# Shimmen/ArkoseRenderer

Hardware: AMD Instinct MI355X
Metric: Mrays/s + probes-updated/s, DDGI 32^3 grid x 256 rays, at 1/2/4/8 MI355X (higher is better)
Workload: dtype f32; 1 GPU; C4: synthetic 10M-triangle strip soup, 32x32x32 probes x 256 rays, whole grid updated per step; triangles=10000000, grid=32, rays_per_probe=256, parallelism=zslab1, bvh_nodes=1132708, bvh_max_depth=11

## Files before the change

arkoserenderer_amd/abi.py:

```python
from __future__ import annotations

import ctypes as C
import os

_HERE = os.path.dirname(os.path.abspath(__file__))
LIB_PATH = os.environ.get("ARK_DDGI_LIB") or os.path.join(_HERE, "lib", "libark_ddgi.so")

ARK_DDGI_IRRADIANCE_RES = 8
ARK_DDGI_VISIBILITY_RES = 16
ARK_DDGI_ATLAS_PADDING = 1
ARK_DDGI_MAX_RAYS_PER_PROBE = 512
ARK_DDGI_REFERENCE_MAX_PROBE_UPDATES = 4096

ARK_RT_HIT_MASK_OPAQUE = 0x01
ARK_RT_HIT_MASK_MASKED = 0x02
ARK_RT_HIT_MASK_BLEND = 0x04

ARK_BLEND_MODE_OPAQUE = 1
ARK_BLEND_MODE_MASKED = 2
ARK_BLEND_MODE_TRANSLUCENT = 3

ARK_DDGI_OK = 0
ERRORS = {
    -1: "ARK_DDGI_E_INVALID_ARGUMENT",
    -2: "ARK_DDGI_E_NO_PROBE_GRID",
    -3: "ARK_DDGI_E_NO_SCENE",
    -4: "ARK_DDGI_E_OUT_OF_MEMORY",
    -5: "ARK_DDGI_E_DEVICE",
    -6: "ARK_DDGI_E_UNSUPPORTED",
    -7: "ARK_DDGI_E_SIZE_MISMATCH",
}

ARK_DDGI_ATLAS_IRRADIANCE = 0
ARK_DDGI_ATLAS_VISIBILITY = 1
ARK_DDGI_SURFELS = 2
ARK_DDGI_PROBE_OFFSETS = 3
ARK_DDGI_DEBUG_HITS = 100
ARK_DDGI_DEBUG_RAY_STEPS = 101

ARK_DDGI_CLEAR_OVERFLOW_INF = 0
ARK_DDGI_CLEAR_OVERFLOW_MAX_FINITE = 1
ARK_DDGI_SUN_BVH_AUTO = 0
ARK_DDGI_SUN_BVH_WORLD = 1
ARK_DDGI_SUN_BVH_LIGHT_SPACE = 2
ARK_DDGI_FLAG_SERIAL_FRAMES = 0x1
ARK_DDGI_FLAG_NO_BACKGROUND_REBUILD = 0x2
ARK_DDGI_FLAG_GPU_REBUILD = 0x4
ARK_DDGI_FLAG_GPU_REBUILD_SUN = 0x8
ARK_DDGI_FLAG_GPU_REBUILD_SAH = 0x10
ARK_DDGI_FLAG_GPU_REBUILD_PLAN = 0x80
ARK_DDGI_FLAG_NO_SUN_COVER_MAP = 0x20
ARK_DDGI_FLAG_NO_FUSED_SUN_SHADE = 0x40

ARK_TEX_RGBA8_UNORM = 0
ARK_TEX_RGBA8_SRGB = 1
ARK_TEX_R32F = 2
ARK_TEX_RGBA32F = 3
ARK_BRDF_DEFAULT = 0
ARK_BRDF_SKIN = 1
ARK_WRAP_REPEAT = 0
ARK_WRAP_CLAMP_TO_EDGE = 1
ARK_WRAP_MIRRORED_REPEAT = 2
ARK_WRAP_PER_AXIS = 0x100


def ark_wrap_axes(s: int, t: int) -> int:
    return ARK_WRAP_PER_AXIS | (s & 0xF) | ((t & 0xF) << 4)


class ArkDdgiDesc(C.Structure):
    _fields_ = [
        ("struct_size", C.c_uint32),
        ("grid_dims", C.c_int32 * 3),
        ("probe_spacing", C.c_float * 3),
        ("offset_to_first", C.c_float * 3),
        ("z_far", C.c_float),
        ("max_rays_per_probe", C.c_int32),
        ("max_probe_updates", C.c_int32),
        ("device", C.c_int32),
        ("clear_overflow_mode", C.c_int32),
        ("shard_rank", C.c_int32),
        ("shard_count", C.c_int32),
        ("sun_bvh", C.c_int32),
        ("flags", C.c_uint32),
        ("build_threads", C.c_int32),
        ("reserved", C.c_int32 * 1),
    ]


class ArkRTVertex(C.Structure):
    _fields_ = [("tex_coord", C.c_float * 2), ("normal", C.c_float * 3), ("tangent", C.c_float * 4)]


class ArkRTTriangleMesh(C.Structure):
    _fields_ = [("first_vertex", C.c_int32), ("first_index", C.c_int32), ("material_index", C.c_int32)]


class ArkShaderMaterial(C.Structure):
    _fields_ = [
        ("base_color", C.c_int32),
        ("normal_map", C.c_int32),
        ("metallic_roughness", C.c_int32),
        ("emissive", C.c_int32),
        ("occlusion", C.c_int32),
        ("bent_normal_map", C.c_int32),
# ... 365 lines not shown
    "ark_ddgi_write": (C.c_int, [C.c_void_p, C.c_int, C.c_void_p, C.c_uint64]),
    "ark_ddgi_state_size": (C.c_int, [C.c_void_p, C.POINTER(C.c_uint64)]),
    "ark_ddgi_save_state": (C.c_int, [C.c_void_p, C.c_void_p, C.c_uint64]),
    "ark_ddgi_load_state": (C.c_int, [C.c_void_p, C.c_void_p, C.c_uint64]),
    "ark_ddgi_get_device_views": (C.c_int, [C.c_void_p, C.POINTER(ArkDdgiDeviceViews)]),
    "ark_ddgi_reset_history": (C.c_int, [C.c_void_p]),
    "ark_ddgi_set_counting": (C.c_int, [C.c_void_p, C.c_int]),
    "ark_ddgi_get_counters": (C.c_int, [C.c_void_p, C.POINTER(ArkDdgiCounters)]),
    "ark_ddgi_get_last_timings": (C.c_int, [C.c_void_p, C.POINTER(C.c_float), C.c_int]),
    "ark_ddgi_set_timing": (C.c_int, [C.c_void_p, C.c_int]),
    "ark_ddgi_get_bvh_stats": (C.c_int, [C.c_void_p, C.POINTER(ArkDdgiBvhStats)]),
    "ark_ddgi_bake_ao": (C.c_int, [C.c_void_p, C.POINTER(ArkBakeAoDesc), C.c_void_p]),
    "ark_ddgi_bake_read": (C.c_int, [C.c_void_p, C.c_int, C.c_void_p, C.c_uint64]),
    "ark_ddgi_lighting_compose": (C.c_int, [C.c_void_p, C.POINTER(ArkComposeDesc), C.c_void_p]),
    "ark_ddgi_probe_debug": (C.c_int, [C.c_void_p, C.POINTER(ArkProbeDebugDesc), C.c_void_p]),
    "ark_ddgi_rt_reflections": (C.c_int, [C.c_void_p, C.POINTER(ArkReflectionsDesc), C.c_void_p]),
    "ark_ies_lut_from_memory": (C.c_int, [C.c_char_p, C.c_uint64, C.c_uint32, C.c_void_p, C.POINTER(ArkIesInfo)]),
    "ark_ies_lut_from_file": (C.c_int, [C.c_char_p, C.c_uint32, C.c_void_p, C.POINTER(ArkIesInfo)]),
    "ark_ies_lookup": (C.c_int, [C.c_char_p, C.c_uint64, C.c_float, C.c_float, C.POINTER(C.c_float)]),
    "ark_ies_last_error": (C.c_char_p, []),
    "ark_soup_default_params": (None, [C.POINTER(ArkSoupParams)]),
    "ark_soup_generate": (C.c_int, [C.POINTER(ArkSoupParams), C.POINTER(C.c_void_p)]),
    "ark_soup_scene_view": (C.POINTER(ArkDdgiScene), [C.c_void_p]),
    "ark_soup_free": (None, [C.c_void_p]),
    "ark_ddgi_debug_fmath": (C.c_int, [C.c_int, C.c_int, C.c_void_p, C.c_void_p, C.c_void_p, C.c_uint64]),
    "ark_ddgi_debug_fmath_host": (C.c_int, [C.c_int, C.c_void_p, C.c_void_p, C.c_void_p, C.c_uint64]),
    "ark_ddgi_debug_struct_sizes": (C.c_int, [C.POINTER(C.c_uint32), C.c_int]),
    "ark_ddgi_debug_bvh8_check": (C.c_int, [C.c_void_p, C.c_uint64, C.POINTER(C.c_uint64)]),
    "ark_ddgi_debug_bvh8_check_opts": (C.c_int, [C.c_void_p, C.c_uint64, C.c_int, C.c_float, C.POINTER(C.c_uint64)]),
    "ark_ddgi_debug_sun_bvh_check": (C.c_int, [C.c_void_p, C.c_uint64, C.c_void_p, C.c_void_p, C.c_uint64, C.c_float, C.POINTER(C.c_uint64)]),
    "ark_ddgi_debug_sun_choice": (C.c_int, [C.c_void_p, C.c_uint64, C.c_void_p, C.c_uint32, C.POINTER(C.c_double)]),
    "ark_ddgi_debug_scene_digest": (C.c_int, [C.c_void_p, C.POINTER(C.c_uint64)]),
    "ark_ddgi_debug_lbvh_check": (C.c_int, [C.c_void_p, C.c_uint64, C.POINTER(C.c_uint64)]),
    "ark_ddgi_debug_lbvh_check_opts": (C.c_int, [C.c_void_p, C.c_uint64, C.c_int, C.POINTER(C.c_uint64)]),
    "ark_ddgi_debug_lbvh_device_parity_sah": (C.c_int, [C.c_int, C.c_void_p, C.c_uint64, C.c_void_p, C.c_uint32, C.c_void_p, C.c_int, C.c_int, C.POINTER(C.c_uint64)]),
    "ark_ddgi_debug_lbvh_device_parity": (C.c_int, [C.c_int, C.c_void_p, C.c_uint64, C.c_void_p, C.c_uint32, C.c_void_p, C.c_int, C.POINTER(C.c_uint64)]),
    "ark_ddgi_debug_bvh8_compare_selftest": (C.c_int, [C.c_void_p, C.c_uint64, C.c_void_p, C.c_uint64, C.POINTER(C.c_uint64)]),
    "ark_ddgi_debug_world_bvh_check": (C.c_int, [C.c_void_p, C.POINTER(C.c_uint64)]),
    "ark_ddgi_debug_lbvh_check_sah": (C.c_int, [C.c_void_p, C.c_uint64, C.c_int, C.c_int, C.POINTER(C.c_uint64)]),
    "ark_ddgi_debug_lbvh_check_plan": (C.c_int, [C.c_void_p, C.c_uint64, C.c_int, C.c_int, C.c_int, C.POINTER(C.c_uint64)]),
    "ark_ddgi_debug_sun_lbvh_check_plan": (C.c_int, [C.c_void_p, C.c_uint64, C.c_void_p, C.c_void_p, C.c_uint64, C.c_float, C.c_int, C.c_int, C.c_int, C.POINTER(C.c_uint64)]),
    "ark_ddgi_debug_lbvh_device_parity_plan": (C.c_int, [C.c_int, C.c_void_p, C.c_uint64, C.c_void_p, C.c_uint32, C.c_void_p, C.c_int, C.c_int, C.c_int, C.POINTER(C.c_uint64)]),
    "ark_ddgi_debug_sun_lbvh_check_sah": (C.c_int, [C.c_void_p, C.c_uint64, C.c_void_p, C.c_void_p, C.c_uint64, C.c_float, C.c_int, C.c_int, C.POINTER(C.c_uint64)]),
    "ark_ddgi_debug_sun_lbvh_check": (C.c_int, [C.c_void_p, C.c_uint64, C.c_void_p, C.c_void_p, C.c_uint64, C.c_float, C.POINTER(C.c_uint64)]),
    "ark_ddgi_debug_sun_lbvh_check_opts": (C.c_int, [C.c_void_p, C.c_uint64, C.c_void_p, C.c_void_p, C.c_uint64, C.c_float, C.c_int, C.POINTER(C.c_uint64)]),
    "ark_ddgi_debug_sun_bvh_installed_check": (C.c_int, [C.c_void_p, C.POINTER(C.c_uint64)]),
    "ark_ddgi_debug_refit_reach": (C.c_int, [C.c_void_p, C.POINTER(C.c_uint64)]),
    "ark_ddgi_debug_cover_map_check": (C.c_int, [C.c_void_p, C.c_uint64, C.c_void_p, C.c_void_p, C.c_uint64, C.c_float, C.c_uint64, C.POINTER(C.c_uint64)]),
    "ark_ddgi_debug_cover_map_device": (C.c_int, [C.c_int, C.c_void_p, C.c_uint64, C.c_void_p, C.c_uint64, C.POINTER(C.c_uint64)]),
    "ark_ddgi_debug_sun_cover_counts": (C.c_int, [C.c_void_p, C.POINTER(C.c_uint64)]),
    "ark_ddgi_debug_sun_cover_counts_device": (C.c_int, [C.c_void_p, C.POINTER(C.c_uint64)]),
    "ark_ddgi_debug_shade_schedule": (C.c_int, [C.c_void_p, C.POINTER(C.c_uint64)]),
    "ark_ddgi_debug_set_sun_only_small_windows": (C.c_int, [C.c_void_p, C.c_int]),
}

_lib = None


def library_path() -> str:
    return LIB_PATH


def load_library(path: str | None = None) -> C.CDLL:
    global _lib
    if _lib is not None and path is None:
        return _lib
    p = path or LIB_PATH
    if not os.path.exists(p):
        raise RuntimeError(f"libark_ddgi.so not found at {p}: run __graft_entry__.build() (no CPU fallback exists)")
    try:
        import torch
    except ImportError:
        pass
    lib = C.CDLL(p)
    for name, (res, args) in EXPORTS.items():
        fn = getattr(lib, name)
        fn.restype = res
        fn.argtypes = args
    if path is None:
        _lib = lib
    return lib


class ArkDdgiError(RuntimeError):
    def __init__(self, status: int, message: str):
        super().__init__(f"{ERRORS.get(status, status)}: {message}")
        self.status = status
```

arkoserenderer_amd/csrc/ark_ddgi.cpp:

```cpp
#include <hip/hip_runtime.h>
#include <rocprofiler-sdk-roctx/roctx.h>

#include <algorithm>
#include <chrono>
#include <cmath>
#include <cstdio>
#include <cstdlib>
#include <cstring>
#include <memory>
#include <string>
#include <vector>

#include "../../include/ark_ddgi.h"
#include "../../include/ark_ddgi_debug.h"
#include "ark_fmath.h"
#include "ddgi_kernels.h"
#include "scene_store.h"
#include "shade_schedule.h"
#include "sun_bvh.h"
#include "sun_cover_build.h"

using namespace ark;

namespace {
// ... 27 lines not shown
    return u;
}

void sampleTraversalOrder(uint32_t R, std::vector<uint32_t>& order)
{
    order.resize(R);
    for (uint32_t i = 0; i < R; ++i) order[i] = i;
    const uint32_t G = (R + 63) / 64;
    if (G <= 1) return;
    auto fib = [](uint32_t i, uint32_t n, double* d) {
        const double phi = 2.0 * M_PI * std::fmod(i * 0.6180339887498949, 1.0);
        const double z = 1.0 - (2.0 * i + 1.0) / n, r = std::sqrt(std::max(0.0, 1.0 - z * z));
        d[0] = std::cos(phi) * r; d[1] = std::sin(phi) * r; d[2] = z;
    };
    std::vector<double> pts(3 * R), ctr(3 * G);
    for (uint32_t i = 0; i < R; ++i) fib(i, R, &pts[3 * i]);
    for (uint32_t g = 0; g < G; ++g) fib(g, G, &ctr[3 * g]);
    struct Pair { double d; uint32_t i, g; };
    std::vector<Pair> pairs;
    pairs.reserve(static_cast<size_t>(R) * G);
    for (uint32_t i = 0; i < R; ++i)
        for (uint32_t g = 0; g < G; ++g)
            pairs.push_back({ pts[3 * i] * ctr[3 * g] + pts[3 * i + 1] * ctr[3 * g + 1] + pts[3 * i + 2] * ctr[3 * g + 2], i, g });
    std::stable_sort(pairs.begin(), pairs.end(), [](const Pair& a, const Pair& b) { return a.d > b.d; });
    std::vector<int> groupOf(R, -1);
    std::vector<uint32_t> room(G, 64u);
    room[G - 1] = R - 64u * (G - 1);
    for (const Pair& q : pairs)
        if (groupOf[q.i] < 0 && room[q.g] > 0) { groupOf[q.i] = static_cast<int>(q.g); room[q.g]--; }
    uint32_t k = 0;
    for (uint32_t g = 0; g < G; ++g)
        for (uint32_t i = 0; i < R; ++i)
            if (groupOf[i] == static_cast<int>(g)) order[k++] = i;
}

}

struct ArkDdgiCtx : ErrorSink {
    ArkDdgiDesc desc {};
    hipStream_t stream = nullptr;
    hipEvent_t evOrder = nullptr;
    hipStream_t orderStream = nullptr;
    bool orderValid = false;
    uint32_t refillMin = kRefillMin, sunRefillMin = kSunRefillMin, grabChunk = kGrabChunk;
    int device = 0;
    int cuCount = 0;
    int X = 0, Y = 0, Z = 0, N = 0;
    int Wi = 0, Hi = 0, Wv = 0, Hv = 0;
    int Kmax = 0, Rmax = 0;
    int slabZ0 = 0, slabZ1 = 0;
    DeviceBuffer irr, vis, offsets;
    DeviceBuffer slots, slotOrder, fib, fibOrder, order, hits, surfels, spill, rayCounter, counters, shadeWork, reflWork;
    DeviceBuffer raySteps;
    std::vector<uint32_t> orderHost;
    uint32_t orderR = 0;
    uint32_t lightCount = 0;
    uint32_t spillEntries = 0;
    uint32_t traceBlocks = 0, shadeBlocks = 0, shadowBlocks = 0, shadowBlocksPerCu = 1;
    bool pipelining = true;
    int sunBvh = -1;
    uint32_t pipeTraceBlocks = 0;
    bool pipeReady = false;
    uint32_t parity = 0;
    uint32_t prevR = 0;
    bool prevPipelined = false;
    hipStream_t traceStream = nullptr;
    hipEvent_t evTraced = nullptr, evFrameDone[2] = {};
    bool frameDoneValid[2] = { false, false };
    bool seqSync = true;
    DeviceBuffer seqWords;
    uint32_t frameSeq = 0;
    uint32_t setSeq[2] = { 0, 0 };
    bool setSeqValid[2] = { false, false };
    uint64_t seqTimeoutTicks = 0;
    uint32_t seqTimeoutMs = 10000;
    uint64_t wallClockKhz = 100000;
    uint32_t* hostAbort = nullptr;
    uint32_t* hostAbortDev = nullptr;
    uint32_t seqTimeouts = 0;
    uint32_t lastMainSeq = 0;
    hipStream_t lastStream = nullptr;
    hipEvent_t evExchangeSrc = nullptr;
    hipEvent_t evExchangeDone = nullptr;
    uint32_t exchSeq = 0;
    uint32_t pendingExchange = 0;
    uint32_t lastParity = 0;
    uint32_t fibR[2] = { 0, 0 };
    uint64_t spillRegionWords = 0;
    bool hasScene = false;
    std::shared_ptr<SceneStore> sceneStore;
    uint32_t sceneVersion = 0;
    DeviceBuffer lights;
    std::vector<GpuSpotLight> spotHost;
    int32_t hasSun = 0;
    float sunColor[3] { 0, 0, 0 }, sunDir[3] { 0, 0, 0 };
    bool lightsDirty = false;
    DeviceBuffer bakeTri, bakeBary, bakeOut, bakePixels, bakeCounters;
    uint32_t bakeW = 0, bakeH = 0;
    int bakeBent = 0;
    SceneArgs scene {};
    ArkDdgiBvhStats bvhStats {};
    uint32_t bvhMaxDepth = 0;
    bool counting = false;
    bool lastSunOnly = false;
    const uint32_t* lastDeferredCount = nullptr;
    bool sunOnlySmallWindows = false;
// ... 133 lines not shown
                       std::memcmp(ctx->sunDir, cm.dir, sizeof(ctx->sunDir)) == 0 && 2.0f * ctx->desc.z_far >= cm.grid.wExtent;
    sc.sun_map = mapOk ? cm.buf.as<float2>() : nullptr;
    if (mapOk) {
        sc.sun_grid = cm.grid;
        sc.map_lift = cover::kTmin + cm.grid.margin;
        sc.map_reach = cover::kTmin - cm.grid.margin;
        std::memcpy(sc.sun_frame, cm.frame, sizeof(sc.sun_frame));
    }
    ctx->scene = sc;
    ctx->lightCount = (ctx->hasSun ? 1u : 0u) + static_cast<uint32_t>(ctx->spotHost.size());
    ctx->bvhStats = st.bvhStats;
    ctx->bvhMaxDepth = st.bvhMaxDepth;
    ctx->sceneVersion = st.version;
}

int refreshScene(ArkDdgiCtx* ctx)
{
    deriveSceneArgs(ctx);
    return ensureSpill(ctx);
}

hipError_t flushLights(ArkDdgiCtx* ctx, hipStream_t s)
{
    if (!ctx->lightsDirty) return hipSuccess;
    LightBlock b {};
    b.count = static_cast<uint32_t>(ctx->spotHost.size());
    std::copy(ctx->spotHost.begin(), ctx->spotHost.end(), b.spots);
    const hipError_t e = launch_store_lights(b, ctx->lights.as<GpuSpotLight>(), s);
    if (e == hipSuccess) ctx->lightsDirty = false;
    return e;
}

hipError_t drainContext(ArkDdgiCtx* ctx)
{
    hipError_t e = hipStreamSynchronize(ctx->traceStream);
    if (e == hipSuccess && ctx->orderValid) e = hipEventSynchronize(ctx->evOrder);
    return e;
}

SceneCall sceneCall(ArkDdgiCtx* ctx)
{
    SceneCall c {};
    c.err = ctx;
    c.flags = ctx->desc.flags;
    c.hasSun = ctx->hasSun != 0;
    std::copy(ctx->sunDir, ctx->sunDir + 3, c.sunDir);
    c.shared = ctx->sceneStore.use_count() > 1;
    return c;
}

int adoptScene(ArkDdgiCtx* ctx, std::shared_ptr<SceneStore> st)
{
    ctx->geometrySeen = st->geometrySeq;
    ctx->hasSun = st->hasSunScene;
    for (int k = 0; k < 3; ++k) {
        ctx->sunColor[k] = st->sunScene.color[k];
        ctx->sunDir[k] = st->sunScene.world_space_direction[k];
    }
    ctx->spotHost = st->spotsScene;
    ctx->sceneStore = std::move(st);
    if (!ctx->lights.ptr) ARK_HIP(ctx->lights.alloc((kMaxLights - 1) * sizeof(GpuSpotLight)));
    if (!ctx->spotHost.empty()) ARK_HIP(hipMemcpy(ctx->lights.ptr, ctx->spotHost.data(), ctx->spotHost.size() * sizeof(GpuSpotLight), hipMemcpyHostToDevice));
    ctx->lightsDirty = false;
    deriveSceneArgs(ctx);
    int rc;
    if ((rc = ensureShadeWork(ctx)) != 0) return rc;
    if ((rc = ensureSpill(ctx)) != 0) return rc;
    ctx->hasScene = true;
    return ARK_DDGI_OK;
}

}

extern "C" {

int32_t ark_ddgi_abi_version(void) { return ARK_DDGI_ABI_VERSION; }

int ark_ddgi_create(const ArkDdgiDesc* desc, ArkDdgiCtx** outCtx)
{
    if (!desc || !outCtx || desc->struct_size != sizeof(ArkDdgiDesc)) return ARK_DDGI_E_INVALID_ARGUMENT;
    *outCtx = nullptr;
    if (desc->grid_dims[0] <= 0 || desc->grid_dims[1] <= 0 || desc->grid_dims[2] <= 0) return ARK_DDGI_E_NO_PROBE_GRID;
    auto* ctx = new ArkDdgiCtx();
    ctx->desc = *desc;
    ctx->X = desc->grid_dims[0];
    ctx->Y = desc->grid_dims[1];
    ctx->Z = desc->grid_dims[2];
    ctx->N = ctx->X * ctx->Y * ctx->Z;
    ctx->Rmax = desc->max_rays_per_probe > 0 ? desc->max_rays_per_probe : ARK_DDGI_MAX_RAYS_PER_PROBE;
    ctx->Kmax = desc->max_probe_updates > 0 ? desc->max_probe_updates : ARK_DDGI_REFERENCE_MAX_PROBE_UPDATES;
    const int shards = desc->shard_count > 0 ? desc->shard_count : 1;
    if (ctx->Rmax > ARK_DDGI_MAX_RAYS_PER_PROBE || ctx->Z % shards != 0 || desc->shard_rank < 0 || desc->shard_rank >= shards ||
        desc->sun_bvh < ARK_DDGI_SUN_BVH_AUTO || desc->sun_bvh > ARK_DDGI_SUN_BVH_LIGHT_SPACE || (desc->flags & ~(ARK_DDGI_FLAG_SERIAL_FRAMES | ARK_DDGI_FLAG_NO_BACKGROUND_REBUILD | ARK_DDGI_FLAG_GPU_REBUILD | ARK_DDGI_FLAG_GPU_REBUILD_SUN | ARK_DDGI_FLAG_GPU_REBUILD_SAH | ARK_DDGI_FLAG_GPU_REBUILD_PLAN | ARK_DDGI_FLAG_NO_SUN_COVER_MAP | ARK_DDGI_FLAG_NO_FUSED_SUN_SHADE)) ||
        desc->build_threads < 0) {
        delete ctx;
        return ARK_DDGI_E_INVALID_ARGUMENT;
    }
    ctx->desc.shard_count = shards;
    ctx->slabZ0 = desc->shard_rank * (ctx->Z / shards);
    ctx->slabZ1 = ctx->slabZ0 + ctx->Z / shards;
    const int si = ARK_DDGI_IRRADIANCE_RES + 2 * ARK_DDGI_ATLAS_PADDING;
    const int sv = ARK_DDGI_VISIBILITY_RES + 2 * ARK_DDGI_ATLAS_PADDING;
    ctx->Wi = ctx->X * si * ctx->Y;
    ctx->Hi = ctx->Z * si;
    ctx->Wv = ctx->X * sv * ctx->Y;
    ctx->Hv = ctx->Z * sv;
    auto bad = [&](hipError_t e, const char* what) {
        std::fprintf(stderr, "ark_ddgi_create: %s: %s\n", what, hipGetErrorString(e));
        delete ctx;
        return ARK_DDGI_E_DEVICE;
    };
    hipError_t e = hipSetDevice(desc->device);
    if (e != hipSuccess) return bad(e, "hipSetDevice");
    ctx->device = desc->device;
    hipDeviceProp_t prop;
    e = hipGetDeviceProperties(&prop, desc->device);
    if (e != hipSuccess) return bad(e, "hipGetDeviceProperties");
    ctx->cuCount = prop.multiProcessorCount;
    if ((e = hipStreamCreateWithFlags(&ctx->stream, hipStreamNonBlocking)) != hipSuccess) return bad(e, "hipStreamCreate");
    if ((e = hipEventCreateWithFlags(&ctx->evOrder, hipEventDisableTiming)) != hipSuccess) return bad(e, "hipEventCreate");
    ctx->pipelining = (desc->flags & ARK_DDGI_FLAG_SERIAL_FRAMES) == 0;
    ctx->sunBvh = desc->sun_bvh == ARK_DDGI_SUN_BVH_WORLD ? 0 : desc->sun_bvh == ARK_DDGI_SUN_BVH_LIGHT_SPACE ? 1 : -1;
    if (const char* pc = std::getenv("ROCPROF_COUNTER_COLLECTION"))
        if (*pc && std::strcmp(pc, "0") != 0 && std::strcmp(pc, "false") != 0) ctx->seqSync = false;
    if ((e = hipStreamCreateWithFlags(&ctx->traceStream, hipStreamNonBlocking)) != hipSuccess) return bad(e, "hipStreamCreate");
    const unsigned syncFlags = hipEventDisableTiming;
    if ((e = hipEventCreateWithFlags(&ctx->evTraced, syncFlags)) != hipSuccess) return bad(e, "hipEventCreate");
    if ((e = hipEventCreateWithFlags(&ctx->evExchangeSrc, hipEventDisableTiming)) != hipSuccess) return bad(e, "hipEventCreate");
    if ((e = hipEventCreateWithFlags(&ctx->evExchangeDone, hipEventDisableTiming)) != hipSuccess) return bad(e, "hipEventCreate");
    for (auto& ev : ctx->evFrameDone)
        if ((e = hipEventCreateWithFlags(&ev, syncFlags)) != hipSuccess) return bad(e, "hipEventCreate");
    for (auto& ev : ctx->ev)
        if ((e = hipEventCreate(&ev)) != hipSuccess) return bad(e, "hipEventCreate");
    const size_t K = static_cast<size_t>(ctx->Kmax), R = static_cast<size_t>(ctx->Rmax);
    if ((e = ctx->irr.alloc(static_cast<size_t>(ctx->Wi) * ctx->Hi * 8)) != hipSuccess) return bad(e, "alloc irradiance");
    if ((e = ctx->vis.alloc(static_cast<size_t>(ctx->Wv) * ctx->Hv * 4)) != hipSuccess) return bad(e, "alloc visibility");
    if ((e = ctx->offsets.alloc(static_cast<size_t>(ctx->N) * 16)) != hipSuccess) return bad(e, "alloc offsets");
    if ((e = ctx->slots.alloc(2 * K * sizeof(GpuProbeSlot))) != hipSuccess) return bad(e, "alloc slots");
    if ((e = ctx->slotOrder.alloc(2 * K * 4)) != hipSuccess) return bad(e, "alloc slot order");
    if ((e = ctx->fib.alloc(2 * R * 16)) != hipSuccess) return bad(e, "alloc fib");
    if ((e = ctx->order.alloc(R * 4)) != hipSuccess) return bad(e, "alloc order");
    if ((e = ctx->fibOrder.alloc(2 * R * 16)) != hipSuccess) return bad(e, "alloc fib order");
    if ((e = ctx->hits.alloc(2 * K * R * sizeof(GpuHit))) != hipSuccess) return bad(e, "alloc hits");
    if ((e = ctx->surfels.alloc(K * R * 8)) != hipSuccess) return bad(e, "alloc surfels");
    if ((e = ctx->rayCounter.alloc(2 * kRayCounterWords * 4)) != hipSuccess) return bad(e, "alloc counter");
    if ((e = ctx->counters.alloc(10 * sizeof(unsigned long long))) != hipSuccess) return bad(e, "alloc counters");
    if ((e = ctx->seqWords.alloc(128 * 4)) != hipSuccess) return bad(e, "alloc sequence words");
    if ((e = hipMemset(ctx->seqWords.ptr, 0, ctx->seqWords.bytes)) != hipSuccess) return bad(e, "clear sequence words");
    {
        int rateKhz = 0;
        if (hipDeviceGetAttribute(&rateKhz, hipDeviceAttributeWallClockRate, ctx->device) != hipSuccess || rateKhz <= 0) rateKhz = 100000;
        ctx->wallClockKhz = static_cast<uint64_t>(rateKhz);
        ctx->seqTimeoutTicks = ctx->wallClockKhz * ctx->seqTimeoutMs;
    }
    if ((e = hipHostMalloc(reinterpret_cast<void**>(&ctx->hostAbort), 64, hipHostMallocCoherent | hipHostMallocMapped)) != hipSuccess)
        return bad(e, "hipHostMalloc sequencing flag");
    *reinterpret_cast<volatile uint32_t*>(ctx->hostAbort) = 0u;
    if ((e = hipHostGetDevicePointer(reinterpret_cast<void**>(&ctx->hostAbortDev), ctx->hostAbort, 0)) != hipSuccess)
        return bad(e, "hipHostGetDevicePointer sequencing flag");
    int occT = 0, occS = 0, occW = 0;
    if ((e = hipOccupancyMaxActiveBlocksPerMultiprocessor(&occT, kernel_trace_ptr(false), kTraceBlock, 0)) != hipSuccess) return bad(e, "occupancy trace");
    if ((e = hipOccupancyMaxActiveBlocksPerMultiprocessor(&occS, kernel_shade_ptr(false), kShadeBlock, 0)) != hipSuccess) return bad(e, "occupancy shade");
    if ((e = hipOccupancyMaxActiveBlocksPerMultiprocessor(&occW, kernel_trace_shadow_ptr(false), kTraceBlock, 0)) != hipSuccess) return bad(e, "occupancy shadow");
    ctx->traceBlocks = static_cast<uint32_t>(std::max(1, occT) * ctx->cuCount);
    ctx->pipeTraceBlocks = static_cast<uint32_t>(std::min(kPipeTracePerCu, std::max(1, occT)) * ctx->cuCount);
    ctx->shadeBlocks = static_cast<uint32_t>(std::max(1, occS) * ctx->cuCount);
    ctx->shadowBlocks = static_cast<uint32_t>(std::max(1, occW) * ctx->cuCount);
    ctx->shadowBlocksPerCu = static_cast<uint32_t>(std::max(1, occW));
    if (clearHistory(ctx) != ARK_DDGI_OK) {
        std::fprintf(stderr, "ark_ddgi_create: %s\n", ctx->lastError.c_str());
        delete ctx;
        return ARK_DDGI_E_DEVICE;
    }
    *outCtx = ctx;
    return ARK_DDGI_OK;
}

void ark_ddgi_destroy(ArkDdgiCtx* ctx)
{
    if (!ctx) return;
    (void)hipSetDevice(ctx->device);
    (void)hipDeviceSynchronize();
    for (DeviceBuffer* b : { &ctx->irr, &ctx->vis, &ctx->offsets, &ctx->slots, &ctx->slotOrder, &ctx->fib, &ctx->fibOrder, &ctx->order, &ctx->hits, &ctx->surfels, &ctx->spill, &ctx->rayCounter, &ctx->seqWords, &ctx->shadeWork, &ctx->reflWork,
                             &ctx->raySteps, &ctx->counters, &ctx->lights, &ctx->bakeTri, &ctx->bakeBary, &ctx->bakeOut, &ctx->bakePixels, &ctx->bakeCounters })
        b->release();
    ctx->sceneStore.reset();
    for (auto& ev : ctx->ev)
        if (ev) (void)hipEventDestroy(ev);
    if (ctx->evOrder) (void)hipEventDestroy(ctx->evOrder);
    if (ctx->evTraced) (void)hipEventDestroy(ctx->evTraced);
    if (ctx->evExchangeSrc) (void)hipEventDestroy(ctx->evExchangeSrc);
    if (ctx->evExchangeDone) (void)hipEventDestroy(ctx->evExchangeDone);
    for (auto& ev : ctx->evFrameDone)
        if (ev) (void)hipEventDestroy(ev);
    if (ctx->traceStream) (void)hipStreamDestroy(ctx->traceStream);
    if (ctx->stream) (void)hipStreamDestroy(ctx->stream);
    if (ctx->hostAbort) (void)hipHostFree(ctx->hostAbort);
    delete ctx;
}

const char* ark_ddgi_last_error(const ArkDdgiCtx* ctx) { return ctx ? ctx->lastError.c_str() : "null context"; }

int ark_ddgi_set_scene(ArkDdgiCtx* ctx, const ArkDdgiScene* s)
{
    if (!ctx) return ARK_DDGI_E_INVALID_ARGUMENT;
    ctx->pipeReady = false;
    if (!s || s->struct_size != sizeof(ArkDdgiScene)) return ctx->fail(ARK_DDGI_E_INVALID_ARGUMENT, "bad ArkDdgiScene");
    ARK_HIP(hipSetDevice(ctx->device));
    ARK_HIP(hipDeviceSynchronize());
    ctx->hasScene = false;
    ctx->sceneStore.reset();
    std::shared_ptr<SceneStore> st;
    if (const int rc = buildScene(ctx, s, ctx->device, ctx->desc.build_threads, ctx->sunBvh, (ctx->desc.flags & ARK_DDGI_FLAG_NO_SUN_COVER_MAP) == 0, st)) return rc;
    return adoptScene(ctx, std::move(st));
}

int ark_ddgi_share_scene(ArkDdgiCtx* ctx, const ArkDdgiCtx* src)
{
    if (!ctx) return ARK_DDGI_E_INVALID_ARGUMENT;
    ctx->pipeReady = false;
    if (!src || src == ctx || !src->hasScene || !src->sceneStore) return ctx->fail(ARK_DDGI_E_INVALID_ARGUMENT, "share_scene: the source context has no scene");
    if (src->device != ctx->device) return ctx->fail(ARK_DDGI_E_INVALID_ARGUMENT, "share_scene: contexts on devices %d and %d", src->device, ctx->device);
    ARK_HIP(hipSetDevice(ctx->device));
    ARK_HIP(hipDeviceSynchronize());
    std::shared_ptr<SceneStore> st = src->sceneStore;
    ctx->hasScene = false;
    ctx->sceneStore.reset();
    return adoptScene(ctx, std::move(st));
}

int ark_ddgi_set_lights(ArkDdgiCtx* ctx, const ArkDdgiLights* L)
{
    if (!ctx) return ARK_DDGI_E_INVALID_ARGUMENT;
    if (!L || L->struct_size != sizeof(ArkDdgiLights)) return ctx->fail(ARK_DDGI_E_INVALID_ARGUMENT, "bad ArkDdgiLights");
    if (!ctx->hasScene) return ctx->fail(ARK_DDGI_E_NO_SCENE, "ark_ddgi_set_lights before ark_ddgi_set_scene");
    if (L->spot_light_count > ARK_DDGI_MAX_SPOT_LIGHTS) return ctx->fail(ARK_DDGI_E_UNSUPPORTED, "at most %d spot lights (GpuScene.cpp:430)", ARK_DDGI_MAX_SPOT_LIGHTS);
    if (L->spot_light_count && !L->spot_lights) return ctx->fail(ARK_DDGI_E_INVALID_ARGUMENT, "set_lights: null spot_lights");
// ... 136 lines not shown
    if (inUse) {
        std::vector<GpuTriangle> rec(st.world.records);
        ARK_HIP(hipMemcpy(rec.data(), st.world.tris(st.world.buf), rec.size() * sizeof(GpuTriangle), hipMemcpyDeviceToHost));
        double frame[3][3];
        sun_frame(ctx->sunDir, frame);
        float L[3];
        sunRayDirection(ctx->sunDir, L);
        ok = hostBuildCoverMap(rec.data(), rec.size(), &frame[0][0], L, cover::kDefaultBudget, grid, map) && 2.0f * ctx->desc.z_far >= grid.wExtent;
        for (int k = 0; k < 9; ++k) F[k] = static_cast<float>((&frame[0][0])[k]);
        if (ok) {
            if (std::memcmp(&grid, &st.coverMap.grid, sizeof(grid)) != 0) {
                out[11] = ~0ull;
            } else {
                std::vector<float> dmap(map.size());
                ARK_HIP(hipMemcpy(dmap.data(), st.coverMap.buf.ptr, dmap.size() * 4u, hipMemcpyDeviceToHost));
                for (size_t i = 0; i < map.size(); ++i) out[11] += cover::floatBits(map[i]) != cover::floatBits(dmap[i]);
            }
        }
    }
    const float lift = cover::kTmin + grid.margin, reach = cover::kTmin - grid.margin;
    for (uint32_t i = 0; i < f.window_rays; ++i) {
        const float* o = &P[4u * i];
        if (o[3] == 0.0f) continue;
        int vd = cover::kUndecided;
        if (ok) {
            const float pl[3] = { std::fma(o[0], F[0], std::fma(o[1], F[1], o[2] * F[2])), std::fma(o[0], F[3], std::fma(o[1], F[4], o[2] * F[5])),
                                  std::fma(o[0], F[6], std::fma(o[1], F[7], o[2] * F[8])) };
            const int64_t c = cover::cellIndex(grid, pl[0], pl[1]);
            if (c >= 0) vd = cover::verdict(pl[2], lift, reach, map[2 * c], map[2 * c + 1]);
        }
        out[vd == cover::kOccluded ? 8 : vd == cover::kLit ? 9 : 10]++;
    }
    return ARK_DDGI_OK;
}

int ark_ddgi_debug_set_sun_only_small_windows(ArkDdgiCtx* ctx, int enabled)
{
    if (!ctx) return ARK_DDGI_E_INVALID_ARGUMENT;
    ctx->sunOnlySmallWindows = enabled != 0;
    return ARK_DDGI_OK;
}

int ark_ddgi_debug_shade_schedule(ArkDdgiCtx* ctx, uint64_t* out)
{
    if (!ctx || !out) return ARK_DDGI_E_INVALID_ARGUMENT;
    out[0] = out[1] = 0;
    if (!ctx->lastSunOnly) return ARK_DDGI_OK;
    ARK_HIP(hipSetDevice(ctx->device));
    ARK_HIP(hipDeviceSynchronize());
    uint32_t n = 0;
    ARK_HIP(hipMemcpy(&n, ctx->lastDeferredCount, sizeof(n), hipMemcpyDeviceToHost));
    out[0] = 1;
    out[1] = n;
    return ARK_DDGI_OK;
}

int ark_ddgi_set_instances(ArkDdgiCtx* ctx, const ArkRTInstance* instances, uint32_t count)
{
    if (!ctx) return ARK_DDGI_E_INVALID_ARGUMENT;
    const auto t0 = std::chrono::steady_clock::now();
    if (const int rc = ark_ddgi_set_instances_async(ctx, instances, count, ctx->stream)) return rc;
    ARK_HIP(hipStreamSynchronize(ctx->stream));
    ctx->sceneStore->bvhStats.refit_ms = std::chrono::duration<float, std::milli>(std::chrono::steady_clock::now() - t0).count();
    ctx->bvhStats = ctx->sceneStore->bvhStats;
    return ARK_DDGI_OK;
}

static uint32_t countSlabProbes(const ArkDdgiCtx* ctx, uint32_t first, uint32_t K)
{
    if (ctx->desc.shard_count <= 1) return K;
    return slabRankOf(static_cast<uint32_t>(ctx->X), static_cast<uint32_t>(ctx->Y), static_cast<uint32_t>(ctx->Z), static_cast<uint32_t>(ctx->slabZ0),
                      static_cast<uint32_t>(ctx->slabZ1), first, K);
}

static int updateImpl(ArkDdgiCtx* ctx, const ArkDdgiFrameParams* p, void* hipStream, void* shadeWaitEvent, void* doneEvent, uint32_t shadeWaitSeq = 0);

static int checkSequencing(ArkDdgiCtx* ctx)
{
    if (!ctx->hostAbort || __atomic_load_n(ctx->hostAbort, __ATOMIC_ACQUIRE) == 0u) return ARK_DDGI_OK;
    ARK_HIP(hipSetDevice(ctx->device));
    ARK_HIP(hipDeviceSynchronize());
    ARK_HIP(hipMemset(ctx->seqWords.as<uint32_t>() + 64, 0, 4));
    __atomic_store_n(ctx->hostAbort, 0u, __ATOMIC_RELEASE);
    ctx->seqSync = false;
    ctx->pipeReady = false;
    ++ctx->seqTimeouts;
    return ctx->fail(ARK_DDGI_E_DEVICE,
                     "a frame-sequencing wait between the context's streams gave up after %u ms: every update kernel that started after it skipped "
                     "(its atlases, surfels and offsets left as they were); the context now orders its streams with events",
                     ctx->seqTimeoutMs);
}

int ark_ddgi_set_sequencing(ArkDdgiCtx* ctx, int device_sequence_words, uint32_t timeout_ms)
{
    if (!ctx) return ARK_DDGI_E_INVALID_ARGUMENT;
    if (timeout_ms > 3600u * 1000u) return ctx->fail(ARK_DDGI_E_INVALID_ARGUMENT, "sequencing timeout %u ms above one hour", timeout_ms);
    ctx->seqSync = device_sequence_words != 0;
    if (timeout_ms) {
        ctx->seqTimeoutMs = timeout_ms;
        ctx->seqTimeoutTicks = ctx->wallClockKhz * timeout_ms;
    }
    return ARK_DDGI_OK;
}

int ark_ddgi_get_sequencing(const ArkDdgiCtx* ctx, int* out_device_sequence_words, uint32_t* out_timeout_ms, uint32_t* out_timeouts)
{
// ... 142 lines not shown
        f.origin[k] = ctx->desc.offset_to_first[k];
    }
    f.z_far = ctx->desc.z_far;
    f.frame = p->frame_index;
    f.first = p->first_probe_index % N;
    f.window = K;
    f.sharded = ctx->desc.shard_count > 1 ? 1 : 0;
    f.slab_z0 = ctx->slabZ0;
    f.slab_z1 = ctx->slabZ1;
    f.window_probes = countSlabProbes(ctx, f.first, K);
    f.R = R;
    f.Rmax = static_cast<uint32_t>(ctx->Rmax);
    f.window_rays = f.window_probes * R;
    f.hysteresis_irradiance = p->hysteresis_irradiance;
    f.hysteresis_visibility = p->hysteresis_visibility;
    f.visibility_sharpness = p->visibility_sharpness;
    f.ambient_amount = p->ambient_amount;
    f.environment_multiplier = p->environment_multiplier;
    f.delta_time = p->delta_time;
    f.update_offsets = p->update_offsets;
    f.irr = ctx->irr.as<uint16_t>();
    f.vis = ctx->vis.as<uint16_t>();
    f.offsets = ctx->offsets.as<float4>();
    const bool timing = ctx->timing;
    const bool count = ctx->counting;
    const bool pipe = ctx->pipelining && ctx->pipeReady && !timing && !count && R == ctx->prevR;
    const uint32_t b = ctx->parity;
    const uint64_t Kmax = static_cast<uint64_t>(ctx->Kmax), Rmax = static_cast<uint64_t>(ctx->Rmax);
    f.slots = ctx->slots.as<GpuProbeSlot>() + b * Kmax;
    f.fib = ctx->fib.as<float4>() + b * Rmax;
    RoctxRange ddgiZone("DDGI");
    ARK_HIP(orderBegin(ctx, s));
    if (const int rc = sceneMaintenance(*ctx->sceneStore, sceneCall(ctx), s)) return rc;
    if (ctx->sceneVersion != ctx->sceneStore->version)
        if (const int rc = refreshScene(ctx)) return rc;
    ARK_HIP(flushLights(ctx, s));
    if (ctx->orderR != R) {
        sampleTraversalOrder(R, ctx->orderHost);
        ARK_HIP(hipMemcpyAsync(ctx->order.ptr, ctx->orderHost.data(), R * 4, hipMemcpyHostToDevice, s));
        ctx->orderR = R;
    }
    f.order = ctx->order.as<uint32_t>();
    f.fib_order = ctx->fibOrder.as<float4>() + b * Rmax;
    f.hits = ctx->hits.as<GpuHit>() + b * Kmax * Rmax;
    f.surfels = ctx->surfels.as<uint16_t>();
    f.spill = ctx->spill.as<uint32_t>() + ctx->spillRegionWords;
    f.light_count = ctx->lightCount;
    f.refill_min = ctx->refillMin;
    f.sun_refill_min = ctx->sunRefillMin;
    f.grab_chunk = (pipe && f.window_rays < kPipeHalfRays) ? std::min<uint32_t>(ctx->grabChunk, 32u) : ctx->grabChunk;
    f.ray_counter = ctx->rayCounter.as<uint32_t>() + b * kRayCounterWords;
    f.counters = ctx->counters.as<unsigned long long>();
    f.ray_steps = count ? ctx->raySteps.as<uint16_t>() : nullptr;
    f.cover_counts = count ? ctx->counters.as<uint32_t>() + ctx->counters.bytes / 4u - 3u : nullptr;
    ctx->coverCountsValid = count;
    {
        const ShadeWorkLayout l = shadeWorkLayout(ctx);
        char* w = static_cast<char*>(ctx->shadeWork.ptr);
        f.shadow_bits = reinterpret_cast<uint32_t*>(w + l.bits);
        f.shadow_rays = reinterpret_cast<ShadowRay*>(w + l.list);
    }
    f.shadow_count = f.ray_counter + kShadowCountWord;
    f.shadow_heads = f.ray_counter + kShadowHeadWord;
    if (ctx->scene.sun_root >= 0) {
        f.sun_rays = f.shadow_rays;
        f.shadow_rays += Kmax * Rmax;
        f.sun_count = f.ray_counter + kSunCountWord;
        f.sun_heads = f.ray_counter + kSunHeadWord;
    }
    const hipStream_t ts = pipe ? ctx->traceStream : s;
    uint32_t* seqTrace = ctx->seqWords.as<uint32_t>();
    uint32_t* seqMain = seqTrace + 32;
    uint32_t* seqTimedOut = seqTrace + 64;
    const bool seq = pipe && ctx->seqSync;
    const uint32_t seqN = seq ? ++ctx->frameSeq : 0u;
    if (pipe && ctx->setSeqValid[b]) ARK_HIP(launch_seq_wait(seqMain, ctx->setSeq[b], seqTimedOut, ctx->hostAbortDev, ctx->seqTimeoutTicks, ts));
    else if (pipe && ctx->frameDoneValid[b]) ARK_HIP(hipStreamWaitEvent(ts, ctx->evFrameDone[b], 0));
    if (pipe && !ctx->prevPipelined && ctx->frameDoneValid[b ^ 1u]) ARK_HIP(hipStreamWaitEvent(ts, ctx->evFrameDone[b ^ 1u], 0));
    if (ctx->geometrySeen != ctx->sceneStore->geometrySeq) {
        ARK_HIP(hipStreamWaitEvent(ts, ctx->sceneStore->evGeometry, 0));
        ctx->geometrySeen = ctx->sceneStore->geometrySeq;
    }
    if (count) ARK_HIP(hipMemsetAsync(ctx->counters.ptr, 0, ctx->counters.bytes, s));
    if (timing) ARK_HIP(hipEventRecord(ctx->ev[0], s));
    f.slot_order = ctx->slotOrder.as<uint32_t>() + b * Kmax;
    ARK_HIP(launch_probe_slots(f, ts));
    if (f.window_probes > 0) {
        RoctxRange traceZone("Trace rays");
        const bool half = pipe && f.window_rays < kPipeHalfRays;
        ARK_HIP(launch_trace(ctx->scene, f, half ? ctx->pipeTraceBlocks : ctx->traceBlocks, count, ts));
        if (pipe) {
            ARK_HIP(launch_probe_offsets(f, ts));
            ARK_HIP(tracedSync(ctx, seq, seqN, ts, s));
        }
        if (timing) ARK_HIP(hipEventRecord(ctx->ev[1], s));
        FrameArgs fs = f;
        fs.spill = ctx->spill.as<uint32_t>();
        if (count) ctx->coverFrame = fs;
        const bool sunOnly = shadeScheduleOf({ f.light_count, ctx->scene.has_sun != 0, ctx->scene.sun_map != nullptr, ctx->desc.flags, half,
                                               ctx->sunOnlySmallWindows }) == ShadeSchedule::SunOnly;
        ctx->lastSunOnly = sunOnly;
        ctx->lastDeferredCount = fs.sun_rays ? fs.sun_count : fs.shadow_count;
        if (f.light_count > 0 && !sunOnly) {
            ARK_HIP(launch_shadow_gen(ctx->scene, fs, s));
            ARK_HIP(launch_trace_shadow(ctx->scene, fs, count ? ctx->shadowBlocks : shadowBlocksFor(ctx, f.window_rays), count, s));
        }
        if (timing) ARK_HIP(hipEventRecord(ctx->ev[5], s));
        if (shadeWaitEvent) ARK_HIP(hipStreamWaitEvent(s, static_cast<hipEvent_t>(shadeWaitEvent), 0));
        if (shadeWaitSeq) ARK_HIP(launch_seq_wait(seqTrace + 96, shadeWaitSeq, seqTimedOut, ctx->hostAbortDev, ctx->seqTimeoutTicks, s));
        ARK_HIP(launch_shade(ctx->scene, fs, ctx->shadeBlocks, count, s, sunOnly));
        if (timing) ARK_HIP(hipEventRecord(ctx->ev[2], s));
        if (sunOnly) {
            ARK_HIP(launch_trace_shadow(ctx->scene, fs, count ? ctx->shadowBlocks : shadowBlocksFor(ctx, f.window_rays), count, s));
            ARK_HIP(launch_shade_deferred(ctx->scene, fs, s));
        }
        if (timing) ARK_HIP(hipEventRecord(ctx->ev[4], s));
        traceZone.end();
        RoctxRange updateZone("Update probes");
        if (!pipe) ARK_HIP(launch_probe_offsets(fs, s));
        ARK_HIP(launch_probe_update(fs, s));
    } else {
        ctx->lastSunOnly = false;
        if (pipe) ARK_HIP(tracedSync(ctx, seq, seqN, ts, s));
        if (shadeWaitEvent) ARK_HIP(hipStreamWaitEvent(s, static_cast<hipEvent_t>(shadeWaitEvent), 0));
        if (shadeWaitSeq) ARK_HIP(launch_seq_wait(seqTrace + 96, shadeWaitSeq, seqTimedOut, ctx->hostAbortDev, ctx->seqTimeoutTicks, s));
        if (timing) {
            ARK_HIP(hipEventRecord(ctx->ev[1], s));
            ARK_HIP(hipEventRecord(ctx->ev[5], s));
            ARK_HIP(hipEventRecord(ctx->ev[2], s));
            ARK_HIP(hipEventRecord(ctx->ev[4], s));
        }
    }
    if (timing) ARK_HIP(hipEventRecord(ctx->ev[3], s));
    if (seq) {
// ... 463 lines not shown
```

arkoserenderer_amd/csrc/bvh_builder.cpp:

```cpp
#include "bvh_builder.h"

#include "../../include/ark_ddgi.h"
#include "bvh_internal.h"

#include <algorithm>
#include <array>
#include <atomic>
#include <cmath>
#include <cstdint>
#include <cstdlib>
#include <cstdio>
#include <cstring>
#include <memory>
#include <thread>
#include <utility>

namespace ark {
namespace {

struct Ref {
    Aabb box;
    float c[3];
    uint32_t tri;
};
// ... 1119 lines not shown

bool bvhLevelOrder(const GpuBvh8Node* h, uint64_t n, const int32_t* roots, int nRoots, std::vector<uint32_t>& order, std::vector<uint32_t>& offsets)
{
    std::vector<std::vector<uint32_t>> byDepth;
    std::vector<std::pair<uint32_t, uint32_t>> work;
    for (int r = 0; r < nRoots; ++r)
        if (roots[r] >= 0) work.push_back({ static_cast<uint32_t>(roots[r]), 0u });
    while (!work.empty()) {
        const auto [node, d] = work.back();
        work.pop_back();
        if (node >= n) return false;
        if (byDepth.size() <= d) byDepth.resize(d + 1);
        byDepth[d].push_back(node);
        const uint32_t internal = static_cast<uint32_t>(__builtin_popcount(h[node].imask));
        for (uint32_t k = 0; k < internal; ++k) work.push_back({ h[node].child_base + k, d + 1 });
    }
    order.clear();
    order.reserve(n);
    offsets.assign(1, 0u);
    for (size_t d = byDepth.size(); d-- > 0;) {
        std::sort(byDepth[d].begin(), byDepth[d].end());
        order.insert(order.end(), byDepth[d].begin(), byDepth[d].end());
        offsets.push_back(static_cast<uint32_t>(order.size()));
    }
    return true;
}

bool build_world_bvh8(std::vector<BuildTriangle> cls[3], BvhBuildOptions opt, const Bvh8CollapseOptions& copt, WorldBvh8& out, std::string& why)
{
    out = WorldBvh8 {};
    opt.max_leaf_size = kBvh8MaxLeafSize;
    float lo[3] = { INFINITY, INFINITY, INFINITY }, hi[3] = { -INFINITY, -INFINITY, -INFINITY };
    for (int c = 0; c < 3; ++c)
        for (const BuildTriangle& t : cls[c])
            for (const float* v : { t.v0, t.v1, t.v2 })
                for (int a = 0; a < 3; ++a) {
                    lo[a] = std::min(lo[a], v[a]);
                    hi[a] = std::max(hi[a], v[a]);
                }
    out.inflateAbs = opt.inflate_abs = bvh8_inflation_box(lo, hi);
    for (int c = 0; c < 3; ++c) {
        if (cls[c].empty()) continue;
        BvhBuildResult r2 = build_bvh(cls[c], opt, 0u, 0u);
        std::vector<BuildTriangle>().swap(cls[c]);
        out.maxLeaf = std::max(out.maxLeaf, r2.max_leaf);
        if (r2.max_leaf > static_cast<uint32_t>(kBvh8MaxLeafSize)) {
            why = "BVH2 leaf of " + std::to_string(r2.max_leaf) + " triangles";
            return false;
        }
        if (c == 0) out.sah = r2.sah_cost;
        Bvh8BuildResult r = collapse_bvh8(r2, static_cast<uint32_t>(out.nodes.size()), static_cast<uint32_t>(out.tris.size()), copt);
        out.roots[c] = static_cast<int32_t>(out.nodes.size());
        if (c == 0) out.opaqueNodes = static_cast<uint32_t>(r.nodes.size());
        out.depth = std::max(out.depth, r.max_depth);
        out.triangles += r.triangles;
        out.nodes.insert(out.nodes.end(), r.nodes.begin(), r.nodes.end());
        out.tris.insert(out.tris.end(), r.tris.begin(), r.tris.end());
    }
    if (out.nodes.size() >= (1ull << 31) || out.tris.size() >= (1ull << 31)) {
        out.tooLarge = true;
        why = "scene too large for 31-bit BVH indices";
        return false;
    }
    return checkBvh8Structure(out.nodes, out.tris, out.roots, 3, why);
}

}
```

arkoserenderer_amd/csrc/bvh_builder.h:

```cpp
#pragma once

#include <stdint.h>
#include <string>
#include <vector>

#include "ddgi_types.h"

namespace ark {

struct BuildTriangle {
    float v0[3], v1[3], v2[3];
    uint32_t instance;
    uint32_t primitive;
    uint32_t flip_facing;
};

struct BvhBuildOptions {
    int max_leaf_size = 4;
    int bins = 32;
    int max_depth = 60;
    int threads = 0;
    float inflate_abs = 0.0f;
    float traversal_cost = 1.0f;
    float intersection_cost = 1.0f;
    float area_w[3] = { 1.0f, 1.0f, 1.0f };
    int presplit_levels = 0;
    float presplit_ratio = 8.0f;
};

struct BvhBuildResult {
    std::vector<GpuBvhNode> nodes;
    std::vector<GpuTriangle> tris;
    uint32_t max_depth = 0;
    uint32_t max_leaf = 0;
    float sah_cost = 0.0f;
};

BvhBuildResult build_bvh(const std::vector<BuildTriangle>& tris, const BvhBuildOptions& opt, uint32_t node_base, uint32_t tri_base);

struct Bvh8BuildResult {
    std::vector<GpuBvh8Node> nodes;
    std::vector<GpuTriangle> tris;
    uint32_t max_depth = 0;
    uint32_t leaf_children = 0;
    uint64_t triangles = 0;
    float sah_cost = 0.0f;
};

struct Bvh8CollapseOptions {
    bool sah_optimal = true;
    float node_cost = 1.0f;
    float tri_cost = 1.0f;
    float area_w[3] = { 1.0f, 1.0f, 1.0f };
    int slot_sort_axis = -1;
    int threads = 0;
};
Bvh8BuildResult collapse_bvh8(const BvhBuildResult& bvh2, uint32_t node_base, uint32_t tri_base, const Bvh8CollapseOptions& opt);

int hit_mask_class(uint32_t hit_mask);

struct WorldBvh8 {
    std::vector<GpuBvh8Node> nodes;
    std::vector<GpuTriangle> tris;
    int32_t roots[3] = { -1, -1, -1 };
    uint32_t opaqueNodes = 0, depth = 0, maxLeaf = 0;
    uint64_t triangles = 0;
    float sah = 0.0f;
    float inflateAbs = 0.0f;
    bool tooLarge = false;
};
bool build_world_bvh8(std::vector<BuildTriangle> cls[3], BvhBuildOptions opt, const Bvh8CollapseOptions& copt, WorldBvh8& out, std::string& why);

bool checkBvh8Structure(const std::vector<GpuBvh8Node>& allNodes, const std::vector<GpuTriangle>& allTris, const int32_t* roots, int nRoots, std::string& why);
bool bvhLevelOrder(const GpuBvh8Node* h, uint64_t n, const int32_t* roots, int nRoots, std::vector<uint32_t>& order, std::vector<uint32_t>& offsets);

GpuTriangle make_gpu_triangle(const BuildTriangle& t);

GpuTriangle holeTriangle();
bool isHoleTriangle(const GpuTriangle& t);
int bvh8SlotTriangles(const GpuBvh8Node& nd, int s, uint32_t out[kBvh8MaxLeafSize]);
bool decodeSlotBox(const GpuBvh8Node& nd, int slot, float lo[3], float hi[3]);

std::vector<BuildTriangle> soupTriangles(const float* triangles, uint64_t n);

float bvh8_inflation(const float* xyz, uint64_t nTriangles);
float bvh8_inflation_box(const float lo[3], const float hi[3]);

}
```

arkoserenderer_amd/csrc/ddgi_kernels.h:

```cpp
#pragma once

#include <hip/hip_runtime.h>
#include <stdint.h>

#include "../../include/ark_ddgi.h"
#include "ddgi_types.h"
#include "lbvh_build.h"
#include "sun_cover_map.h"

namespace ark {

#ifndef ARK_STACK_LDS
#define ARK_STACK_LDS 8
#endif
#ifndef ARK_LDS_NODES
#define ARK_LDS_NODES 48
#endif
constexpr int kStackLds = ARK_STACK_LDS;
constexpr int kTraceBlock = 256;
constexpr int kLdsNodes = ARK_LDS_NODES;
constexpr int kShadeBlock = 256;
constexpr int kUpdateProbes = 4;
constexpr int kUpdateBlock = 320;
constexpr int kRayParts = 8;
constexpr int kRayCounterStride = 32;
constexpr int kShadeChunk = 1024;
constexpr int kMaxLights = 11;
constexpr uint32_t kNoHit = 0xffffffffu;

struct ProbeXZY {
    uint32_t y, z, x;
};

__host__ __device__ inline ProbeXZY probeXZY(uint32_t X, uint32_t Z, uint32_t p)
{
    const uint32_t XZ = X * Z, y = p / XZ, r = p - y * XZ, z = r / X;
    return { y, z, r - z * X };
}

__host__ __device__ inline uint32_t boxProbesBelow(ProbeXZY q, uint32_t xa, uint32_t xb, uint32_t za, uint32_t zb)
{
    const uint32_t zc = q.z < za ? za : (q.z > zb ? zb : q.z);
    const uint32_t xc = q.x < xa ? xa : (q.x > xb ? xb : q.x);
    return q.y * (xb - xa) * (zb - za) + (xb - xa) * (zc - za) + ((q.z >= za && q.z < zb) ? xc - xa : 0u);
}

__host__ __device__ inline uint32_t windowBoxCount(uint32_t X, uint32_t Y, uint32_t Z, uint32_t first, uint32_t s, uint32_t xa, uint32_t xb, uint32_t za,
                                                   uint32_t zb)
{
    const uint32_t N = X * Y * Z;
    const uint64_t end = static_cast<uint64_t>(first) + s;
    const uint32_t below = boxProbesBelow(probeXZY(X, Z, first), xa, xb, za, zb);
    if (end <= N) return boxProbesBelow(probeXZY(X, Z, static_cast<uint32_t>(end)), xa, xb, za, zb) - below;
    return Y * (xb - xa) * (zb - za) - below + boxProbesBelow(probeXZY(X, Z, static_cast<uint32_t>(end - N)), xa, xb, za, zb);
}

__host__ __device__ inline uint32_t slabRankOf(uint32_t X, uint32_t Y, uint32_t Z, uint32_t z0, uint32_t z1, uint32_t first, uint32_t s)
{
    return windowBoxCount(X, Y, Z, first, s, 0u, X, z0, z1);
}
// ... 4 lines not shown
    return x * 8u / X;
}

__host__ __device__ inline void slotBucketBox(uint32_t X, uint32_t zlo, uint32_t zext, uint32_t b, uint32_t& xa, uint32_t& xb, uint32_t& za, uint32_t& zb)
{
    if (zext >= 2) {
        const uint32_t bx = b & 3u, zm = (zext + 1u) / 2u;
        xa = (bx * X + 3u) / 4u;
        xb = ((bx + 1u) * X + 3u) / 4u;
        za = zlo + ((b >> 2) ? zm : 0u);
        zb = zlo + ((b >> 2) ? zext : zm);
    } else {
        xa = (b * X + 7u) / 8u;
        xb = ((b + 1u) * X + 7u) / 8u;
        za = zlo;
        zb = zlo + zext;
    }
}

__host__ __device__ inline uint32_t slotQueuePos(uint32_t X, uint32_t Y, uint32_t Z, uint32_t zlo, uint32_t zext, uint32_t first, uint32_t K, uint32_t s,
                                                 uint32_t p)
{
    const ProbeXZY q = probeXZY(X, Z, p);
    const uint32_t b = slotBucketOf(X, zlo, zext, q.x, q.z);
    uint32_t xa, xb, za, zb, pos = 0;
    for (uint32_t k = 0; k < b; ++k) {
        slotBucketBox(X, zlo, zext, k, xa, xb, za, zb);
        pos += windowBoxCount(X, Y, Z, first, K, xa, xb, za, zb);
    }
    slotBucketBox(X, zlo, zext, b, xa, xb, za, zb);
    return pos + windowBoxCount(X, Y, Z, first, s, xa, xb, za, zb);
}

struct alignas(16) ShadowRay {
    float4 origin_tmax;
    float4 dir_owner;
};

constexpr int kShadeHeadWord = kRayParts * kRayCounterStride;
constexpr int kShadowCountWord = 2 * kRayParts * kRayCounterStride;
constexpr int kShadowHeadWord = kShadowCountWord + kRayCounterStride;
constexpr int kSunCountWord = kShadowHeadWord + kRayParts * kRayCounterStride;
constexpr int kSunHeadWord = kSunCountWord + kRayCounterStride;
constexpr int kRayCounterWords = kSunHeadWord + kRayParts * kRayCounterStride;

struct SceneArgs {
    const GpuBvh8Node* nodes;
    const GpuTriangle* tris;
    uint32_t tri_byte_offset;
    int32_t root_opaque;
    int32_t root_masked;
    int32_t root_blend;
    uint32_t opaque_nodes;
    int32_t texture_count;
    const uint32_t* indices;
    const float* vertices;
    const ArkRTTriangleMesh* meshes;
    const ArkShaderMaterial* materials;
    const GpuInstance* instances;
    const GpuTextureInfo* tex_infos;
    const float4* texels;
    int32_t white_texture;
    int32_t env_texture;
    int32_t has_sun;
    int32_t spot_count;
    float sun_color[3];
    float sun_dir[3];
    const GpuSpotLight* spots;
    const float4* tri_normals;
    const GpuBvh8Node* sun_nodes;
    const GpuTriangle* sun_tris;
    int32_t sun_root = -1;
    float sun_frame[9];
    const float2* sun_map;
    cover::Grid sun_grid;
    float map_lift, map_reach;

    __device__ __forceinline__ int resolveTexture(int idx) const
    {
        return (idx >= 0 && idx < texture_count) ? idx : white_texture;
    }
    __device__ __forceinline__ float4 sample(int idx, float u, float v) const;
};

struct FrameArgs {
    int32_t X, Y, Z;
    int32_t Wi, Hi, Wv, Hv;
    float spacing[3];
    float origin[3];
    float z_far;
    uint32_t frame;
    uint32_t first;
    uint32_t window;
    uint32_t window_probes;
    uint32_t window_rays;
    uint32_t R;
    uint32_t Rmax;
    int32_t sharded;
    int32_t slab_z0, slab_z1;
    float hysteresis_irradiance;
    float hysteresis_visibility;
    float visibility_sharpness;
    float ambient_amount;
    float environment_multiplier;
    float delta_time;
    int32_t update_offsets;
    uint16_t* irr;
    uint16_t* vis;
    float4* offsets;
    GpuProbeSlot* slots;
    float4* fib;
    const uint32_t* order;
    const uint32_t* slot_order;
    float4* fib_order;
    GpuHit* hits;
    uint16_t* surfels;
    uint32_t* spill;
    uint32_t light_count;
    uint32_t refill_min;
    uint32_t sun_refill_min;
    uint32_t grab_chunk;
    uint32_t* shadow_bits;
    ShadowRay* shadow_rays;
    uint32_t* shadow_count;
    uint32_t* shadow_heads;
    ShadowRay* sun_rays;
    uint32_t* sun_count;
    uint32_t* sun_heads;
    uint32_t* ray_counter;
    unsigned long long* counters;
    uint32_t* cover_counts;
    uint16_t* ray_steps;
    const float4* ray_list;
    const uint32_t* list_count;
    const uint32_t* abort_word;
};

__device__ __forceinline__ bool frameAborted(const uint32_t* abortWord)
{
    if (!abortWord) return false;
    __shared__ uint32_t sAbort;
    if (threadIdx.x == 0) sAbort = __hip_atomic_load(abortWord, __ATOMIC_RELAXED, __HIP_MEMORY_SCOPE_AGENT);
    __syncthreads();
    return sAbort != 0u;
}

struct BakeArgs {
    uint32_t W, H, samples, tri_count;
    int32_t bent;
    uint32_t first_index, first_vertex;
    const uint32_t* indices;
    const float* positions;
    const float* vertices;
    uint32_t* tri_idx;
    uint16_t* bary;
    uint8_t* out;
    uint32_t* pixels;
    uint32_t* counters;
    uint32_t* spill;
};

struct LightBlock {
    GpuSpotLight spots[kMaxLights - 1];
    uint32_t count;
};
struct alignas(16) RefitInstance {
    float m[12];
    int32_t first_vertex;
    uint32_t first_index;
    uint32_t flip;
    uint32_t dirty;
};
struct RefitBoxArgs {
    double frame[9];
    float inflate;
    uint32_t light;
    uint64_t dirty;
};
hipError_t launch_store_lights(const LightBlock& b, GpuSpotLight* dst, hipStream_t s);
hipError_t launch_node_masks(const GpuBvh8Node* nodes, const GpuTriangle* tris, uint64_t* masks, const uint32_t* order, uint32_t count, hipStream_t s);
hipError_t launch_refit_nodes(GpuBvh8Node* nodes, GpuTriangle* tris, float* boxes, const uint32_t* order, uint32_t count, const RefitBoxArgs& a,
                              const uint64_t* masks, const RefitInstance* inst, const uint32_t* indices, const float* positions, hipStream_t s);
hipError_t launch_gather_records(float4* dst, const float4* src, const uint32_t* perm, uint64_t count, hipStream_t s);

struct LbvhHeader {
// ... 119 lines not shown
```

arkoserenderer_amd/csrc/ddgi_kernels.hip:

```cpp

#include <hip/hip_runtime.h>

#include <algorithm>
#include <cstdlib>
#include <type_traits>
#include <utility>
#include <vector>

#include "../../include/ark_ddgi.h"
#include "ddgi_device.h"
#include "ddgi_kernels.h"

namespace ark {

__device__ __forceinline__ float4 SceneArgs::sample(int idx, float u, float v) const
{
    const int r = resolveTexture(idx);
    if (r == white_texture && fabsf(u) < INFINITY && fabsf(v) < INFINITY) return make_float4(1.0f, 1.0f, 1.0f, 1.0f);
    return dev::sampleTexture(tex_infos, texels, r, u, v);
}

namespace dev {

__device__ V3 sphericalFibonacciSample(uint32_t i, uint32_t n)
// ... 649 lines not shown
        const uint32_t off = atomicAdd(heads + p * kRayCounterStride, CHUNK);
        if (off < pe - pb) {
            b = pb + off;
            e = min(b + CHUNK, pe);
            return;
        }
    }
}

__device__ __forceinline__ uint32_t waveAtomicAdd(uint32_t* p, uint32_t v, uint32_t lane)
{
    uint32_t off = 0;
    if (lane == 0) off = atomicAdd(p, v);
    return __builtin_amdgcn_readfirstlane(off);
}

__device__ __forceinline__ void grabItemsWave(uint32_t* heads, uint32_t total, uint32_t home, uint32_t lane, uint32_t& tried, uint32_t& b, uint32_t& e, uint32_t CHUNK)
{
    b = e = 0;
    for (; tried < kRayParts; ++tried) {
        const uint32_t p = (home + tried) & (kRayParts - 1);
        const uint32_t pb = static_cast<uint32_t>(static_cast<uint64_t>(total) * p / kRayParts);
        const uint32_t pe = static_cast<uint32_t>(static_cast<uint64_t>(total) * (p + 1) / kRayParts);
        if (pb >= pe) continue;
        const uint32_t off = waveAtomicAdd(heads + p * kRayCounterStride, CHUNK, lane);
        if (off < pe - pb) {
            b = pb + off;
            e = min(b + CHUNK, pe);
            return;
        }
    }
}

__device__ __forceinline__ void grabRaysWave(const FrameArgs& f, uint32_t* heads, uint32_t home, uint32_t lane, uint32_t& tried, uint32_t& b, uint32_t& e, uint32_t CHUNK)
{
    b = e = 0;
    for (; tried < kRayParts; ++tried) {
        const uint32_t p = (home + tried) & (kRayParts - 1);
        const uint32_t pb = partRayBegin(f, p), pe = partRayBegin(f, p + 1);
        if (pb >= pe) continue;
        const uint32_t off = waveAtomicAdd(heads + p * kRayCounterStride, CHUNK, lane);
        if (off < pe - pb) {
            b = pb + off;
            e = min(b + CHUNK, pe);
            return;
        }
    }
}


struct PoolRec {
    V3 o, d;
    uint32_t a;
};

struct ProbeRays {
    static constexpr bool kMaskedPass = true;
    static constexpr float kTmin = 0.0001f;
    __device__ static void grab(const FrameArgs& f, uint32_t home, uint32_t lane, uint32_t& tried, uint32_t& b, uint32_t& e, uint32_t chunk)
    {
        grabRaysWave(f, f.ray_counter, home, lane, tried, b, e, chunk);
    }
    __device__ static PoolRec stage(const FrameArgs& f, uint32_t r)
    {
        const uint32_t qp = r / f.R;
        const uint32_t slot = slotAt(f, qp);
        const float4 fv = f.fib_order[r - qp * f.R];
        const GpuProbeSlot ps = f.slots[slot];
        PoolRec rec;
        rec.o = { ps.pos[0], ps.pos[1], ps.pos[2] };
        rec.d = rotate(v3(fv.x, fv.y, fv.z), v3(ps.axis[0], ps.axis[1], ps.axis[2]), ps.angle_sin, ps.angle_cos);
        rec.a = slot * f.R + __float_as_uint(fv.w);
        return rec;
    }
    __device__ static void take(const FrameArgs& f, uint32_t r, uint32_t recA, uint32_t& ray, float& tmax)
    {
        ray = recA;
        tmax = f.z_far;
    }
};

struct ListRays {
    static constexpr bool kMaskedPass = false;
    static constexpr float kTmin = 0.01f;
    __device__ static void grab(const FrameArgs& f, uint32_t home, uint32_t lane, uint32_t& tried, uint32_t& b, uint32_t& e, uint32_t chunk)
    {
        grabItemsWave(f.ray_counter, *f.list_count, home, lane, tried, b, e, chunk);
    }
    __device__ static PoolRec stage(const FrameArgs& f, uint32_t r)
    {
        const float4 a = f.ray_list[2u * r], b = f.ray_list[2u * r + 1u];
        PoolRec rec;
        rec.o = { a.x, a.y, a.z };
        rec.d = { b.x, b.y, b.z };
        rec.a = __float_as_uint(a.w);
        return rec;
    }
    __device__ static void take(const FrameArgs& f, uint32_t r, uint32_t recA, uint32_t& ray, float& tmax)
    {
        ray = r;
        tmax = __uint_as_float(recA);
    }
};

template<bool COUNT, int WPE, class Src = ProbeRays, int SLOTS = 64>
__global__ void __launch_bounds__(kTraceBlock) __attribute__((amdgpu_waves_per_eu(WPE))) k_trace(SceneArgs sc, FrameArgs f)
{
    if (frameAborted(f.abort_word)) return;
    __shared__ uint32_t ldsStack[kStackLds * 2 * kTraceBlock];
    __shared__ uint4 ldsNodes[5];
    static_assert(SLOTS == 32 || SLOTS == 64, "a wave stages at most one record per lane");
    __shared__ uint4 ldsPool[2 * SLOTS * (kTraceBlock / 64)];
    const NodeCache nc = loadNodeCache<kTraceBlock, 0>(sc, ldsNodes);
    const uint32_t gtid = blockIdx.x * kTraceBlock + threadIdx.x;
    const uint32_t nthreads = gridDim.x * kTraceBlock;
    Stack<kTraceBlock> st { ldsStack + threadIdx.x, f.spill + gtid, nthreads, 0 };
    const uint32_t lane = threadIdx.x & 63u;
    uint4* const pool = ldsPool + 2u * SLOTS * (threadIdx.x >> 6);
    const uint32_t chunk = min(f.grab_chunk, static_cast<uint32_t>(SLOTS));
    const float tmin = Src::kTmin;
    uint32_t cNodes = 0, cTris = 0, cHits = 0, cIter = 0, rSteps = 0;

    uint32_t poolNext = 0, poolEnd = 0;
    uint32_t poolBase = 0;
    const uint32_t home = xccId();
    uint32_t tried = 0;
    bool exhausted = false;
    bool active = false;
    uint32_t ray = 0;
    int pass = 0;
    TravState ts { 0u, 0u, 0u, 0u };
    uint32_t nBase = 0, nBits = 0;
    uint32_t oct = 0;
    V3 o = { 0, 0, 0 }, d = { 0, 0, 1 }, idir = { 0, 0, 1 };
    RayHit h { 0.0f, 0.0f, 0.0f, kNoHit, 0u, 0u, false };
    float opaqueT = 0.0f;
    auto done = [&]() { return travDoneDual(ts, nBits, st); };
    bool pending = false;
    auto storeHit = [&]() {
        GpuHit out;
        if (h.tri == kNoHit) {
            out.t = __builtin_bit_cast(float, 0x7f800000u);
            out.u = out.v = 0.0f;
            out.tri = kNoHit;
        } else {
            out.t = h.backface ? -h.t : h.t;
            out.u = h.u;
            out.v = h.v;
            out.tri = h.tri;
            if (COUNT) cHits++;
        }
        f.hits[ray] = out;
        if (COUNT && f.ray_steps) f.ray_steps[ray] = static_cast<uint16_t>(min(rSteps, 65535u));
        if (COUNT) rSteps = 0;
    };

    for (;;) {
        const uint64_t need = __ballot(!active);
        if (need != 0 && !exhausted && (static_cast<uint32_t>(__popcll(need)) >= f.refill_min || need == ~0ull)) {
            if (pending) {
                storeHit();
                pending = false;
            }
            const uint32_t n = static_cast<uint32_t>(__popcll(need));
            const uint32_t rank = __builtin_amdgcn_mbcnt_hi(static_cast<uint32_t>(need >> 32), __builtin_amdgcn_mbcnt_lo(static_cast<uint32_t>(need), 0u));
            const uint32_t avail = poolEnd - poolNext;
            uint32_t fb = 0, fe = 0;
            if (avail < n) Src::grab(f, home, lane, tried, fb, fe, chunk);
            uint32_t r = kNoHit, recA = 0;
            auto readRec = [&](uint32_t slot) {
                const uint4 lo = pool[slot], hi = pool[SLOTS + slot];
                o = { __uint_as_float(lo.x), __uint_as_float(lo.y), __uint_as_float(lo.z) };
                d = { __uint_as_float(lo.w), __uint_as_float(hi.x), __uint_as_float(hi.y) };
                recA = hi.z;
            };
            if (!active && rank < avail) {
                r = poolNext + rank;
                readRec(r - poolBase);
            }
            if (fb < fe) {
                __builtin_amdgcn_fence(__ATOMIC_SEQ_CST, "wavefront");
                if (lane < fe - fb) {
                    const PoolRec s = Src::stage(f, fb + lane);
                    pool[lane] = make_uint4(__float_as_uint(s.o.x), __float_as_uint(s.o.y), __float_as_uint(s.o.z), __float_as_uint(s.d.x));
                    pool[SLOTS + lane] = make_uint4(__float_as_uint(s.d.y), __float_as_uint(s.d.z), s.a, 0u);
                }
                __builtin_amdgcn_fence(__ATOMIC_SEQ_CST, "wavefront");
                poolBase = __builtin_amdgcn_readfirstlane(fb);
                if (!active && rank >= avail && rank - avail < fe - fb) {
                    r = fb + (rank - avail);
                    readRec(rank - avail);
                }
            }
            if (r != kNoHit) {
                float tmax;
                Src::take(f, r, recA, ray, tmax);
                idir = safeInv(d);
                oct = rayOctant(idir);
                active = true;
                h = RayHit { tmax, 0.0f, 0.0f, kNoHit, 0u, 0u, false };
                pass = 0;
                st.depth = 0;
                nBits = 0;
                ts = TravState { static_cast<uint32_t>(sc.root_opaque), sc.root_opaque >= 0 ? rootGroupBits() : 0u, 0u, 0u };
            }
            if (avail < n) {
                if (fb >= fe) {
                    exhausted = true;
                    poolNext = poolEnd = 0;
                } else {
                    poolNext = min(fb + (n - avail), fe);
                    poolEnd = fe;
                }
            } else {
                poolNext += n;
            }
        }
        if (__ballot(active) == 0) break;
        if (COUNT) {
            cIter++;
            rSteps += active ? 1u : 0u;
        }
        if (active) travStepDual<kTraceBlock, false, true>(sc, nc, ts, nBase, nBits, st, o, d, idir, oct, tmin, h, pass, cNodes, cTris);
        if (active && done() && (!Src::kMaskedPass || sc.root_masked < 0) && !exhausted) {
            active = false;
            pending = true;
        } else if (active && done()) {
            bool finished = true;
            if (Src::kMaskedPass && pass == 0) {
                opaqueT = (h.tri != kNoHit) ? (h.backface ? -h.t : h.t) : f.z_far;
                if (sc.root_masked >= 0 && opaqueT >= tmin) {
                    pass = 1;
                    finished = false;
                    ts = TravState { static_cast<uint32_t>(sc.root_masked), rootGroupBits(), 0u, 0u };
                    st.depth = 0;
                    f.hits[ray] = GpuHit { h.tri == kNoHit ? __builtin_bit_cast(float, 0x7f800000u) : opaqueT, h.u, h.v, h.tri };
                    h = RayHit { opaqueT, 0.0f, 0.0f, kNoHit, 0u, 0u, false };
                }
            }
            if (finished) {
                GpuHit out;
                if (pass == 1 && h.tri == kNoHit) {
                    out = f.hits[ray];
                    if (COUNT && out.tri != kNoHit) cHits++;
                    if (COUNT && f.ray_steps) f.ray_steps[ray] = static_cast<uint16_t>(min(rSteps, 65535u));
                    if (COUNT) rSteps = 0;
                } else {
                    storeHit();
                }
                active = false;
            }
        }
    }
    if (COUNT) {
        atomicAdd(&f.counters[0], static_cast<unsigned long long>(cNodes));
        atomicAdd(&f.counters[1], static_cast<unsigned long long>(cTris));
        atomicAdd(&f.counters[2], static_cast<unsigned long long>(cHits));
        if (lane == 0) atomicAdd(&f.counters[7], static_cast<unsigned long long>(cIter));
    }
}

__device__ __forceinline__ void atlasSampleUV(const FrameArgs& f, int px, int py, int pz, V3 dir, int res, float invW, float invH, float* u, float* v)
{
    const int pad = ARK_DDGI_ATLAS_PADDING;
    int tileX = px + py * f.X, tileY = pz;
    int firstX = pad + tileX * (res + 2 * pad), firstY = pad + tileY * (res + 2 * pad);
    float ex, ey;
    octahedralEncode(dir, &ex, &ey);
    float tx = (ex * 0.5f + 0.5f) * static_cast<float>(res);
    float ty = (ey * 0.5f + 0.5f) * static_cast<float>(res);
    float ax = static_cast<float>(firstX) + tx, ay = static_cast<float>(firstY) + ty;
    *u = ax * invW;
    *v = ay * invH;
}

template<int CH, int NOUT>
__device__ __forceinline__ void sampleAtlas(const uint16_t* __restrict__ atlas, int W, int H, float u, float v, float* out)
{
    float x = u * static_cast<float>(W) - 0.5f;
    float y = v * static_cast<float>(H) - 0.5f;
    float x0f = floorf_(x), y0f = floorf_(y);
    float fx = x - x0f, fy = y - y0f;
    int x0 = static_cast<int>(x0f), y0 = static_cast<int>(y0f);
    int xa = min(max(x0, 0), W - 1), xb = min(max(x0 + 1, 0), W - 1);
    int ya = min(max(y0, 0), H - 1), yb = min(max(y0 + 1, 0), H - 1);
    uint16_t q[4][CH];
    auto loadRow = [&](int k, int yy) {
        const uint16_t* pa = atlas + (static_cast<size_t>(yy) * W + xa) * CH;
        const uint16_t* pb = atlas + (static_cast<size_t>(yy) * W + xb) * CH;
        if (CH == 4) {
            uint2 wa, wb;
            if (xb == xa + 1) {
                const uint4 w = *reinterpret_cast<const uint4*>(pa);
                wa = make_uint2(w.x, w.y);
                wb = make_uint2(w.z, w.w);
            } else {
                wa = *reinterpret_cast<const uint2*>(pa);
                wb = *reinterpret_cast<const uint2*>(pb);
            }
            q[k][0] = static_cast<uint16_t>(wa.x & 0xffffu);
            q[k][1] = static_cast<uint16_t>(wa.x >> 16);
            q[k][2 % CH] = static_cast<uint16_t>(wa.y & 0xffffu);
            q[k][3 % CH] = static_cast<uint16_t>(wa.y >> 16);
            q[k + 1][0] = static_cast<uint16_t>(wb.x & 0xffffu);
            q[k + 1][1] = static_cast<uint16_t>(wb.x >> 16);
            q[k + 1][2 % CH] = static_cast<uint16_t>(wb.y & 0xffffu);
            q[k + 1][3 % CH] = static_cast<uint16_t>(wb.y >> 16);
        } else {
            uint32_t wa, wb;
            if (xb == xa + 1) {
                const uint2 w = *reinterpret_cast<const uint2*>(pa);
// ... 1060 lines not shown
                ++pass;
                while (pass < 3 && roots[pass] < 0) ++pass;
                if (pass < 3) {
                    st.depth = 0;
                    ts = TravState { static_cast<uint32_t>(roots[pass]), rootGroupBits(), 0u, 0u };
                } else {
                    rayDone = true;
                }
            }
            if (rayDone) {
                if (hit) aoAcc += 1.0f;
                else dirAcc = dirAcc + d;
                if (++sampleIdx < b.samples) {
                    startRay();
                } else {
                    if (b.bent) {
                        const V3 bent = dirAcc / static_cast<float>(b.samples);
                        const float cone = (kPi / 2.0f) / (kPi / 2.0f);
                        const V3 enc = bent * v3(0.5f, 0.5f, 0.5f) + v3(0.5f, 0.5f, 0.5f);
                        reinterpret_cast<uint32_t*>(b.out)[pixel] = static_cast<uint32_t>(unorm8(enc.x)) | (static_cast<uint32_t>(unorm8(enc.y)) << 8) |
                                                                    (static_cast<uint32_t>(unorm8(enc.z)) << 16) | (static_cast<uint32_t>(unorm8(cone)) << 24);
                    } else {
                        const float ao = aoAcc / static_cast<float>(b.samples);
                        b.out[pixel] = unorm8(1.0f - ao);
                    }
                    active = false;
                }
            }
        }
    }
}

#include "ddgi_compose.inc"
#include "ddgi_reflections.inc"

}

hipError_t launch_probe_slots(const FrameArgs& f, hipStream_t s)
{
    const uint32_t n = f.window > f.R ? f.window : f.R;
    hipLaunchKernelGGL(dev::k_probe_slots, dim3((n + 255u) / 256u), dim3(256), 0, s, f);
    return hipGetLastError();
}

constexpr int kTraceWpe = 6, kShadowWpe = 6;
const void* kernel_trace_ptr(bool count)
{
    return count ? reinterpret_cast<const void*>(&dev::k_trace<true, 1>) : reinterpret_cast<const void*>(&dev::k_trace<false, kTraceWpe>);
}

hipError_t launch_trace(const SceneArgs& sc, const FrameArgs& f, uint32_t blocks, bool count, hipStream_t s)
{
    void* args[] = { const_cast<SceneArgs*>(&sc), const_cast<FrameArgs*>(&f) };
    const void* fn = kernel_trace_ptr(count);
    if (!count && f.grab_chunk <= 32u) fn = reinterpret_cast<const void*>(&dev::k_trace<false, kTraceWpe, dev::ProbeRays, 32>);
    return hipLaunchKernel(fn, dim3(blocks), dim3(kTraceBlock), args, 0, s);
}

static uint32_t persistentBlocks(const void* fn, int block, uint32_t fallback)
{
    static thread_local std::vector<std::pair<const void*, uint32_t>> cache;
    for (const auto& c : cache)
        if (c.first == fn) return c.second;
    int dev = 0, cus = 0, occ = 0;
    if (hipGetDevice(&dev) != hipSuccess || hipDeviceGetAttribute(&cus, hipDeviceAttributeMultiprocessorCount, dev) != hipSuccess ||
        hipOccupancyMaxActiveBlocksPerMultiprocessor(&occ, fn, block, 0) != hipSuccess || occ <= 0 || cus <= 0)
        return fallback;
    cache.emplace_back(fn, static_cast<uint32_t>(occ * cus));
    return cache.back().second;
}

constexpr int kShadeWpe = 4;
hipError_t launch_shade(const SceneArgs& sc, const FrameArgs& f, uint32_t blocks, bool count, hipStream_t s, bool sunFused)
{
    if (sunFused && (f.light_count != 1u || !sc.has_sun || sc.sun_map == nullptr)) return hipErrorInvalidValue;
    void* args[] = { const_cast<SceneArgs*>(&sc), const_cast<FrameArgs*>(&f) };
    const void* fn;
    if (count) {
        fn = sunFused ? reinterpret_cast<const void*>(&dev::k_shade<true, 1, dev::kShadeSunFused>) : reinterpret_cast<const void*>(&dev::k_shade<true, 1>);
    } else {
        fn = sunFused ? reinterpret_cast<const void*>(&dev::k_shade<false, kShadeWpe, dev::kShadeSunFused>)
                      : reinterpret_cast<const void*>(&dev::k_shade<false, kShadeWpe>);
        blocks = persistentBlocks(fn, kShadeBlock, blocks);
    }
    return hipLaunchKernel(fn, dim3(blocks), dim3(kShadeBlock), args, 0, s);
}

constexpr uint32_t kDeferredBlocks = 512;
hipError_t launch_shade_deferred(const SceneArgs& sc, const FrameArgs& f, hipStream_t s)
{
    hipLaunchKernelGGL((dev::k_shade<false, kShadeWpe, dev::kShadeDeferred>), dim3(kDeferredBlocks), dim3(kShadeBlock), 0, s, sc, f);
    return hipGetLastError();
}

hipError_t launch_trace_shadow(const SceneArgs& sc, const FrameArgs& f, uint32_t blocks, bool count, hipStream_t s)
{
    void* args[] = { const_cast<SceneArgs*>(&sc), const_cast<FrameArgs*>(&f) };
    const void* fn = kernel_trace_shadow_ptr(count);
    if (f.sun_rays && f.light_count <= 1u)
        fn = count ? reinterpret_cast<const void*>(&dev::k_trace_shadow<true, 1, dev::kShadowSun>)
                   : reinterpret_cast<const void*>(&dev::k_trace_shadow<false, kShadowWpe, dev::kShadowSun>);
    else if (f.sun_rays)
        fn = count ? reinterpret_cast<const void*>(&dev::k_trace_shadow<true, 1, dev::kShadowSunWorld>)
                   : reinterpret_cast<const void*>(&dev::k_trace_shadow<false, kShadowWpe, dev::kShadowSunWorld>);
    return hipLaunchKernel(fn, dim3(blocks), dim3(kTraceBlock), args, 0, s);
}

hipError_t launch_shadow_gen(const SceneArgs& sc, const FrameArgs& f, hipStream_t s)
// ... 91 lines not shown
```

arkoserenderer_amd/csrc/ddgi_update.hip:

```cpp

#include <hip/hip_runtime.h>

#include <algorithm>

#include "../../include/ark_ddgi.h"
#include "ddgi_device.h"
#include "ddgi_kernels.h"

namespace ark {
namespace dev {


__device__ __forceinline__ void borderSource(int res, int b, int* dx, int* dy, int* sx, int* sy)
{
    const int side = res + 2;
    if (b < 4) {
        int cx = b & 1, cy = b >> 1;
        int scx = (cx + 1) % 2, scy = (cy + 1) % 2;
        *dx = cx * (side - 1);
        *dy = cy * (side - 1);
        *sx = scx * (side - 1) + (scx == 0 ? 1 : -1);
        *sy = scy * (side - 1) + (scy == 0 ? 1 : -1);
        return;
    }
// ... 282 lines not shown
__host__ __device__ __forceinline__ uint32_t offsetProbesPerBlock(uint32_t R)
{
    const uint32_t p = R ? 1024u / R : 1u;
    return p < 1u ? 1u : (p > 32u ? 32u : p);
}


__host__ __device__ __forceinline__ size_t offsetLdsBytes(uint32_t P, uint32_t R)
{
    return sizeof(float) * (static_cast<size_t>(P) * (6u * R + 8u) + 6u * P) + sizeof(uint32_t) * 2u * P;
}

__global__ void __launch_bounds__(kOffsetBlock) k_probe_offsets(FrameArgs f)
{
    if (frameAborted(f.abort_word)) return;
    extern __shared__ __attribute__((aligned(16))) unsigned char smem[];
    const uint32_t R = f.R;
    const uint32_t P = offsetProbesPerBlock(R);
    const uint32_t stride = 6u * R + 8u;
    float* valL = reinterpret_cast<float*>(smem);
    float* sumL = valL + P * stride;
    uint32_t* cntL = reinterpret_cast<uint32_t*>(sumL + 6u * P);
    const uint32_t tid = threadIdx.x;
    const uint32_t slot0 = blockIdx.x * P;
    const float minAxialSpacing = fminf_(f.spacing[0], fminf_(f.spacing[1], f.spacing[2]));
    const float maxOffset = minAxialSpacing / 2.0f;
    for (uint32_t i = tid; i < 2u * P; i += kOffsetBlock) cntL[i] = 0u;
    __syncthreads();
    constexpr uint32_t kBatch = 4;
    for (uint32_t i0 = 0; i0 < P * R; i0 += kBatch * kOffsetBlock) {
        GpuHit h[kBatch];
        float4 fb[kBatch];
        bool ok[kBatch];
#pragma unroll
        for (uint32_t k = 0; k < kBatch; ++k) {
            const uint32_t i = i0 + k * kOffsetBlock + tid;
            const uint32_t p = i / R, s = i - p * R;
            ok[k] = i < P * R && slot0 + p < f.window_probes;
            if (ok[k]) {
                h[k] = f.hits[static_cast<size_t>(slot0 + p) * R + s];
                fb[k] = f.fib[s];
            }
        }
#pragma unroll
        for (uint32_t k = 0; k < kBatch; ++k) {
            if (!ok[k]) continue;
            const uint32_t i = i0 + k * kOffsetBlock + tid;
            const uint32_t p = i / R, s = i - p * R;
            const float dist = h[k].tri == kNoHit ? f.z_far : (h[k].t < 0.0f ? h[k].t * 0.2f : h[k].t);
            const float a = f16_to_f32(f32_to_f16(dist));
            const uint32_t cls = (a > 0.0f && a < maxOffset) ? 1u : (a < 0.0f ? 2u : 0u);
            const GpuProbeSlot& ps = f.slots[slot0 + p];
            const V3 d = rotate(v3(fb[k].x, fb[k].y, fb[k].z), v3(ps.axis[0], ps.axis[1], ps.axis[2]), ps.angle_sin, ps.angle_cos);
            float* v = valL + p * stride + 6u * s;
            v[0] = cls == 1u ? d.x : 0.0f;
            v[1] = cls == 1u ? d.y : 0.0f;
            v[2] = cls == 1u ? d.z : 0.0f;
            v[3] = cls == 2u ? d.x : 0.0f;
            v[4] = cls == 2u ? d.y : 0.0f;
            v[5] = cls == 2u ? d.z : 0.0f;
            if (cls) atomicAdd(cntL + 2u * p + (cls - 1u), 1u);
        }
    }
    __syncthreads();
    if (tid < 6u * P && slot0 + tid / 6u < f.window_probes) {
        const float* v = valL + (tid / 6u) * stride + tid % 6u;
        float acc = 0.0f;
#pragma unroll 8
        for (uint32_t s = 0; s < R; ++s) acc += v[6u * s];
        sumL[tid] = acc;
    }
    __syncthreads();
    const uint32_t slot = slot0 + tid;
    if (tid < P && slot < f.window_probes) {
        const float* sm = sumL + 6u * tid;
        const V3 accumNearFrontfaceDir = v3(sm[0], sm[1], sm[2]);
        const V3 accumBackfaceDir = v3(sm[3], sm[4], sm[5]);
        const uint32_t nc = cntL[2u * tid], bc = cntL[2u * tid + 1u];
        const uint32_t probeIdx = f.slots[slot].probe_index;
        float4 cur = f.offsets[probeIdx];
        V3 currentOffset = v3(cur.x, cur.y, cur.z);
        V3 offset = splat(0.0f);
        const float stepSize = 0.125f, lerpSpeed = 10.0f;
        if (static_cast<float>(bc) / static_cast<float>(R) >= 0.25f)
            offset = offset + normalize(accumBackfaceDir) * stepSize;
        else if (nc >= 1)
            offset = offset - normalize(accumNearFrontfaceDir) * stepSize;
        else
            offset = offset - currentOffset * stepSize;
        V3 newOffset = currentOffset + offset;
        if (length(newOffset) > maxOffset) newOffset = maxOffset * normalize(newOffset);
        newOffset = mix3(newOffset, currentOffset, exp2f_(-lerpSpeed * f.delta_time));
        f.offsets[probeIdx] = make_float4(newOffset.x, newOffset.y, newOffset.z, 0.0f);
    }
}

}

hipError_t launch_probe_offsets(const FrameArgs& f, hipStream_t s)
{
    if (f.window_probes == 0 || !f.update_offsets) return hipSuccess;
    const uint32_t P = dev::offsetProbesPerBlock(f.R);
    const uint32_t blocks = (f.window_probes + P - 1) / P;
    const size_t lds = dev::offsetLdsBytes(P, f.R);
    static size_t lds_set = 0;
    if (lds > 65536 && lds > lds_set) {
// ... 25 lines not shown
```

arkoserenderer_amd/csrc/lbvh_device_build.cpp:

```cpp
#include "lbvh_device_build.h"

#include <algorithm>
#include <array>
#include <cstring>

#include "../../include/ark_ddgi_debug.h"
#include "bvh8_check.h"
#include "bvh_builder.h"
#include "lbvh_host.h"
#include "sun_bvh.h"

namespace ark {

constexpr uint32_t kGpuBuildMaxDepth = 60;

bool isDeviceFault(hipError_t e)
{
    return e == hipErrorIllegalAddress || e == hipErrorLaunchFailure || e == hipErrorLaunchTimeOut || e == hipErrorECCNotCorrectable || e == hipErrorAssert ||
           e == hipErrorNoDevice || e == hipErrorInvalidDevice;
}

struct LbvhGpuTrace {
    LbvhHeader hdr {};
    std::vector<uint32_t> idx, idxSorted, split;
// ... 186 lines not shown
    a.position = w.position.as<uint32_t>();
    a.counters = w.counters.as<uint32_t>();
    a.criterion = g.sah ? lbvh::kOpenLargestBox : lbvh::kDefaultCriterion;
    a.slotRule = g.slotRule;
    a.wBits = g.wBits;
    a.useSah = g.sah ? 1 : 0;
    a.sah.nbox = w.nbox.as<float>();
    a.sah.pbox = w.pbox.as<float>();
    for (int k = 0; k < 3; ++k) {
        a.sah.lo[k] = lo[k];
        a.sah.hi[k] = hi[k];
    }
    std::vector<std::array<uint32_t, 3>> levels;
    uint32_t nodeTotal = 0, counters[kLbvhCounters] = {};
    for (int c = 0; c < 3; ++c) {
        if (!hdr.classCount[c]) continue;
        g.roots[c] = static_cast<int32_t>(nodeTotal);
        a.items = nullptr;
        a.root.r.first = classLo[c];
        a.root.r.last = classLo[c] + hdr.classCount[c] - 1u;
        a.root.node = classLo[c];
        a.count = 1;
        a.levelBase = nodeTotal;
        int pong = 0;
        for (uint32_t depth = 0; a.count; ++depth) {
            if (depth >= kGpuBuildMaxDepth || a.levelBase + a.count > nodeCap) {
                why = depth >= kGpuBuildMaxDepth ? "BVH8 deeper than the device build installs" : "more nodes than the device build's scratch";
                return hipSuccess;
            }
            a.nextBase = a.levelBase + a.count;
            a.nextCapacity = nodeCap - a.nextBase;
            a.next = w.items[pong].as<lbvh::Member>();
            ARK_GB(hipMemsetAsync(w.counters.as<uint32_t>() + kLbvhNextCount, 0, 4, s));
            ARK_GB(launch_lbvh_collapse(a, s, plan ? w.picks.as<uint32_t>() : nullptr));
            ARK_GB(hipMemcpyAsync(counters, w.counters.ptr, sizeof(counters), hipMemcpyDeviceToHost, s));
            ARK_GB(hipStreamSynchronize(s));
            if (counters[kLbvhOverflow]) {
                why = "more nodes than the device build's scratch";
                return hipSuccess;
            }
            if (counters[kLbvhPlanStalled]) {
                why = "the collapse plan did not finish";
                return hipSuccess;
            }
            if (levels.size() <= depth) levels.push_back({ 0u, 0u, 0u });
            levels[depth][c] = a.count;
            a.items = a.next;
            a.levelBase = a.nextBase;
            a.count = counters[kLbvhNextCount];
            pong ^= 1;
        }
        nodeTotal = a.levelBase;
        if (c == 0) g.opaqueNodes = nodeTotal;
    }
    const uint32_t outRecords = counters[kLbvhRecords];
    if (!(DeviceBvh::bytesFor(nodeTotal, outRecords) < (1ull << 32))) {
        why = "nodes and records of 4 GiB or more";
        return hipSuccess;
    }
    DeviceBvh& b = *g.bvh;
    b.triOffset = DeviceBvh::triOffsetFor(nodeTotal);
    ARK_GB(b.buf.alloc(DeviceBvh::bytesFor(nodeTotal, outRecords)));
    if (g.perm) ARK_GB(g.perm->alloc(std::max<size_t>(16, outRecords * 4ull)));
    GpuBvh8Node* nodes = b.nodes(b.buf);
    GpuTriangle* tris = b.tris(b.buf);
    ARK_GB(hipMemcpyAsync(nodes, w.nodes.ptr, nodeTotal * sizeof(GpuBvh8Node), hipMemcpyDeviceToDevice, s));
    ARK_GB(launch_lbvh_scatter(snap, w.idxSorted.as<uint32_t>(), w.position.as<uint32_t>(), tris, g.perm ? g.perm->as<uint32_t>() : nullptr, n, outRecords, s));
    std::vector<uint32_t>& order = g.order;
    order.clear();
    order.reserve(nodeTotal);
    b.levelOffsets.assign(1, 0u);
    {
        std::vector<std::array<uint32_t, 3>> base(levels.size());
        uint32_t at[3];
        for (int c = 0; c < 3; ++c) at[c] = g.roots[c] >= 0 ? static_cast<uint32_t>(g.roots[c]) : 0u;
        for (size_t d = 0; d < levels.size(); ++d)
            for (int c = 0; c < 3; ++c) {
                base[d][c] = at[c];
                at[c] += levels[d][c];
            }
        for (size_t d = levels.size(); d-- > 0;) {
            for (int c = 0; c < 3; ++c)
                for (uint32_t k = 0; k < levels[d][c]; ++k) order.push_back(base[d][c] + k);
            b.levelOffsets.push_back(static_cast<uint32_t>(order.size()));
        }
    }
    ARK_GB(b.order.alloc(std::max<size_t>(16, order.size() * 4)));
    ARK_GB(hipMemcpyAsync(b.order.ptr, order.data(), order.size() * 4, hipMemcpyHostToDevice, s));
    ARK_GB(hipMemsetAsync(w.masks.ptr, 0xff, nodeTotal * 8ull, s));
    ARK_GB(hipMemsetAsync(w.inst.ptr, 0, instances * sizeof(RefitInstance), s));
    RefitBoxArgs ra {};
    ra.inflate = bvh8_inflation_box(lo, hi);
    ra.light = 0;
    if (g.light) {
        float maxAbs;
        std::memcpy(&maxAbs, &hdr.maxAbs, 4);
        ra.inflate = 2.0f * bvh8_inflation_box(lo, hi) + 2e-6f * maxAbs;
        ra.light = 1;
        std::memcpy(ra.frame, g.frame, sizeof(ra.frame));
    }
    g.inflateAbs = ra.inflate;
    ra.dirty = ~0ull;
    for (size_t l = 0; l + 1 < b.levelOffsets.size(); ++l)
        ARK_GB(launch_refit_nodes(nodes, tris, w.boxes.as<float>(), b.order.as<uint32_t>() + b.levelOffsets[l], b.levelOffsets[l + 1] - b.levelOffsets[l], ra,
                                  w.masks.as<uint64_t>(), w.inst.as<RefitInstance>(), nullptr, nullptr, s));
    ARK_GB(hipStreamSynchronize(s));
// ... 283 lines not shown
```

arkoserenderer_amd/csrc/lbvh_device_build.h:

```cpp
#pragma once

#include <hip/hip_runtime.h>

#include <cstdint>
#include <string>
#include <vector>

#include "device_bvh.h"
#include "lbvh_build.h"

namespace ark {

struct LbvhGpuTrace;

struct LbvhGpuBuild {
    const GpuTriangle* snap = nullptr;
    hipEvent_t evSnap = nullptr;
    uint32_t records = 0;
    std::vector<uint32_t> classHost;
    bool light = false;
    double frame[9] {};
    int slotRule = lbvh::kSlotsOctant, wBits = lbvh::kMortonBits;
    bool sah = false;
    bool plan = false;
    DeviceBvh* bvh = nullptr;
    DeviceBuffer* perm = nullptr;
    LbvhGpuTrace* trace = nullptr;
    int32_t roots[3] { -1, -1, -1 };
    uint32_t opaqueNodes = 0, prims = 0;
    float inflateAbs = 0.0f;
    std::vector<uint32_t> order;
};

hipError_t buildLbvhGpu(LbvhGpuBuild& g, hipStream_t s, std::string& why);

bool isDeviceFault(hipError_t e);

}
```

arkoserenderer_amd/csrc/scene_store.cpp:

```cpp
#include "scene_store.h"

#include <algorithm>
#include <atomic>
#include <chrono>
#include <cmath>
#include <cstring>
#include <mutex>
#include <thread>

#include "../../include/ark_ddgi_debug.h"
#include "ark_fmath.h"
#include "bvh8_check.h"
#include "bvh_builder.h"
#include "lbvh_device_build.h"
#include "sun_bvh.h"
#include "sun_cover_build.h"

#define ARK_HIP(expr) ARK_HIP_TO(err, expr)

namespace ark {

struct RebuildJob {
    enum Kind { World, Sun } kind = World;
    std::thread t;
    std::atomic<bool> done { false };
    uint32_t version = 0;
    uint32_t refitsAt = 0;
    DeviceBuffer snap;
    hipEvent_t evSnap = nullptr;
    uint64_t snapRecords = 0;
    DeviceBvh bvh;
    float ms = 0.0f;
    bool ok = false;
    bool gpu = false, gpuFallback = false;
    std::vector<int> classOf;
    DeviceBuffer perm;
    int32_t roots[3] { -1, -1, -1 };
    uint32_t opaqueNodes = 0, maxLeaf = 0;
    float sah = 0.0f;
    std::string error;
    float dir[3] {};
    double frame[9] {};
    uint32_t instances = 0;
    bool sahPass = false;
    bool planPass = false;
    bool coverWanted = false, coverOk = false;
    float coverDir[3] {};
    double coverFrame[9] {};
    cover::Grid coverGrid {};
    DeviceBuffer coverBuf;
    float coverMs = 0.0f;
    ~RebuildJob()
    {
        if (t.joinable()) t.join();
        bvh.release();
        for (DeviceBuffer* b : { &perm, &snap, &coverBuf }) b->release();
        if (evSnap) (void)hipEventDestroy(evSnap);
    }
};

namespace {

template<typename T>
int upload(ErrorSink* err, DeviceBuffer& buf, const T* data, size_t count)
{
    size_t bytes = count * sizeof(T);
    ARK_HIP(buf.alloc(std::max<size_t>(bytes, 16)));
    if (bytes) ARK_HIP(hipMemcpy(buf.ptr, data, bytes, hipMemcpyHostToDevice));
    return ARK_DDGI_OK;
}

}

GpuSpotLight gpuSpotLight(const ArkSpotLight& sl)
{
    GpuSpotLight g;
    std::memset(&g, 0, sizeof(g));
    for (int k = 0; k < 3; ++k) {
        g.color[k] = sl.color[k];
        g.direction[k] = sl.world_space_direction[k];
        g.right[k] = sl.world_space_right[k];
        g.up[k] = sl.world_space_up[k];
        g.position[k] = sl.world_space_position[k];
    }
    g.position[3] = sl.outer_cone_half_angle;
    g.ies_texture = sl.ies_profile_index;
    return g;
}

namespace {

// ... 211 lines not shown
    return e;
}

struct HostBvh {
    std::vector<GpuBvh8Node> nodes;
    std::vector<GpuTriangle> tris;
    std::vector<uint32_t> perm, order;
};

bool hostBuildWorld(RebuildJob* job, const std::vector<GpuTriangle>& rec, int threads, HostBvh& out)
{
    std::vector<BuildTriangle> cls[3];
    for (size_t i = 0; i < rec.size(); ++i) {
        const GpuTriangle& g = rec[i];
        if (isHoleTriangle(g)) continue;
        uint32_t inst, flip;
        std::memcpy(&inst, &g.t2[1], 4);
        std::memcpy(&flip, &g.t2[3], 4);
        if (inst >= job->classOf.size()) {
            job->error = "record of an unknown instance";
            return false;
        }
        BuildTriangle t;
        const float e1[3] = { g.t0[3], g.t1[0], g.t1[1] }, e2[3] = { g.t1[2], g.t1[3], g.t2[0] };
        for (int a = 0; a < 3; ++a) {
            t.v0[a] = g.t0[a];
            t.v1[a] = g.t0[a] + e1[a];
            t.v2[a] = g.t0[a] + e2[a];
        }
        t.instance = inst;
        t.primitive = static_cast<uint32_t>(i);
        t.flip_facing = flip;
        cls[job->classOf[inst]].push_back(t);
    }
    WorldBvh8 w;
    BvhBuildOptions opt;
    opt.threads = threads;
    Bvh8CollapseOptions copt;
    copt.threads = threads;
    const bool ok = build_world_bvh8(cls, opt, copt, w, job->error);
    if (w.maxLeaf > static_cast<uint32_t>(kBvh8MaxLeafSize)) job->error = "BVH2 leaf over the leaf size";
    if (!ok) return false;
    out.perm.assign(w.tris.size(), 0xffffffffu);
    for (size_t i = 0; i < w.tris.size(); ++i) {
        GpuTriangle& g = w.tris[i];
        if (isHoleTriangle(g)) continue;
        uint32_t src;
        std::memcpy(&src, &g.t2[2], 4);
        out.perm[i] = src;
        g = rec[src];
    }
    std::copy(w.roots, w.roots + 3, job->roots);
    job->opaqueNodes = w.opaqueNodes;
    job->maxLeaf = w.maxLeaf;
    job->sah = w.sah;
    job->bvh.depth = w.depth;
    out.nodes.swap(w.nodes);
    out.tris.swap(w.tris);
    return bvhLevelOrder(out.nodes.data(), out.nodes.size(), job->roots, 3, out.order, job->bvh.levelOffsets);
}

bool hostBuildSun(RebuildJob* job, std::vector<GpuTriangle>& rec, int threads, HostBvh& out)
{
    SunBvhInput in;
    std::memcpy(in.frame, job->frame, sizeof(in.frame));
    sun_add_records(in, rec, threads);
    std::vector<GpuTriangle>().swap(rec);
    BvhBuildOptions opt;
    opt.threads = threads;
    Bvh8CollapseOptions copt;
    copt.threads = threads;
    Bvh8BuildResult r;
    const bool ok = build_sun_bvh(in, opt, copt, r) && !r.nodes.empty();
    job->bvh.inflateAbs = in.inflateAbs;
    job->bvh.depth = r.max_depth;
    out.nodes.swap(r.nodes);
    out.tris.swap(r.tris);
    const int32_t root = 0;
    return ok && bvhLevelOrder(out.nodes.data(), out.nodes.size(), &root, 1, out.order, job->bvh.levelOffsets);
}

bool hostBuild(RebuildJob* job, hipStream_t s, int threads)
{
    const bool world = job->kind == RebuildJob::World;
    bool ok = s && hipEventSynchronize(job->evSnap) == hipSuccess;
    std::vector<GpuTriangle> rec(ok ? job->snapRecords : 0);
    ok = ok && hipMemcpyAsync(rec.data(), job->snap.ptr, rec.size() * sizeof(GpuTriangle), hipMemcpyDeviceToHost, s) == hipSuccess && hipStreamSynchronize(s) == hipSuccess;
    if (!ok) job->error = "snapshot download failed";
    HostBvh h;
    ok = ok && (world ? hostBuildWorld(job, rec, threads, h) : hostBuildSun(job, rec, threads, h));
    if (ok) {
        ok = (!world || (DeviceBvh::bytesFor(h.nodes.size(), h.tris.size()) < (1ull << 32) && job->perm.alloc(std::max<size_t>(16, h.perm.size() * 4)) == hipSuccess)) &&
             job->bvh.order.alloc(std::max<size_t>(16, h.order.size() * 4)) == hipSuccess &&
             (!world || hipMemcpyAsync(job->perm.ptr, h.perm.data(), h.perm.size() * 4, hipMemcpyHostToDevice, s) == hipSuccess) &&
             hipMemcpyAsync(job->bvh.order.ptr, h.order.data(), h.order.size() * 4, hipMemcpyHostToDevice, s) == hipSuccess && uploadBvh(h.nodes, h.tris, s, job->bvh) == hipSuccess;
        if (!ok && job->error.empty()) job->error = "upload failed";
    }
    return ok;
}

void deviceBuildWorld(RebuildJob* job, LbvhGpuBuild& g)
{
    g.classHost.assign(job->classOf.begin(), job->classOf.end());
    g.perm = &job->perm;
    g.sah = job->sahPass;
    g.plan = job->planPass;
}

void deviceBuildSun(RebuildJob* job, LbvhGpuBuild& g)
{
    g.classHost.assign(job->instances, 0u);
    g.light = true;
    std::memcpy(g.frame, job->frame, sizeof(g.frame));
    g.slotRule = lbvh::kSlotsAscendingW;
    g.wBits = lbvh::kSunKeyBitsW;
    g.sah = job->sahPass;
    g.plan = job->planPass;
}

hipError_t deviceBuild(RebuildJob* job, hipStream_t s, std::string& why)
{
    if (job->snapRecords > 0x7fffffffull) {
        why = "no records";
        return hipSuccess;
    }
    const bool world = job->kind == RebuildJob::World;
    LbvhGpuBuild g;
    g.snap = job->snap.as<GpuTriangle>();
    g.evSnap = job->evSnap;
    g.records = static_cast<uint32_t>(job->snapRecords);
    g.bvh = &job->bvh;
    world ? deviceBuildWorld(job, g) : deviceBuildSun(job, g);
    const hipError_t e = buildLbvhGpu(g, s, why);
    if (world) {
        std::copy(g.roots, g.roots + 3, job->roots);
        job->opaqueNodes = g.opaqueNodes;
        job->maxLeaf = std::min<uint32_t>(g.prims, static_cast<uint32_t>(kBvh8MaxLeafSize));
        job->sah = 0.0f;
    } else {
        job->bvh.inflateAbs = g.inflateAbs;
    }
    return e;
}

void runRebuildJob(RebuildJob* job, int device, int threads, bool tryDevice)
{
    const auto t0 = std::chrono::steady_clock::now();
    hipStream_t s = nullptr;
    auto openStream = [&](bool lowest) {
        hipError_t e = hipSetDevice(device);
        int least = 0, greatest = 0;
        if (e == hipSuccess && lowest) e = hipDeviceGetStreamPriorityRange(&least, &greatest);
        if (e == hipSuccess) e = lowest ? hipStreamCreateWithPriority(&s, hipStreamNonBlocking, least) : hipStreamCreateWithFlags(&s, hipStreamNonBlocking);
        return e;
    };
    auto closeStream = [&] {
        if (s) (void)hipStreamDestroy(s);
        s = nullptr;
    };
    DeviceBuildOutcome outcome = DeviceBuildOutcome::HostBuild;
    if (tryDevice) {
        std::string why;
        hipError_t e = openStream(true);
        if (e == hipSuccess) e = deviceBuild(job, s, why);
        closeStream();
        outcome = deviceBuildOutcome(e == hipSuccess, isDeviceFault(e), !why.empty());
        if (outcome == DeviceBuildOutcome::Failed) job->error = std::string("device build: ") + hipGetErrorString(e);
        if (outcome == DeviceBuildOutcome::HostBuild) {
            job->bvh.release();
            job->bvh = DeviceBvh {};
            job->perm.release();
            job->roots[0] = job->roots[1] = job->roots[2] = -1;
            job->opaqueNodes = 0;
            job->gpuFallback = true;
        }
    }
    bool ok = outcome == DeviceBuildOutcome::Installed;
    job->gpu = ok;
    if (outcome == DeviceBuildOutcome::HostBuild) {
        (void)openStream(false);
        ok = hostBuild(job, s, threads);
        closeStream();
    }
    if (ok && job->coverWanted) {
        const auto tc = std::chrono::steady_clock::now();
        float L[3];
        sunRayDirection(job->coverDir, L);
        if (openStream(true) == hipSuccess && hipEventSynchronize(job->evSnap) == hipSuccess &&
            deviceBuildCoverMap(job->snap.as<GpuTriangle>(), job->snapRecords, job->coverFrame, L, cover::kDefaultBudget, s, job->coverGrid, job->coverBuf,
                                job->coverOk) != hipSuccess)
            job->coverOk = false;
        closeStream();
        job->coverMs = std::chrono::duration<float, std::milli>(std::chrono::steady_clock::now() - tc).count();
    }
    job->ms = std::chrono::duration<float, std::milli>(std::chrono::steady_clock::now() - t0).count();
    job->ok = ok;
    job->done.store(true, std::memory_order_release);
}

hipError_t sharedBegin(const SceneCall& c) { return c.shared ? hipDeviceSynchronize() : hipSuccess; }
hipError_t sharedEnd(const SceneCall& c, hipStream_t s) { return c.shared ? hipStreamSynchronize(s) : hipSuccess; }

hipError_t geometryChanged(SceneStore& st, hipStream_t s)
{
    ++st.geometrySeq;
    return hipEventRecord(st.evGeometry, s);
}

std::vector<int> instanceClasses(const SceneStore& st)
{
    std::vector<int> c(st.instHost.size());
    for (size_t i = 0; i < c.size(); ++i) c[i] = hit_mask_class(st.instHost[i].hit_mask);
    return c;
}

void setWorldArgs(SceneStore& st)
{
    st.args.nodes = st.world.nodes(st.world.buf);
    st.args.tris = st.world.tris(st.world.buf);
    st.args.tri_byte_offset = static_cast<uint32_t>(st.world.triOffset);
    st.args.instances = st.instances.as<GpuInstance>();
}

void setWorldRoots(SceneStore& st, const int32_t roots[3], uint32_t opaqueNodes)
{
    st.args.root_opaque = roots[0];
    st.args.root_masked = roots[1];
    st.args.root_blend = roots[2];
    st.args.opaque_nodes = opaqueNodes;
}

void setSunArgs(SceneStore& st)
{
    st.sunArgs.sun_nodes = st.sun.nodes(st.sun.buf);
    st.sunArgs.sun_tris = st.sun.tris(st.sun.buf);
    st.sunArgs.sun_root = 0;
}

hipError_t growBoxes(SceneStore& st, DeviceBvh& b, hipStream_t s)
{
    const size_t need = b.nodeCount * 6 * sizeof(float);
    if (b.boxes.bytes >= need) return hipSuccess;
    const hipError_t e = retireBuffer(st, b.boxes, s);
    return e == hipSuccess ? b.boxes.alloc(std::max<size_t>(16, need * 5 / 4)) : e;
}

hipError_t replaceBvh(SceneStore& st, DeviceBvh& cur, DeviceBvh& b, hipStream_t s)
{
    hipError_t e = retireBuffer(st, cur.buf, s);
    if (e == hipSuccess) e = retireBuffer(st, cur.order, s);
    if (e != hipSuccess) return e;
    b.boxes = cur.boxes;
    b.masks = cur.masks;
    b.masksValid = false;
    cur = std::move(b);
    b = DeviceBvh {};
    return hipSuccess;
}

int installSunBvh(ErrorSink* err, SceneStore& st, DeviceBvh& b, Bvh8BuildResult* host, const double* frame, const float* dir, hipStream_t s)
{
    ARK_HIP(replaceBvh(st, st.sun, b, s));
    ARK_HIP(growBoxes(st, st.sun, s));
    if (host) ARK_HIP(uploadBvh(host->nodes, host->tris, nullptr, st.sun));
    setSunArgs(st);
    for (int k = 0; k < 9; ++k) {
        st.sunArgs.sun_frame[k] = static_cast<float>(frame[k]);
        st.sunFrameD[k] = frame[k];
    }
    std::memcpy(st.sunDirBuilt, dir, sizeof(st.sunDirBuilt));
    return ARK_DDGI_OK;
}

hipError_t clearCoverMap(SceneStore& st, hipStream_t s)
{
    if (st.coverMap.buf.ptr) ++st.version;
    st.coverMap.valid = false;
    return retireBuffer(st, st.coverMap.buf, s);
}

void setCoverMap(SceneStore& st, DeviceBuffer& buf, const cover::Grid& grid, const float* dir, const double* frame, float ms)
{
// ... 97 lines not shown
    job.coverWanted = st.coverWanted && hasSun;
    if (job.coverWanted) {
        std::memcpy(job.coverDir, sunDir, sizeof(job.coverDir));
        double frame[3][3];
        sun_frame(sunDir, frame);
        std::memcpy(job.coverFrame, frame, sizeof(job.coverFrame));
    }
    job.t = std::thread(runRebuildJob, &job, st.device, std::max(1, st.buildThreads / 2), gpu);
    return ARK_DDGI_OK;
}

int sunStart(SceneStore& st, const SceneCall& c, hipStream_t s, bool gpu)
{
    auto job = std::make_unique<RebuildJob>();
    job->kind = RebuildJob::Sun;
    std::memcpy(job->dir, c.sunDir, sizeof(job->dir));
    double frame[3][3];
    sun_frame(job->dir, frame);
    std::memcpy(job->frame, frame, sizeof(job->frame));
    job->instances = static_cast<uint32_t>(st.instHost.size());
    job->sahPass = (c.flags & ARK_DDGI_FLAG_GPU_REBUILD_SAH) != 0;
    job->planPass = (c.flags & ARK_DDGI_FLAG_GPU_REBUILD_PLAN) != 0;
    if (const int rc = launchJob(st, c.err, *job, s, gpu, c.hasSun, c.sunDir)) return rc;
    st.sunJob = std::move(job);
    st.lastBackground = kBackgroundSun;
    return ARK_DDGI_OK;
}

int worldCollect(SceneStore& st, const SceneCall& c, hipStream_t s)
{
    ErrorSink* err = c.err;
    if (st.worldJob && st.worldJob->done.load(std::memory_order_acquire)) {
        std::unique_ptr<RebuildJob> job = std::move(st.worldJob);
        job->t.join();
        if (job->gpuFallback) st.bvhStats.bvh_gpu_fallbacks++;
        if (!job->ok) {
            st.worldRebuildFailed = true;
            st.bvhStats.bvh_rebuild_failures++;
            err->lastError = "background BVH rebuild failed: " + job->error;
            return ARK_DDGI_OK;
        }
        ARK_HIP(sharedBegin(c));
        DeviceBuffer tn;
        ARK_HIP(tn.alloc(std::max<size_t>(64, job->bvh.records * 64)));
        ARK_HIP(launch_gather_records(tn.as<float4>(), st.triNormals.as<float4>(), job->perm.as<uint32_t>(), job->bvh.records, s));
        ARK_HIP(retireBuffer(st, st.triNormals, s));
        st.triNormals = tn;
        job->bvh.inflateAbs = st.world.inflateAbs;
        ARK_HIP(replaceBvh(st, st.world, job->bvh, s));
        ARK_HIP(retireBuffer(st, job->perm, s));
        ARK_HIP(retireBuffer(st, job->snap, s));
        ARK_HIP(growBoxes(st, st.world, s));
        setWorldArgs(st);
        setWorldRoots(st, job->roots, job->opaqueNodes);
        st.args.tri_normals = st.triNormals.as<float4>();
        st.bvhMaxDepth = std::max(st.world.depth, st.sunArgs.sun_root >= 0 ? st.sun.depth : 0u);
        st.bvhStats.node_count = st.world.nodeCount;
        st.bvhStats.max_depth = st.bvhMaxDepth;
        st.bvhStats.max_leaf_size = job->maxLeaf;
        st.bvhStats.sah_cost = job->sah;
        st.bvhStats.node_bytes = st.world.nodeCount * sizeof(GpuBvh8Node);
        st.bvhStats.triangle_bytes = st.world.records * sizeof(GpuTriangle);
        st.bvhStats.bvh_rebuilds = ++st.worldRebuilds;
        ArkDdgiBvhStats& b = st.bvhStats;
        return finishInstall(st, c, *job, { st.worldGpuBuilt, st.refitsSinceBuild, b.bvh_installed_builder, b.bvh_gpu_rebuilds, b.bvh_built_refit_version, b.bvh_rebuild_ms }, s);
    }
    return ARK_DDGI_OK;
}

int worldStart(SceneStore& st, const SceneCall& c, hipStream_t s, bool gpu)
{
    auto job = std::make_unique<RebuildJob>();
    job->kind = RebuildJob::World;
    job->classOf = instanceClasses(st);
    job->sahPass = (c.flags & ARK_DDGI_FLAG_GPU_REBUILD_SAH) != 0;
    job->planPass = (c.flags & ARK_DDGI_FLAG_GPU_REBUILD_PLAN) != 0;
    if (const int rc = launchJob(st, c.err, *job, s, gpu, c.hasSun, c.sunDir)) return rc;
    st.worldJob = std::move(job);
    st.lastBackground = kBackgroundWorld;
    st.refitsSinceBuild = 0;
    return ARK_DDGI_OK;
}

int startRebuild(SceneStore& st, const SceneCall& c, hipStream_t s, bool sunOnly)
{
    RebuildState q;
    q.sunWanted = st.sunWanted;
    q.hasSun = c.hasSun;
    q.sunJobRunning = static_cast<bool>(st.sunJob);
    q.worldJobRunning = static_cast<bool>(st.worldJob);
    q.sunInstalled = st.sunArgs.sun_root >= 0 && sameDir(c.sunDir, st.sunDirBuilt);
    q.requestStable = st.sunReqStreak >= 2 && sameDir(st.sunReqDir, c.sunDir);
    q.sunFailedHere = st.sunFailed && st.sunFailedVersion == st.version && sameDir(st.sunFailedDir, c.sunDir);
    q.worldRebuildFailed = st.worldRebuildFailed;
    q.worldGpuBuilt = st.worldGpuBuilt;
    q.sunGpuBuilt = st.sunGpuBuilt && q.sunInstalled;
    q.refitsSinceBuild = st.refitsSinceBuild;
    q.sunRefitsSinceBuild = st.sunRefitsSinceBuild;
    q.flags = c.flags;
    q.lastBackground = st.lastBackground;
    q.sunOnly = sunOnly;
    switch (rebuildToStart(q)) {
    case RebuildStart::Sun: return sunStart(st, c, s, false);
    case RebuildStart::SunDevice: return sunStart(st, c, s, true);
    case RebuildStart::WorldHost: return worldStart(st, c, s, false);
    case RebuildStart::WorldDevice: return worldStart(st, c, s, true);
    case RebuildStart::None: break;
// ... 271 lines not shown
    if (sunThread.t.joinable()) sunThread.t.join();
    const auto ts0 = std::chrono::steady_clock::now();
    const int32_t sroot = 0;
    if (sunBuilt) {
        if (!sunOk) return err->fail(ARK_DDGI_E_DEVICE, "sun BVH2 leaf over %d triangles", kBvh8MaxLeafSize);
        if (!checkBvh8Structure(r.nodes, r.tris, &sroot, 1, why)) return err->fail(ARK_DDGI_E_DEVICE, "%s", why.c_str());
        const float* sd = s->directional_light.world_space_direction;
        const float dd = sd[0] * sd[0] + sd[1] * sd[1] + sd[2] * sd[2];
        const float isc = 1.0f / std::sqrt(dd);
        const float L[3] = { -(sd[0] * isc), -(sd[1] * isc), -(sd[2] * isc) };
        std::vector<float> origins;
        sun_sample_origins(w.tris, L, 4096u, origins);
        st->sunCostWorld = static_cast<float>(sun_shadow_cost(w.nodes, w.tris, w.roots, 3, nullptr, L, origins));
        st->sunCostLight = static_cast<float>(sun_shadow_cost(r.nodes, r.tris, &sroot, 1, sunIn.frame, L, origins));
    }
    st->sunArgs.sun_root = -1;
    if (sunBuilt && (sunBvh == 1 ||sun_bvh_pays(st->sunCostWorld, st->sunCostLight))) {
        DeviceBvh sb;
        std::vector<uint32_t> order;
        if (!bvhLevelOrder(r.nodes.data(), r.nodes.size(), &sroot, 1, order, sb.levelOffsets)) return err->fail(ARK_DDGI_E_DEVICE, "sun BVH: a node outside it");
        sb.depth = r.max_depth;
        sb.inflateAbs = sunIn.inflateAbs;
        sb.nodeCount = r.nodes.size();
        rc = upload(err, sb.order, order.data(), order.size());
        if (rc == 0) rc = installSunBvh(err, *st, sb, &r, &sunIn.frame[0][0], s->directional_light.world_space_direction, nullptr);
        sb.order.release();
        if (rc != 0) return rc;
    }
    sunBuildMs += std::chrono::duration<float, std::milli>(std::chrono::steady_clock::now() - ts0).count();
    std::vector<GpuTriangle>().swap(sunIn.world);
    if ((rc = upload(err, st->indices, s->indices, s->index_count)) != 0) return rc;
    if ((rc = upload(err, st->vertices, reinterpret_cast<const float*>(s->vertices), s->vertex_count * 9)) != 0) return rc;
    if ((rc = upload(err, st->positions, s->positions, s->vertex_count * 3)) != 0) return rc;
    st->instHost.assign(s->instances, s->instances + s->instance_count);
    st->xf[0].resize(s->instance_count);
    for (uint32_t ii = 0; ii < s->instance_count; ++ii) std::memcpy(st->xf[0][ii].data(), s->instances[ii].object_to_world, sizeof(float) * 12);
    st->xf[1] = st->xf[2] = st->xf[0];
    st->spare[0].slot = 1;
    st->spare[1].slot = 2;
    st->meshHost.assign(s->meshes, s->meshes + s->mesh_count);
    instanceObjectBoxes(s, opt.threads, st->instObjBox);
    if ((rc = upload(err, st->meshes, s->meshes, s->mesh_count)) != 0) return rc;
    if ((rc = upload(err, st->materials, s->materials, s->material_count)) != 0) return rc;
    if ((rc = upload(err, st->instances, ginst.data(), ginst.size())) != 0) return rc;
    if ((rc = upload(err, st->texInfos, infos.data(), infos.size())) != 0) return rc;
    if ((rc = upload(err, st->texels, texels.data(), texels.size())) != 0) return rc;
    {
        std::vector<float> tn;
        shadingRecords(s, w.tris, opt.threads, tn);
        if ((rc = upload(err, st->triNormals, tn.data(), tn.size())) != 0) return rc;
    }
    SceneArgs& sc = st->args;
    setWorldArgs(*st);
    setWorldRoots(*st, w.roots, w.opaqueNodes);
    sc.tri_normals = st->triNormals.as<float4>();
    sc.texture_count = static_cast<int32_t>(s->texture_count);
    sc.indices = st->indices.as<uint32_t>();
    sc.vertices = st->vertices.as<float>();
    sc.meshes = st->meshes.as<ArkRTTriangleMesh>();
    sc.materials = st->materials.as<ArkShaderMaterial>();
    sc.tex_infos = st->texInfos.as<GpuTextureInfo>();
    sc.texels = st->texels.as<float4>();
    sc.white_texture = static_cast<int32_t>(s->texture_count);
    sc.env_texture = (s->environment_texture >= 0 && static_cast<uint32_t>(s->environment_texture) < s->texture_count) ? s->environment_texture : sc.white_texture;
    sc.sun_root = -1;
    st->hasSunScene = s->has_directional_light ? 1 : 0;
    st->sunScene = s->directional_light;
    st->spotsScene = std::move(gspots);
    st->sunWanted = st->sun.nodeCount > 0;
    st->buildThreads = opt.threads;
    st->coverWanted = coverMap;
    if (coverMap && s->has_directional_light && st->world.records > 0) {
        const auto tc = std::chrono::steady_clock::now();
        double frame[3][3];
        sun_frame(s->directional_light.world_space_direction, frame);
        float L[3];
        sunRayDirection(s->directional_light.world_space_direction, L);
        cover::Grid grid {};
        DeviceBuffer buf;
        bool ok = false;
        ARK_HIP(deviceBuildCoverMap(st->world.tris(st->world.buf), st->world.records, &frame[0][0], L, cover::kDefaultBudget, nullptr, grid, buf, ok));
        if (ok) setCoverMap(*st, buf, grid, s->directional_light.world_space_direction, &frame[0][0], std::chrono::duration<float, std::milli>(std::chrono::steady_clock::now() - tc).count());
    }
    st->bvhMaxDepth = std::max(st->world.depth, st->sun.depth);
    const auto t1 = std::chrono::steady_clock::now();
    st->bvhStats.node_count = w.nodes.size();
    st->bvhStats.triangle_count = w.triangles;
    st->bvhStats.max_depth = st->bvhMaxDepth;
    st->bvhStats.max_leaf_size = w.maxLeaf;
    st->bvhStats.sah_cost = w.sah;
    st->bvhStats.build_ms = std::chrono::duration<float, std::milli>(t1 - t0).count();
    st->bvhStats.node_bytes = w.nodes.size() * sizeof(GpuBvh8Node);
    st->bvhStats.triangle_bytes = w.tris.size() * sizeof(GpuTriangle);
    st->bvhStats.sun_node_count = st->sun.nodeCount;
    st->bvhStats.sun_max_depth = st->sun.depth;
    st->bvhStats.sun_cost_world = st->sunCostWorld;
    st->bvhStats.sun_cost_light = st->sunCostLight;
    st->bvhStats.sun_build_ms = sunBuildMs;
    out = std::move(st);
    return ARK_DDGI_OK;
}

namespace {

int prepareRefit(ErrorSink* err, SceneStore& st)
{
    DeviceBvh& w = st.world;
// ... 226 lines not shown
```

arkoserenderer_amd/csrc/scene_store.h:

```cpp
#pragma once

#include <hip/hip_runtime.h>

#include <array>
#include <cstdarg>
#include <cstdint>
#include <cstdio>
#include <memory>
#include <string>
#include <vector>

#include "../../include/ark_ddgi.h"
#include "ddgi_kernels.h"
#include "device_bvh.h"
#include "scene_rebuild_policy.h"

namespace ark {

struct ErrorSink {
    std::string lastError;
    int fail(int code, const char* fmt, ...)
    {
        char buf[512];
        va_list ap;
// ... 41 lines not shown
        float buildMs = 0.0f;
    } coverMap;
    bool coverWanted = false;
    int32_t hasSunScene = 0;
    ArkDirectionalLight sunScene {};
    std::vector<GpuSpotLight> spotsScene;
    ArkDdgiBvhStats bvhStats {};
    uint32_t bvhMaxDepth = 0;
    uint32_t version = 0;
    DeviceBuffer refitInst;
    double sunFrameD[9] {};
    std::vector<RefitInstance> refitHost;
    static constexpr int kStageSlots = 8;
    void* stage[kStageSlots] {};
    size_t stageBytes[kStageSlots] {};
    hipEvent_t stageDone[kStageSlots] {};
    int stageNext = 0;
    std::vector<std::array<float, 6>> instObjBox;
    struct Spare {
        DeviceBuffer world, sun, instances;
        bool valid = false;
        int slot = 0;
    };
    Spare spare[2];
    bool refitFull = true;
    float inflCopy[3][2] {};
    int front = 0;
    std::vector<std::array<float, 12>> xf[3];
    bool sunWanted = false;
    int buildThreads = 16;
    std::unique_ptr<RebuildJob> sunJob;
    uint32_t sunRebuilds = 0;
    float sunReqDir[3] { 0, 0, 0 };
    uint32_t sunReqStreak = 0;
    bool sunFailed = false;
    float sunFailedDir[3] { 0, 0, 0 };
    uint32_t sunFailedVersion = 0;
    uint32_t sunFailures = 0;
    uint32_t refitsSinceBuild = 0, sunRefitsSinceBuild = 0;
    std::unique_ptr<RebuildJob> worldJob;
    uint32_t worldRebuilds = 0, refitCount = 0;
    bool worldRebuildFailed = false;
    bool worldGpuBuilt = false;
    bool sunGpuBuilt = false;
    uint8_t lastBackground = kBackgroundNone;
    std::vector<Retired> retired;
    hipStream_t refitStream = nullptr;
    hipEvent_t evFree[3] = {};
    bool freeValid[3] = { false, false, false };
    hipEvent_t evInstalled = nullptr;
    bool installValid = false;
    hipEvent_t evGeometry = nullptr;
    uint32_t geometrySeq = 0;
    SceneStore();
    SceneStore(const SceneStore&) = delete;
    SceneStore& operator=(const SceneStore&) = delete;
    ~SceneStore();
};

struct SceneCall {
    ErrorSink* err;
    uint32_t flags;
    bool hasSun;
    float sunDir[3];
    bool shared;
};

int buildScene(ErrorSink* err, const ArkDdgiScene* s, int device, int buildThreads, int sunBvh, bool coverMap, std::shared_ptr<SceneStore>& out);

int sceneMaintenance(SceneStore& st, const SceneCall& c, hipStream_t s);

int sceneSunStep(SceneStore& st, const SceneCall& c, hipStream_t s, bool mayEnqueue);
bool sunStepMayEnqueue(const SceneStore& st, const SceneCall& c);
bool sunJobPending(const SceneStore& st);

int sceneSetInstances(SceneStore& st, const SceneCall& c, const ArkRTInstance* instances, uint32_t count, hipStream_t s);

int sceneDigest(const SceneStore& st, ErrorSink* err, uint64_t* out);
int sceneWorldBvhCheck(const SceneStore& st, ErrorSink* err, uint64_t* out);
int sceneSunBvhCheck(const SceneStore& st, ErrorSink* err, uint64_t* out);
int sceneRefitReach(const SceneStore& st, ErrorSink* err, uint64_t* out);

GpuSpotLight gpuSpotLight(const ArkSpotLight& sl);

}
```

arkoserenderer_amd/ddgi.py:

```python
from __future__ import annotations

import ctypes as C
from dataclasses import dataclass

import numpy as np

from . import abi
from .scene import SceneData


@dataclass
class ProbeGrid:
    grid_dimensions: tuple
    probe_spacing: tuple
    offset_to_first: tuple

    def probe_count(self) -> int:
        x, y, z = self.grid_dimensions
        return int(x * y * z)

    @staticmethod
    def from_bounding_box(lo, hi):
        lo = np.asarray(lo, np.float32) - np.float32(1.0)
        hi = np.asarray(hi, np.float32) + np.float32(1.0)
        bounds = (hi - lo).astype(np.float32)
        largest = 0
        if bounds[1] > bounds[0] or bounds[2] > bounds[0]:
            largest = 1 if bounds[1] > bounds[2] else 2
        counts = np.array([16.0, 16.0, 16.0], np.float32)
        counts[largest] = 32.0
        spacing = (bounds / counts).astype(np.float32)
        return ProbeGrid(tuple(int(v) for v in counts), tuple(float(v) for v in spacing), tuple(float(v) for v in lo))


@dataclass
class DDGIConfig:
    rays_per_probe: int = 256
    hysteresis_irradiance: float = 0.93
    hysteresis_visibility: float = 0.93
    visibility_sharpness: float = 50.0
    probe_updates_per_frame: int = 2048
    compute_probe_offsets: bool = True
    apply_probe_offsets: bool = True
    use_scene_ambient: bool = True
    injected_ambient_lx: float = 100.0
    max_rays_per_probe: int = abi.ARK_DDGI_MAX_RAYS_PER_PROBE
    max_probe_updates: int = abi.ARK_DDGI_REFERENCE_MAX_PROBE_UPDATES
    clear_overflow_mode: int = abi.ARK_DDGI_CLEAR_OVERFLOW_INF
    sun_bvh: int = abi.ARK_DDGI_SUN_BVH_AUTO
    serial_frames: bool = False
    background_rebuild: bool = True
    gpu_rebuild: bool = False
    gpu_rebuild_sun: bool = False
    gpu_rebuild_sah: bool = False
    gpu_rebuild_plan: bool = False
    sun_cover_map: bool = True
    fused_sun_shade: bool = True
    build_threads: int = 0


@dataclass
class AppState:
    frame_index: int = 0
    delta_time: float = 1.0 / 60.0

    def is_first_frame(self) -> bool:
        return self.frame_index == 0


def _check(lib, ctx, rc, what):
    if rc != 0:
        msg = lib.ark_ddgi_last_error(ctx)
        raise abi.ArkDdgiError(rc, f"{what}: {msg.decode() if msg else ''}")


def desc_for(grid: ProbeGrid, z_far: float, config: DDGIConfig, device: int = 0, shard_rank: int = 0,
             shard_count: int = 1) -> abi.ArkDdgiDesc:
    d = abi.ArkDdgiDesc()
    d.struct_size = C.sizeof(abi.ArkDdgiDesc)
    for k in range(3):
        d.grid_dims[k] = int(grid.grid_dimensions[k])
        d.probe_spacing[k] = float(grid.probe_spacing[k])
        d.offset_to_first[k] = float(grid.offset_to_first[k])
    d.z_far = float(z_far)
    d.max_rays_per_probe = int(config.max_rays_per_probe)
    d.max_probe_updates = int(config.max_probe_updates)
    d.device = int(device)
    d.clear_overflow_mode = int(config.clear_overflow_mode)
    d.shard_rank = int(shard_rank)
    d.shard_count = int(shard_count)
    d.sun_bvh = int(config.sun_bvh)
    d.flags = (abi.ARK_DDGI_FLAG_SERIAL_FRAMES if config.serial_frames else 0) | (0 if config.background_rebuild else abi.ARK_DDGI_FLAG_NO_BACKGROUND_REBUILD)
    d.flags |= abi.ARK_DDGI_FLAG_GPU_REBUILD if config.gpu_rebuild else 0
    d.flags |= abi.ARK_DDGI_FLAG_GPU_REBUILD_SUN if config.gpu_rebuild_sun else 0
    d.flags |= abi.ARK_DDGI_FLAG_GPU_REBUILD_SAH if config.gpu_rebuild_sah else 0
    d.flags |= abi.ARK_DDGI_FLAG_GPU_REBUILD_PLAN if config.gpu_rebuild_plan else 0
    d.flags |= 0 if config.sun_cover_map else abi.ARK_DDGI_FLAG_NO_SUN_COVER_MAP
    d.flags |= 0 if config.fused_sun_shade else abi.ARK_DDGI_FLAG_NO_FUSED_SUN_SHADE
    d.build_threads = int(config.build_threads)
    return d


class DDGIContext:

    def __init__(self, grid: ProbeGrid, z_far: float, config: DDGIConfig | None = None, device: int = 0,
                 shard_rank: int = 0, shard_count: int = 1):
        self.lib = abi.load_library()
        self.grid = grid
        self.config = config or DDGIConfig()
        d = desc_for(grid, z_far, self.config, device, shard_rank, shard_count)
        self.desc = d
        h = C.c_void_p()
        rc = self.lib.ark_ddgi_create(C.byref(d), C.byref(h))
        if rc != 0:
            raise abi.ArkDdgiError(rc, "ark_ddgi_create")
        self.h = h
        self._scene = None

    def close(self):
        if getattr(self, "h", None):
            self.lib.ark_ddgi_destroy(self.h)
            self.h = None

    def __del__(self):
        self.close()

    def check(self, rc, what):
        _check(self.lib, self.h, rc, what)

    def last_error(self) -> str:
        m = self.lib.ark_ddgi_last_error(self.h)
        return m.decode() if m else ""

    def set_scene(self, scene: SceneData):
        s = scene.to_abi()
        self.check(self.lib.ark_ddgi_set_scene(self.h, C.byref(s)), "ark_ddgi_set_scene")
        self._scene = scene

    def set_lights(self, sun=None, spots=()):
        from .scene import lights_abi

        L, keep = lights_abi(sun, spots)
        self.check(self.lib.ark_ddgi_set_lights(self.h, C.byref(L)), "ark_ddgi_set_lights")
        del keep

    def set_instances(self, instances: np.ndarray):
        a = np.ascontiguousarray(instances)
        self.check(self.lib.ark_ddgi_set_instances(self.h, C.c_void_p(a.ctypes.data), int(a.size)), "ark_ddgi_set_instances")

    def set_instances_async(self, instances: np.ndarray, stream: int | None):
        a = np.ascontiguousarray(instances)
# ... 128 lines not shown
        d = abi.ArkComposeDesc()
        d.struct_size = C.sizeof(abi.ArkComposeDesc)
        d.width, d.height, d.flags = int(width), int(height), int(flags)
        for k in ("view_from_pixel", "view_from_world", "world_from_view"):
            m = np.ascontiguousarray(camera[k], np.float32).reshape(16)
            getattr(d, k)[:] = [float(v) for v in m]
        for name, _, _ in abi.COMPOSE_PLANES:
            ptr = planes.get(name)
            setattr(d, name, int(ptr) if ptr else None)
        d.out = int(out_ptr)
        self.check(self.lib.ark_ddgi_lighting_compose(self.h, C.byref(d), C.c_void_p(stream) if stream else None),
                   "ark_ddgi_lighting_compose")

    def rt_reflections(self, desc: abi.ArkReflectionsDesc, stream: int | None = None):
        desc.struct_size = C.sizeof(abi.ArkReflectionsDesc)
        self.check(self.lib.ark_ddgi_rt_reflections(self.h, C.byref(desc), C.c_void_p(stream) if stream else None), "ark_ddgi_rt_reflections")

    def probe_debug(self, visualisation: int, distance_scale: float, count: int, probes_ptr: int, dirs_ptr: int, out_ptr: int,
                    stream: int | None = None):
        d = abi.ArkProbeDebugDesc()
        d.struct_size = C.sizeof(abi.ArkProbeDebugDesc)
        d.visualisation, d.distance_scale, d.count = int(visualisation), float(distance_scale), int(count)
        d.probe_indices, d.directions, d.out = int(probes_ptr), int(dirs_ptr), int(out_ptr)
        self.check(self.lib.ark_ddgi_probe_debug(self.h, C.byref(d), C.c_void_p(stream) if stream else None), "ark_ddgi_probe_debug")

    def bvh_stats(self) -> abi.ArkDdgiBvhStats:
        s = abi.ArkDdgiBvhStats()
        self.check(self.lib.ark_ddgi_get_bvh_stats(self.h, C.byref(s)), "ark_ddgi_get_bvh_stats")
        return s

    def scene_digest(self) -> tuple:
        out = (C.c_uint64 * 4)()
        self.check(self.lib.ark_ddgi_debug_scene_digest(self.h, out), "ark_ddgi_debug_scene_digest")
        return tuple(int(v) for v in out)

    def world_bvh_check(self) -> dict:
        out = (C.c_uint64 * 8)()
        rc = self.lib.ark_ddgi_debug_world_bvh_check(self.h, out)
        if rc < 0:
            self.check(rc, "ark_ddgi_debug_world_bvh_check")
        return dict(zip(_BVH_CHECK_KEYS, (int(v) for v in out)))

    def sun_cover_counts(self, host_restatement: bool = True) -> dict:
        out = (C.c_uint64 * 12)()
        fn = self.lib.ark_ddgi_debug_sun_cover_counts if host_restatement else self.lib.ark_ddgi_debug_sun_cover_counts_device
        self.check(fn(self.h, out), "ark_ddgi_debug_sun_cover_counts")
        keys = ("occluded", "lit", "listed", "in_use", "nx", "ny", "bytes", "build_us", "host_occluded", "host_lit", "host_listed", "map_diff")
        return dict(zip(keys, (int(v) for v in out)))

    def shade_schedule(self) -> dict:
        out = (C.c_uint64 * 2)()
        self.check(self.lib.ark_ddgi_debug_shade_schedule(self.h, out), "ark_ddgi_debug_shade_schedule")
        return {"sun_only": bool(out[0]), "deferred": int(out[1])}

    def set_sun_only_small_windows(self, on: bool):
        self.check(self.lib.ark_ddgi_debug_set_sun_only_small_windows(self.h, int(on)), "ark_ddgi_debug_set_sun_only_small_windows")

    def sun_bvh_installed_check(self) -> dict:
        out = (C.c_uint64 * 8)()
        rc = self.lib.ark_ddgi_debug_sun_bvh_installed_check(self.h, out)
        if rc < 0:
            self.check(rc, "ark_ddgi_debug_sun_bvh_installed_check")
        r = dict(zip(_BVH_CHECK_KEYS, (int(v) for v in out)))
        r["installed"] = r["nodes"] > 0
        return r

    def refit_reach(self) -> dict:
        out = (C.c_uint64 * 4)()
        self.check(self.lib.ark_ddgi_debug_refit_reach(self.h, out), "ark_ddgi_debug_refit_reach")
        return dict(zip(("world_nodes", "world_reached", "sun_nodes", "sun_reached"), (int(v) for v in out)))


_BVH_CHECK_KEYS = ("nodes", "leaf_children", "max_depth", "violations", "records", "records_with_holes", "record_digest", "installed_builder")


def sun_lbvh_check(triangles, sun_dir, origins, tmax: float = 1e30, w_bits: int | None = None, sah: bool | None = None, plan: bool | None = None) -> tuple:
    lib = abi.load_library()
    tris = np.ascontiguousarray(triangles, dtype=np.float32).reshape(-1, 9)
    sd = np.ascontiguousarray(sun_dir, dtype=np.float32).reshape(3)
    org = np.ascontiguousarray(origins, dtype=np.float32).reshape(-1, 3)
    keys = ("rays", "occluded_brute", "occluded_bvh", "mismatches", "node_visits", "triangle_tests", "nodes", "max_stack_depth", "violations",
            "inflation_differs", "cost_lbvh", "cost_host", "leaf_children", "depth", "records_with_holes", "w_bits")
    if plan is not None:
        out = (C.c_uint64 * 19)()
        rc = lib.ark_ddgi_debug_sun_lbvh_check_plan(tris.ctypes.data, tris.shape[0], sd.ctypes.data, org.ctypes.data, org.shape[0], float(tmax),
                                                    -1 if w_bits is None else int(w_bits), 0 if sah is False else 1, 1 if plan else 0, out)
        keys = keys + ("treelets", "plan_root_cost", "small_internal")
    elif sah is None:
        out = (C.c_uint64 * 16)()
        rc = lib.ark_ddgi_debug_sun_lbvh_check_opts(tris.ctypes.data, tris.shape[0], sd.ctypes.data, org.ctypes.data, org.shape[0], float(tmax),
                                                    -1 if w_bits is None else int(w_bits), out)
    else:
        out = (C.c_uint64 * 17)()
        rc = lib.ark_ddgi_debug_sun_lbvh_check_sah(tris.ctypes.data, tris.shape[0], sd.ctypes.data, org.ctypes.data, org.shape[0], float(tmax),
                                                   -1 if w_bits is None else int(w_bits), 1 if sah else 0, out)
        keys = keys + ("treelets",)
    r = dict(zip(keys, (int(v) for v in out)))
    r["cost_lbvh"] /= 1e6
    r["cost_host"] /= 1e6
    return rc, r


def lbvh_check(triangles, criterion: int | None = None, sah: bool | None = None, plan: bool | None = None) -> tuple:
    lib = abi.load_library()
    tris = np.ascontiguousarray(triangles, dtype=np.float32).reshape(-1, 9)
    out = (C.c_uint64 * (11 if plan is not None else 8 if sah is None else 9))()
# ... 313 lines not shown
```

arkoserenderer_amd/host/apps/ddgi_headless.cpp:

```cpp
#include <sys/stat.h>

#include <algorithm>
#include <chrono>
#include <cstdio>
#include <cstdlib>
#include <cstring>
#include <ctime>
#include <memory>
#include <thread>
#include <string>
#include <vector>

#include "../../../include/ark_ddgi.h"
#include "../../../include/ark_scene.h"
#include "core/Logging.h"
#include "rendering/GpuScene.h"
#include "rendering/RenderPipeline.h"
#include "rendering/backend/hip/SlabExchange.h"
#include "rendering/nodes/DDGINode.h"

#include <hip/hip_runtime.h>

namespace {

// ... 204 lines not shown
            int32_t ies = -1;
            ok = rd(v, sizeof(v)) && rd(&ies, 4);
            ManagedSpotLight sl;
            for (int k = 0; k < 3; ++k) {
                sl.color[k] = v[k];
                sl.forward[k] = v[4 + k];
                sl.right[k] = v[7 + k];
                sl.up[k] = v[10 + k];
                sl.position[k] = v[13 + k];
            }
            sl.intensity = v[3];
            sl.outerConeAngle = v[16];
            sl.iesLut = ies;
            c.spots.push_back(sl);
        }
        uint32_t moved = 0;
        ok = ok && rd(&moved, 4);
        if (ok && moved) {
            c.transforms.resize(static_cast<size_t>(instances) * 12);
            ok = rd(c.transforms.data(), c.transforms.size() * 4);
        }
        out.push_back(std::move(c));
    }
    std::fclose(f);
    return ok;
}

bool dump(ArkDdgiCtx* ctx, int which, const std::string& path)
{
    uint64_t bytes = 0;
    if (ark_ddgi_resource_size(ctx, which, &bytes) != 0) return false;
    std::vector<uint8_t> buf(bytes);
    if (ark_ddgi_read(ctx, which, buf.data(), bytes) != 0) return false;
    FILE* f = std::fopen(path.c_str(), "wb");
    if (!f) return false;
    bool ok = std::fwrite(buf.data(), 1, bytes, f) == bytes;
    std::fclose(f);
    return ok;
}

}

int main(int argc, char** argv)
{
    std::string scenePath, out = "ddgi";
    uint64_t soupTris = 0;
    ProbeGrid grid;
    int rays = 64, updates = 512, frames = 4, device = 0, offsets = 1, rebuildAt = -1;
    int shards = 1, world = 1, rank = 0;
    std::string ncclIdPath, ncclNonce;
    double exchangeTimeout = 0.0;
    std::string saveStatePath, loadStatePath, frameScriptPath;
    int firstFrame = 0, gpuRebuild = 0;
    bool deadlineTest = false;
    const std::time_t startedAt = std::time(nullptr);
    float zFar = 10000.0f, exposure = 1.0f, env = 1.0f, ambient = 0.0f;
    for (int i = 1; i < argc; ++i) {
        std::string a = argv[i];
        auto next = [&]() -> const char* {
            if (i + 1 >= argc) ARKOSE_LOG(Fatal, "missing value for %s", a.c_str());
            return argv[++i];
        };
        if (a == "--scene") scenePath = next();
        else if (a == "--soup") soupTris = std::strtoull(next(), nullptr, 10);
        else if (a == "--grid") for (int k = 0; k < 3; ++k) grid.gridDimensions[k] = std::atoi(next());
        else if (a == "--spacing") for (int k = 0; k < 3; ++k) grid.probeSpacing[k] = std::strtof(next(), nullptr);
        else if (a == "--origin") for (int k = 0; k < 3; ++k) grid.offsetToFirst[k] = std::strtof(next(), nullptr);
        else if (a == "--rays") rays = std::atoi(next());
        else if (a == "--updates") updates = std::atoi(next());
        else if (a == "--frames") frames = std::atoi(next());
        else if (a == "--zfar") zFar = std::strtof(next(), nullptr);
        else if (a == "--exposure") exposure = std::strtof(next(), nullptr);
        else if (a == "--env") env = std::strtof(next(), nullptr);
        else if (a == "--ambient") ambient = std::strtof(next(), nullptr);
        else if (a == "--offsets") offsets = std::atoi(next());
        else if (a == "--rebuild-at") rebuildAt = std::atoi(next());
        else if (a == "--device") device = std::atoi(next());
        else if (a == "--out") out = next();
        else if (a == "--shards") shards = std::atoi(next());
        else if (a == "--world") world = std::atoi(next());
        else if (a == "--rank") rank = std::atoi(next());
        else if (a == "--nccl-id") ncclIdPath = next();
        else if (a == "--nccl-nonce") ncclNonce = next();
        else if (a == "--exchange-timeout") exchangeTimeout = std::strtod(next(), nullptr);
        else if (a == "--exchange-deadline-test") deadlineTest = true;
        else if (a == "--save-state") saveStatePath = next();
        else if (a == "--load-state") loadStatePath = next();
        else if (a == "--first-frame") firstFrame = std::atoi(next());
        else if (a == "--frame-script") frameScriptPath = next();
        else if (a == "--gpu-rebuild") gpuRebuild = std::atoi(next());
        else ARKOSE_LOG(Fatal, "unknown argument %s", a.c_str());
    }
    SceneFile file;
    ArkSoupScene* soup = nullptr;
    const ArkDdgiScene* rt = nullptr;
    if (!scenePath.empty()) {
        if (!loadScene(scenePath.c_str(), file)) ARKOSE_LOG(Fatal, "cannot read scene %s", scenePath.c_str());
        rt = &file.view;
    } else {
        ArkSoupParams sp;
        ark_soup_default_params(&sp);
        sp.triangle_count = soupTris ? soupTris : 1000000;
        if (ark_soup_generate(&sp, &soup) != 0) ARKOSE_LOG(Fatal, "soup generation failed");
        rt = ark_soup_scene_view(soup);
    }

    HipBackend backend(device);
    GpuScene scene(backend);
    populate(scene, *rt);
    if (scene.rtScene().instance_count != rt->instance_count) ARKOSE_LOG(Fatal, "GpuScene adapter dropped instances");
    scene.scene().setProbeGrid(grid);
    scene.scene().setAmbientIlluminance(ambient);
    scene.scene().setEnvironmentBrightness(env);
    scene.camera().setFarClipPlane(zFar);
    scene.camera().setExposure(exposure);

    if (world > 1 && ncclNonce.empty())
        ARKOSE_LOG(Fatal, "--world %d needs --nccl-nonce S (one value per launch, the same on every rank): a rendezvous file's age "
                          "cannot tell this launch's id from a stale one", world);
    if (shards < 1 || world < 1 || rank < 0 || rank >= world || (shards > 1 && world > 1) || (world > 1 && ncclIdPath.empty()))
        ARKOSE_LOG(Fatal, "bad sharding arguments (--shards %d, --world %d --rank %d)", shards, world, rank);
    const bool rccl = !ncclIdPath.empty();
    const int ranksHere = shards;
    const int slabCount = rccl ? world : shards;

    auto makePipeline = [&](int shardRank) {
        auto pipeline = std::make_unique<RenderPipeline>(&scene);
        DDGINode& node = pipeline->addNode<DDGINode>();
        node.setRaysPerProbe(rays);
        node.setProbeUpdatesPerFrame(updates);
        node.setComputeProbeOffsets(offsets != 0);
        node.setMaxProbeUpdates(updates);
        node.setGpuRebuild((gpuRebuild & 1) != 0);
        node.setGpuRebuildSun((gpuRebuild & 2) != 0);
        node.setGpuRebuildSah((gpuRebuild & 4) != 0);
        node.setGpuRebuildPlan((gpuRebuild & 8) != 0);
        if (slabCount > 1) node.setShard(shardRank, slabCount);
        return pipeline;
    };
    auto nodeOf = [](RenderPipeline& p) {
        RenderPipelineNode* n = nullptr;
        p.forEachNodeInResolvedOrder([&](RenderPipelineNode& node, const RenderPipelineNode::ExecuteCallback&) { n = &node; });
        return static_cast<DDGINode*>(n);
    };
    std::vector<std::unique_ptr<RenderPipeline>> pipelines;
    std::vector<std::unique_ptr<Registry>> registries;
    for (int r = 0; r < ranksHere; ++r) {
        pipelines.push_back(makePipeline(rccl ? rank : r));
        registries.push_back(std::make_unique<Registry>(backend, nullptr));
        pipelines.back()->constructAll(*registries.back());
    }
    std::unique_ptr<SlabExchange> exchange;
    if (slabCount > 1 || rccl) {
        std::string err;
        if (rccl) {
            SlabBands bands;
            if (!SlabBands::fromContext(nodeOf(*pipelines[0])->context(), rank, world, bands, err)) ARKOSE_LOG(Fatal, "%s", err.c_str());
            std::vector<uint8_t> id;
            if (!shareUniqueId(ncclIdPath, rank, ncclNonce, startedAt, id)) ARKOSE_LOG(Fatal, "cannot share the ncclUniqueId through %s", ncclIdPath.c_str());
            auto ex = std::make_unique<RcclSlabExchange>(device, rank, world, id.data(), bands, deadlineTest ? 0.2 : exchangeTimeout);
            if (!ex->ok()) ARKOSE_LOG(Fatal, "RCCL: %s", ex->error().c_str());
            if (deadlineTest) {
                if (world != 1) ARKOSE_LOG(Fatal, "--exchange-deadline-test runs with --world 1");
                RcclSlabExchange* rx = ex.get();
                rx->watchdog().setFailureHandler([rx](const std::string& why) {
                    std::printf("ddgi_headless: watchdog fired: %s\n", why.c_str());
                    (void)hipDeviceSynchronize();
                    ExchangeWatchdog::abortAndExit(rx->comm(), why);
                });
                int khz = 0;
                if (hipDeviceGetAttribute(&khz, hipDeviceAttributeWallClockRate, device) != hipSuccess || khz <= 0) khz = 100000;
                hipLaunchKernelGGL(k_stall, dim3(1), dim3(1), 0, static_cast<hipStream_t>(rx->stream()), static_cast<uint64_t>(khz) * 1500u);
                if (hipGetLastError() != hipSuccess) ARKOSE_LOG(Fatal, "stall kernel launch failed");
            }
            exchange = std::move(ex);
        } else {
            std::vector<SlabBands> all(ranksHere);
            for (int r = 0; r < ranksHere; ++r)
                if (!SlabBands::fromContext(nodeOf(*pipelines[r])->context(), r, ranksHere, all[r], err)) ARKOSE_LOG(Fatal, "%s", err.c_str());
            exchange = std::make_unique<DeviceCopySlabExchange>(std::move(all));
        }
        for (auto& p : pipelines) nodeOf(*p)->setSlabExchange(exchange.get());
    }
    if (!loadStatePath.empty()) {
        if (ranksHere != 1 || exchange) ARKOSE_LOG(Fatal, "--load-state is for unsharded runs");
        FILE* fh = std::fopen(loadStatePath.c_str(), "rb");
        if (!fh) ARKOSE_LOG(Fatal, "cannot read %s", loadStatePath.c_str());
        std::vector<uint8_t> blob;
        uint8_t buf[1 << 16];
// ... 83 lines not shown
```

arkoserenderer_amd/host/rendering/nodes/DDGINode.cpp:

```cpp
#include "DDGINode.h"

#include <hip/hip_runtime.h>

#include <algorithm>
#include <cstring>
#include <vector>

#include "core/Logging.h"

struct DDGIProbeGridData {
    int gridDimensions[4];
    float probeSpacing[4];
    float offsetToFirst[4];
};

DDGINode::~DDGINode()
{
    if (m_updateDone) (void)hipEventDestroy(static_cast<hipEvent_t>(m_updateDone));
}

bool DDGINode::saveState(std::vector<uint8_t>& out) const
{
    uint64_t bytes = 0;
    if (!m_ctx || ark_ddgi_state_size(m_ctx, &bytes) != ARK_DDGI_OK) return false;
    out.resize(bytes);
    if (int rc = ark_ddgi_save_state(m_ctx, out.data(), bytes); rc != ARK_DDGI_OK) {
        ARKOSE_LOG(Error, "DDGINode: ark_ddgi_save_state failed (%d): %s", rc, ark_ddgi_last_error(m_ctx));
        return false;
    }
    return true;
}

bool DDGINode::loadState(const std::vector<uint8_t>& blob)
{
    if (!m_ctx) return false;
    if (int rc = ark_ddgi_load_state(m_ctx, blob.data(), blob.size()); rc != ARK_DDGI_OK) {
        ARKOSE_LOG(Error, "DDGINode: ark_ddgi_load_state failed (%d): %s", rc, ark_ddgi_last_error(m_ctx));
        return false;
    }
    uint32_t next = 0;
    if (ark_ddgi_get_next_probe_index(m_ctx, &next) != ARK_DDGI_OK) return false;
    m_probeUpdateIdx = static_cast<int>(next);
    return true;
}

RenderPipelineNode::ExecuteCallback DDGINode::construct(GpuScene& scene, Registry& reg)
{
    if (!scene.scene().hasProbeGrid()) {
        ARKOSE_LOG(Error, "DDGINode is used but no probe grid is available, will no-op");
        return RenderPipelineNode::NullExecuteCallback;
    }

    const ProbeGrid& probeGrid = scene.scene().probeGrid();
    DDGIProbeGridData probeGridData {};
    for (int k = 0; k < 3; ++k) {
        probeGridData.gridDimensions[k] = probeGrid.gridDimensions[k];
        probeGridData.probeSpacing[k] = probeGrid.probeSpacing[k];
        probeGridData.offsetToFirst[k] = probeGrid.offsetToFirst[k];
    }
    Buffer& probeGridDataBuffer = reg.createBufferForData(probeGridData, Buffer::Usage::ConstantBuffer);

    ArkDdgiDesc desc {};
    desc.struct_size = sizeof(ArkDdgiDesc);
    for (int k = 0; k < 3; ++k) {
        desc.grid_dims[k] = probeGrid.gridDimensions[k];
        desc.probe_spacing[k] = probeGrid.probeSpacing[k];
        desc.offset_to_first[k] = probeGrid.offsetToFirst[k];
    }
    desc.z_far = scene.camera().farClipPlane();
    desc.max_rays_per_probe = MaxNumProbeSamples;
    desc.max_probe_updates = std::min(m_maxProbeUpdates, probeGrid.probeCount());
    desc.device = scene.backend().device();
    desc.clear_overflow_mode = ARK_DDGI_CLEAR_OVERFLOW_INF;
    desc.shard_rank = m_shardRank;
    desc.shard_count = m_shardCount;
    desc.flags = (m_gpuRebuild ? ARK_DDGI_FLAG_GPU_REBUILD : 0u) | (m_gpuRebuildSun ? ARK_DDGI_FLAG_GPU_REBUILD_SUN : 0u) |
                 (m_gpuRebuildSah ? ARK_DDGI_FLAG_GPU_REBUILD_SAH : 0u) | (m_gpuRebuildPlan ? ARK_DDGI_FLAG_GPU_REBUILD_PLAN : 0u);
    auto created = reg.createOrReuseDdgiContext("ddgi", desc);
    ArkDdgiCtx* ctx = created.first;
    if (!ctx) {
        ARKOSE_LOG(Error, "DDGINode: could not create the DDGI context, will no-op");
        return RenderPipelineNode::NullExecuteCallback;
    }
    m_ctx = ctx;
    if (created.second == Registry::ReuseMode::Reused) {
        uint64_t bytes = 0;
        ark_ddgi_resource_size(ctx, ARK_DDGI_PROBE_OFFSETS, &bytes);
        std::vector<uint8_t> zeros(bytes, 0);
        ark_ddgi_write(ctx, ARK_DDGI_PROBE_OFFSETS, zeros.data(), bytes);
    }
    if (int rc = ark_ddgi_set_scene(ctx, &scene.rtScene()); rc != ARK_DDGI_OK) {
        ARKOSE_LOG(Error, "DDGINode: ark_ddgi_set_scene failed (%d): %s", rc, ark_ddgi_last_error(ctx));
        return RenderPipelineNode::NullExecuteCallback;
    }
    m_instanceVersion = scene.instanceVersion();

    ArkDdgiDeviceViews views {};
    ark_ddgi_get_device_views(ctx, &views);
    Buffer& probeOffsetBuffer = reg.wrapBuffer(views.probe_offsets, views.probe_offsets_bytes, Buffer::Usage::StorageBuffer);
    probeOffsetBuffer.setName("DDGIProbeOffsetBuffer");
    probeOffsetBuffer.setStride(16);
    Texture& irradiance = reg.wrapTexture("ddgi-irradiance", views.irradiance_atlas, views.irradiance_width, views.irradiance_height, Texture::Format::RGBA16F);
    Texture& visibility = reg.wrapTexture("ddgi-visibility", views.visibility_atlas, views.visibility_width, views.visibility_height, Texture::Format::RG16F);
    BindingSet& ddgiSamplingBindingSet = reg.createBindingSet({ ShaderBinding::constantBuffer(probeGridDataBuffer),
                                                                ShaderBinding::storageBuffer(probeOffsetBuffer),
                                                                ShaderBinding::sampledTexture(irradiance),
                                                                ShaderBinding::sampledTexture(visibility) });
    reg.publish("DDGISamplingSet", ddgiSamplingBindingSet);

    return [&, ctx](const AppState& appState, CommandList& cmdList, UploadBuffer&) {
        const ProbeGrid& grid = scene.scene().probeGrid();
        const uint32_t frameIdx = appState.frameIndex();
        const uint32_t raysPerProbe = static_cast<uint32_t>(m_raysPerProbeInt);
        const float ambientLx = m_useSceneAmbient ? scene.scene().ambientIlluminance() : m_injectedAmbientLx;
        const uint32_t probeUpdatesThisFrame = static_cast<uint32_t>(std::min(m_probeUpdatesPerFrame, grid.probeCount()));
        const uint32_t firstProbeIdx = static_cast<uint32_t>(m_probeUpdateIdx);

        ArkDdgiFrameParams p {};
        p.struct_size = sizeof(ArkDdgiFrameParams);
        p.frame_index = frameIdx;
        p.first_probe_index = firstProbeIdx;
        p.probe_updates = probeUpdatesThisFrame;
        p.rays_per_probe = raysPerProbe;
        p.hysteresis_irradiance = appState.isFirstFrame() ? 0.0f : m_hysteresisIrradiance;
        p.hysteresis_visibility = appState.isFirstFrame() ? 0.0f : m_hysteresisVisibility;
        p.visibility_sharpness = m_visibilitySharpness;
        p.ambient_amount = ambientLx * scene.lightPreExposure();
        p.environment_multiplier = scene.preExposedEnvironmentBrightnessFactor();
        p.delta_time = appState.deltaTime();
        p.update_offsets = (m_computeProbeOffsets && m_applyProbeOffsets) ? 1 : 0;
// ... 32 lines not shown
```

arkoserenderer_amd/host/rendering/nodes/DDGINode.h:

```cpp
#pragma once

#include "../GpuScene.h"
#include "../RenderPipelineNode.h"
#include "../backend/hip/SlabExchange.h"

#include <cstdint>
#include <vector>

class DDGINode final : public RenderPipelineNode {
public:
    std::string name() const override { return "DDGI"; }
    void drawGui() override {}

    ExecuteCallback construct(GpuScene&, Registry&) override;

    void setRaysPerProbe(int r) { m_raysPerProbeInt = r; }
    void setProbeUpdatesPerFrame(int n) { m_probeUpdatesPerFrame = n; }
    void setHysteresis(float irradiance, float visibility) { m_hysteresisIrradiance = irradiance; m_hysteresisVisibility = visibility; }
    void setVisibilitySharpness(float s) { m_visibilitySharpness = s; }
    void setComputeProbeOffsets(bool c) { m_computeProbeOffsets = c; }
    void setApplyProbeOffsets(bool a) { m_applyProbeOffsets = a; }
    void setMaxProbeUpdates(int n) { m_maxProbeUpdates = n; }
    void setShard(int rank, int count) { m_shardRank = rank; m_shardCount = count; }
    void setGpuRebuild(bool on) { m_gpuRebuild = on; }
    void setGpuRebuildSun(bool on) { m_gpuRebuildSun = on; }
    void setGpuRebuildSah(bool on) { m_gpuRebuildSah = on; }
    void setGpuRebuildPlan(bool on) { m_gpuRebuildPlan = on; }
    void setSlabExchange(SlabExchange* exchange) { m_exchange = exchange; }
    void* pendingExchange() const { return m_exchangePending; }
    ArkDdgiCtx* context() const { return m_ctx; }
    int probeUpdateIdx() const { return m_probeUpdateIdx; }
    void setProbeUpdateIdx(int idx) { m_probeUpdateIdx = idx; }
    bool saveState(std::vector<uint8_t>& out) const;
    bool loadState(const std::vector<uint8_t>& blob);

    static constexpr int MaxNumProbeSamples { ARK_DDGI_MAX_RAYS_PER_PROBE };
    static constexpr int MaxNumProbeUpdates { ARK_DDGI_REFERENCE_MAX_PROBE_UPDATES };

private:
    int m_raysPerProbeInt = 256;
    float m_hysteresisIrradiance { 0.93f };
    float m_hysteresisVisibility { 0.93f };

    float m_visibilitySharpness { 50.0f };

    int m_probeUpdatesPerFrame { 2048 };
    int m_probeUpdateIdx { 0 };

    bool m_computeProbeOffsets { true };
    bool m_applyProbeOffsets { true };

    bool m_useSceneAmbient { true };
    float m_injectedAmbientLx { 100.0f };

    int m_maxProbeUpdates { MaxNumProbeUpdates };
    int m_shardRank { 0 };
    int m_shardCount { 1 };
    bool m_gpuRebuild { false };
    bool m_gpuRebuildSun { false };
    bool m_gpuRebuildSah { false };
    bool m_gpuRebuildPlan { false };
    ArkDdgiCtx* m_ctx { nullptr };
    uint32_t m_instanceVersion { 0 };
    SlabExchange* m_exchange { nullptr };
    void* m_updateDone { nullptr };
    void* m_exchangePending { nullptr };
public:
    ~DDGINode() override;
};
```

include/ark_ddgi.h:

```cpp
#ifndef ARK_DDGI_H
#define ARK_DDGI_H

#include <stddef.h>
#include <stdint.h>

#ifdef __cplusplus
extern "C" {
#endif

#define ARK_DDGI_ABI_VERSION 1

#define ARK_DDGI_IRRADIANCE_RES 8
#define ARK_DDGI_VISIBILITY_RES 16
#define ARK_DDGI_ATLAS_PADDING 1
#define ARK_DDGI_MAX_RAYS_PER_PROBE 512
#define ARK_DDGI_REFERENCE_MAX_PROBE_UPDATES 4096

#define ARK_RT_HIT_MASK_OPAQUE 0x01u
#define ARK_RT_HIT_MASK_MASKED 0x02u
#define ARK_RT_HIT_MASK_BLEND 0x04u

#define ARK_BLEND_MODE_OPAQUE 1
#define ARK_BLEND_MODE_MASKED 2
#define ARK_BLEND_MODE_TRANSLUCENT 3
// ... 15 lines not shown
    ARK_DDGI_SURFELS = 2,
    ARK_DDGI_PROBE_OFFSETS = 3
};

enum {
    ARK_DDGI_CLEAR_OVERFLOW_INF = 0,
    ARK_DDGI_CLEAR_OVERFLOW_MAX_FINITE = 1
};

enum {
    ARK_TEX_RGBA8_UNORM = 0,
    ARK_TEX_RGBA8_SRGB = 1,
    ARK_TEX_R32F = 2,
    ARK_TEX_RGBA32F = 3
};

enum {
    ARK_WRAP_REPEAT = 0,
    ARK_WRAP_CLAMP_TO_EDGE = 1,
    ARK_WRAP_MIRRORED_REPEAT = 2,
    ARK_WRAP_PER_AXIS = 0x100
};
#define ARK_WRAP_AXES(s, t) (ARK_WRAP_PER_AXIS | ((s) & 0xf) | (((t) & 0xf) << 4))

typedef struct ArkDdgiDesc {
    uint32_t struct_size;
    int32_t grid_dims[3];
    float probe_spacing[3];
    float offset_to_first[3];
    float z_far;
    int32_t max_rays_per_probe;
    int32_t max_probe_updates;
    int32_t device;
    int32_t clear_overflow_mode;
    int32_t shard_rank;
    int32_t shard_count;
    int32_t sun_bvh;
    uint32_t flags;
    int32_t build_threads;
    int32_t reserved[1];
} ArkDdgiDesc;

#define ARK_DDGI_SUN_BVH_AUTO 0
#define ARK_DDGI_SUN_BVH_WORLD 1
#define ARK_DDGI_SUN_BVH_LIGHT_SPACE 2
#define ARK_DDGI_FLAG_SERIAL_FRAMES 0x1u
#define ARK_DDGI_FLAG_NO_BACKGROUND_REBUILD 0x2u
#define ARK_DDGI_FLAG_GPU_REBUILD 0x4u
#define ARK_DDGI_FLAG_GPU_REBUILD_SUN 0x8u
#define ARK_DDGI_FLAG_GPU_REBUILD_SAH 0x10u
#define ARK_DDGI_FLAG_NO_SUN_COVER_MAP 0x20u
#define ARK_DDGI_FLAG_NO_FUSED_SUN_SHADE 0x40u
#define ARK_DDGI_FLAG_GPU_REBUILD_PLAN 0x80u

typedef struct ArkRTVertex {
    float tex_coord[2];
    float normal[3];
    float tangent[4];
} ArkRTVertex;

typedef struct ArkRTTriangleMesh {
    int32_t first_vertex;
    int32_t first_index;
    int32_t material_index;
} ArkRTTriangleMesh;

typedef struct ArkShaderMaterial {
    int32_t base_color;
    int32_t normal_map;
    int32_t metallic_roughness;
    int32_t emissive;
    int32_t occlusion;
    int32_t bent_normal_map;
    float clearcoat;
    float clearcoat_roughness;
    int32_t blend_mode;
    float mask_cutoff;
    float metallic_factor;
    float roughness_factor;
    float emissive_factor[3];
    int32_t brdf;
    float dielectric_reflectance;
    float _unused[3];
    float color_tint[4];
} ArkShaderMaterial;

typedef struct ArkTexture {
    int32_t width;
    int32_t height;
    int32_t format;
    int32_t wrap;
    const void* data;
} ArkTexture;

typedef struct ArkRTInstance {
    float object_to_world[12];
    uint32_t rt_mesh_index;
    uint32_t triangle_count;
    uint32_t hit_mask;
    uint32_t _pad;
} ArkRTInstance;

typedef struct ArkDirectionalLight {
    float color[3];
    float world_space_direction[3];
} ArkDirectionalLight;
// ... 257 lines not shown
```

include/ark_ddgi_debug.h:

```cpp
#ifndef ARK_DDGI_DEBUG_H
#define ARK_DDGI_DEBUG_H

#include <stdint.h>

#ifdef __cplusplus
extern "C" {
#endif

#define ARK_DDGI_DEBUG_HITS 100

#define ARK_DDGI_DEBUG_RAY_STEPS 101

int ark_ddgi_debug_fmath(int device, int op, const float* x, const float* y, float* out, uint64_t n);

int ark_ddgi_debug_fmath_host(int op, const float* x, const float* y, float* out, uint64_t n);

int ark_ddgi_debug_struct_sizes(uint32_t* out, int n);

int ark_ddgi_debug_bvh8_check(const float* triangles, uint64_t n, uint64_t* out);
int ark_ddgi_debug_bvh8_check_opts(const float* triangles, uint64_t n, int sah_optimal, float tri_cost, uint64_t* out);


int ark_ddgi_debug_sun_bvh_check(const float* triangles, uint64_t n, const float* sun_dir, const float* origins, uint64_t n_rays, float tmax,
                                 uint64_t* out);

int ark_ddgi_debug_sun_choice(const float* triangles, uint64_t n, const float* sun_dir, uint32_t n_samples, double* out);

int ark_ddgi_debug_scene_digest(struct ArkDdgiCtx* ctx, uint64_t* out);

int ark_ddgi_debug_lbvh_check(const float* triangles, uint64_t n, uint64_t* out);
int ark_ddgi_debug_lbvh_check_opts(const float* triangles, uint64_t n, int criterion, uint64_t* out);
int ark_ddgi_debug_lbvh_check_sah(const float* triangles, uint64_t n, int criterion, int sah, uint64_t* out);
int ark_ddgi_debug_lbvh_check_plan(const float* triangles, uint64_t n, int criterion, int sah, int plan, uint64_t* out);

int ark_ddgi_debug_lbvh_device_parity(int device, const void* records, uint64_t n_records, const int32_t* class_of, uint32_t n_instances,
                                      const float* sun_dir, int w_bits, uint64_t* out);
int ark_ddgi_debug_lbvh_device_parity_sah(int device, const void* records, uint64_t n_records, const int32_t* class_of, uint32_t n_instances,
                                          const float* sun_dir, int w_bits, int sah, uint64_t* out);
int ark_ddgi_debug_lbvh_device_parity_plan(int device, const void* records, uint64_t n_records, const int32_t* class_of, uint32_t n_instances,
                                           const float* sun_dir, int w_bits, int sah, int plan, uint64_t* out);

int ark_ddgi_debug_bvh8_compare_selftest(const float* triangles, uint64_t n, const float* sun_dir, uint64_t seed, uint64_t* out);

int ark_ddgi_debug_world_bvh_check(struct ArkDdgiCtx* ctx, uint64_t* out);

int ark_ddgi_debug_sun_lbvh_check(const float* triangles, uint64_t n, const float* sun_dir, const float* origins, uint64_t n_rays, float tmax,
                                  uint64_t* out);
int ark_ddgi_debug_sun_lbvh_check_opts(const float* triangles, uint64_t n, const float* sun_dir, const float* origins, uint64_t n_rays, float tmax,
                                       int w_bits, uint64_t* out);
int ark_ddgi_debug_sun_lbvh_check_sah(const float* triangles, uint64_t n, const float* sun_dir, const float* origins, uint64_t n_rays, float tmax,
                                      int w_bits, int sah, uint64_t* out);
int ark_ddgi_debug_sun_lbvh_check_plan(const float* triangles, uint64_t n, const float* sun_dir, const float* origins, uint64_t n_rays, float tmax,
                                       int w_bits, int sah, int plan, uint64_t* out);

int ark_ddgi_debug_sun_bvh_installed_check(struct ArkDdgiCtx* ctx, uint64_t* out);

int ark_ddgi_debug_refit_reach(struct ArkDdgiCtx* ctx, uint64_t* out);

int ark_ddgi_debug_cover_map_check(const float* triangles, uint64_t n, const float* sun_dir, const float* origins, uint64_t n_rays, float tmax,
                                   uint64_t budget_bytes, uint64_t* out);

int ark_ddgi_debug_cover_map_device(int device, const float* triangles, uint64_t n, const float* sun_dir, uint64_t budget_bytes, uint64_t* out);

int ark_ddgi_debug_sun_cover_counts(struct ArkDdgiCtx* ctx, uint64_t* out);
int ark_ddgi_debug_sun_cover_counts_device(struct ArkDdgiCtx* ctx, uint64_t* out);

int ark_ddgi_debug_shade_schedule(struct ArkDdgiCtx* ctx, uint64_t* out);
int ark_ddgi_debug_set_sun_only_small_windows(struct ArkDdgiCtx* ctx, int enabled);

#ifdef __cplusplus
}
#endif

#endif
```

Measured before the change: 3079 Mrays/s.

## Seed probe rays with cached per-direction hit triangles to shrink tmax early

Adds a per-probe octahedral cache (16x16 texels) that stores the triangle last hit by a probe ray in each direction bin. At staging time each probe ray looks up its bin and passes the candidate triangle into the traversal state, so an early intersection test can tighten tmax before BVH descent and prune nodes. Hits from the opaque pass write back into the cache. The cache is invalidated on topology changes. The cost is an extra gather per staged ray, scattered writes per hit, and an extra pool word.

```diff
diff --git a/arkoserenderer_amd/abi.py b/arkoserenderer_amd/abi.py
--- a/arkoserenderer_amd/abi.py
+++ b/arkoserenderer_amd/abi.py
@@ -51,6 +51,7 @@
 ARK_DDGI_FLAG_GPU_REBUILD_PLAN = 0x80
 ARK_DDGI_FLAG_NO_SUN_COVER_MAP = 0x20
 ARK_DDGI_FLAG_NO_FUSED_SUN_SHADE = 0x40
+ARK_DDGI_FLAG_NO_RAY_SEEDS = 0x100
 
 ARK_TEX_RGBA8_UNORM = 0
 ARK_TEX_RGBA8_SRGB = 1
@@ -522,6 +523,10 @@
     "ark_ddgi_debug_sun_cover_counts_device": (C.c_int, [C.c_void_p, C.POINTER(C.c_uint64)]),
     "ark_ddgi_debug_shade_schedule": (C.c_int, [C.c_void_p, C.POINTER(C.c_uint64)]),
     "ark_ddgi_debug_set_sun_only_small_windows": (C.c_int, [C.c_void_p, C.c_int]),
+    "ark_ddgi_debug_seed_texel": (C.c_uint32, [C.c_float, C.c_float, C.c_float]),
+    "ark_ddgi_debug_seed_candidate_ok": (C.c_int, [C.c_uint32, C.c_uint32, C.c_uint32]),
+    "ark_ddgi_debug_seed_info": (C.c_int, [C.c_void_p, C.POINTER(C.c_uint64)]),
+    "ark_ddgi_debug_seed_fill": (C.c_int, [C.c_void_p, C.c_int, C.c_uint64]),
 }
 
 _lib = None
diff --git a/arkoserenderer_amd/csrc/ark_ddgi.cpp b/arkoserenderer_amd/csrc/ark_ddgi.cpp
--- a/arkoserenderer_amd/csrc/ark_ddgi.cpp
+++ b/arkoserenderer_amd/csrc/ark_ddgi.cpp
@@ -103,6 +103,9 @@
     DeviceBuffer irr, vis, offsets;
     DeviceBuffer slots, slotOrder, fib, fibOrder, order, hits, surfels, spill, rayCounter, counters, shadeWork, reflWork;
     DeviceBuffer raySteps;
+    DeviceBuffer seeds;
+    bool seedStale = true;
+    uint32_t seedTopologySeen = 0;
     std::vector<uint32_t> orderHost;
     uint32_t orderR = 0;
     uint32_t lightCount = 0;
@@ -342,6 +345,7 @@
 int adoptScene(ArkDdgiCtx* ctx, std::shared_ptr<SceneStore> st)
 {
     ctx->geometrySeen = st->geometrySeq;
+    ctx->seedStale = true;
     ctx->hasSun = st->hasSunScene;
     for (int k = 0; k < 3; ++k) {
         ctx->sunColor[k] = st->sunScene.color[k];
@@ -381,7 +385,7 @@
     ctx->Kmax = desc->max_probe_updates > 0 ? desc->max_probe_updates : ARK_DDGI_REFERENCE_MAX_PROBE_UPDATES;
     const int shards = desc->shard_count > 0 ? desc->shard_count : 1;
     if (ctx->Rmax > ARK_DDGI_MAX_RAYS_PER_PROBE || ctx->Z % shards != 0 || desc->shard_rank < 0 || desc->shard_rank >= shards ||
-        desc->sun_bvh < ARK_DDGI_SUN_BVH_AUTO || desc->sun_bvh > ARK_DDGI_SUN_BVH_LIGHT_SPACE || (desc->flags & ~(ARK_DDGI_FLAG_SERIAL_FRAMES | ARK_DDGI_FLAG_NO_BACKGROUND_REBUILD | ARK_DDGI_FLAG_GPU_REBUILD | ARK_DDGI_FLAG_GPU_REBUILD_SUN | ARK_DDGI_FLAG_GPU_REBUILD_SAH | ARK_DDGI_FLAG_GPU_REBUILD_PLAN | ARK_DDGI_FLAG_NO_SUN_COVER_MAP | ARK_DDGI_FLAG_NO_FUSED_SUN_SHADE)) ||
+        desc->sun_bvh < ARK_DDGI_SUN_BVH_AUTO || desc->sun_bvh > ARK_DDGI_SUN_BVH_LIGHT_SPACE || (desc->flags & ~(ARK_DDGI_FLAG_SERIAL_FRAMES | ARK_DDGI_FLAG_NO_BACKGROUND_REBUILD | ARK_DDGI_FLAG_GPU_REBUILD | ARK_DDGI_FLAG_GPU_REBUILD_SUN | ARK_DDGI_FLAG_GPU_REBUILD_SAH | ARK_DDGI_FLAG_GPU_REBUILD_PLAN | ARK_DDGI_FLAG_NO_SUN_COVER_MAP | ARK_DDGI_FLAG_NO_FUSED_SUN_SHADE | ARK_DDGI_FLAG_NO_RAY_SEEDS)) ||
         desc->build_threads < 0) {
         delete ctx;
         return ARK_DDGI_E_INVALID_ARGUMENT;
@@ -435,6 +439,9 @@
     if ((e = ctx->surfels.alloc(K * R * 8)) != hipSuccess) return bad(e, "alloc surfels");
     if ((e = ctx->rayCounter.alloc(2 * kRayCounterWords * 4)) != hipSuccess) return bad(e, "alloc counter");
     if ((e = ctx->counters.alloc(10 * sizeof(unsigned long long))) != hipSuccess) return bad(e, "alloc counters");
+    if (!(desc->flags & ARK_DDGI_FLAG_NO_RAY_SEEDS)) {
+        if ((e = ctx->seeds.alloc(static_cast<size_t>(ctx->N) * seed::kProbeWords * 4)) != hipSuccess) return bad(e, "alloc seed cache");
+    }
     if ((e = ctx->seqWords.alloc(128 * 4)) != hipSuccess) return bad(e, "alloc sequence words");
     if ((e = hipMemset(ctx->seqWords.ptr, 0, ctx->seqWords.bytes)) != hipSuccess) return bad(e, "clear sequence words");
     {
@@ -472,7 +479,7 @@
     (void)hipSetDevice(ctx->device);
     (void)hipDeviceSynchronize();
     for (DeviceBuffer* b : { &ctx->irr, &ctx->vis, &ctx->offsets, &ctx->slots, &ctx->slotOrder, &ctx->fib, &ctx->fibOrder, &ctx->order, &ctx->hits, &ctx->surfels, &ctx->spill, &ctx->rayCounter, &ctx->seqWords, &ctx->shadeWork, &ctx->reflWork,
-                             &ctx->raySteps, &ctx->counters, &ctx->lights, &ctx->bakeTri, &ctx->bakeBary, &ctx->bakeOut, &ctx->bakePixels, &ctx->bakeCounters })
+                             &ctx->raySteps, &ctx->seeds, &ctx->counters, &ctx->lights, &ctx->bakeTri, &ctx->bakeBary, &ctx->bakeOut, &ctx->bakePixels, &ctx->bakeCounters })
         b->release();
     ctx->sceneStore.reset();
     for (auto& ev : ctx->ev)
@@ -715,6 +722,58 @@
     ARK_HIP(hipMemcpy(&n, ctx->lastDeferredCount, sizeof(n), hipMemcpyDeviceToHost));
     out[0] = 1;
     out[1] = n;
+    return ARK_DDGI_OK;
+}
+
+uint32_t ark_ddgi_debug_seed_texel(float x, float y, float z) { return seed::texelOf(x, y, z); }
+int ark_ddgi_debug_seed_candidate_ok(uint32_t word, uint32_t first, uint32_t end) { return seed::candidateOk(word, first, end) ? 1 : 0; }
+
+int ark_ddgi_debug_seed_info(ArkDdgiCtx* ctx, uint64_t* out)
+{
+    if (!ctx || !out) return ARK_DDGI_E_INVALID_ARGUMENT;
+    out[0] = ctx->seeds.ptr ? 1u : 0u;
+    out[1] = seed::kTexels;
+    out[2] = ctx->hasScene ? ctx->sceneStore->args.opaque_tri_first : 0u;
+    out[3] = ctx->hasScene ? ctx->sceneStore->args.opaque_tri_end : 0u;
+    out[4] = 0;
+    if (ctx->seeds.ptr && ctx->countersPending) {
+        uint32_t n = 0;
+        ARK_HIP(hipSetDevice(ctx->device));
+        ARK_HIP(hipDeviceSynchronize());
+        ARK_HIP(hipMemcpy(&n, ctx->counters.as<uint32_t>() + ctx->counters.bytes / 4u - 4u, sizeof(n), hipMemcpyDeviceToHost));
+        out[4] = n;
+    }
+    return ARK_DDGI_OK;
+}
+
+int ark_ddgi_debug_seed_fill(ArkDdgiCtx* ctx, int mode, uint64_t value)
+{
+    if (!ctx || mode < 0 || mode > 2) return ARK_DDGI_E_INVALID_ARGUMENT;
+    if (!ctx->hasScene) return ctx->fail(ARK_DDGI_E_NO_SCENE, "seed fill before ark_ddgi_set_scene");
+    if (!ctx->seeds.ptr) return ctx->fail(ARK_DDGI_E_INVALID_ARGUMENT, "the context keeps no seed cache (ARK_DDGI_FLAG_NO_RAY_SEEDS)");
+    const uint32_t first = ctx->sceneStore->args.opaque_tri_first, end = ctx->sceneStore->args.opaque_tri_end;
+    std::vector<uint32_t> words(ctx->seeds.bytes / 4, seed::kNone);
+    if (mode != 0 && end > first) {
+        uint64_t x = value * 0x9e3779b97f4a7c15ull + 0x632be59bd9b4e019ull;
+        for (uint32_t& w : words) {
+            if (mode == 2) {
+                w = static_cast<uint32_t>(value);
+            } else {
+                x += 0x9e3779b97f4a7c15ull;
+                uint64_t z = x;
+                z = (z ^ (z >> 30)) * 0xbf58476d1ce4e5b9ull;
+                z = (z ^ (z >> 27)) * 0x94d049bb133111ebull;
+                z ^= z >> 31;
+                w = first + static_cast<uint32_t>(z % (end - first));
+            }
+            if (!seed::candidateOk(w, first, end)) return ctx->fail(ARK_DDGI_E_INVALID_ARGUMENT, "seed fill: record %u outside the opaque class [%u, %u)", w, first, end);
+        }
+    }
+    ARK_HIP(hipSetDevice(ctx->device));
+    ARK_HIP(hipDeviceSynchronize());
+    ARK_HIP(hipMemcpy(ctx->seeds.ptr, words.data(), ctx->seeds.bytes, hipMemcpyHostToDevice));
+    ctx->seedStale = false;
+    ctx->seedTopologySeen = ctx->sceneStore->worldTopologySeq;
     return ARK_DDGI_OK;
 }
 
@@ -963,6 +1022,9 @@
     f.ray_counter = ctx->rayCounter.as<uint32_t>() + b * kRayCounterWords;
     f.counters = ctx->counters.as<unsigned long long>();
     f.ray_steps = count ? ctx->raySteps.as<uint16_t>() : nullptr;
+    f.seed_cache = ctx->seeds.as<uint32_t>();
+    f.seed_offsets_write = f.seed_cache && f.update_offsets && ctx->scene.root_masked < 0 ? 1u : 0u;
+    f.seed_counts = count && f.seed_cache ? ctx->counters.as<uint32_t>() + ctx->counters.bytes / 4u - 4u : nullptr;
     f.cover_counts = count ? ctx->counters.as<uint32_t>() + ctx->counters.bytes / 4u - 3u : nullptr;
     ctx->coverCountsValid = count;
     {
@@ -991,6 +1053,11 @@
     if (ctx->geometrySeen != ctx->sceneStore->geometrySeq) {
         ARK_HIP(hipStreamWaitEvent(ts, ctx->sceneStore->evGeometry, 0));
         ctx->geometrySeen = ctx->sceneStore->geometrySeq;
+    }
+    if (f.seed_cache && (ctx->seedStale || ctx->seedTopologySeen != ctx->sceneStore->worldTopologySeq)) {
+        ARK_HIP(launch_fill_u32(ctx->seeds.ptr, ctx->seeds.bytes / 4, seed::kNone, ts));
+        ctx->seedStale = false;
+        ctx->seedTopologySeen = ctx->sceneStore->worldTopologySeq;
     }
     if (count) ARK_HIP(hipMemsetAsync(ctx->counters.ptr, 0, ctx->counters.bytes, s));
     if (timing) ARK_HIP(hipEventRecord(ctx->ev[0], s));
diff --git a/arkoserenderer_amd/csrc/bvh_builder.cpp b/arkoserenderer_amd/csrc/bvh_builder.cpp
--- a/arkoserenderer_amd/csrc/bvh_builder.cpp
+++ b/arkoserenderer_amd/csrc/bvh_builder.cpp
@@ -1195,6 +1195,7 @@
         Bvh8BuildResult r = collapse_bvh8(r2, static_cast<uint32_t>(out.nodes.size()), static_cast<uint32_t>(out.tris.size()), copt);
         out.roots[c] = static_cast<int32_t>(out.nodes.size());
         if (c == 0) out.opaqueNodes = static_cast<uint32_t>(r.nodes.size());
+        if (c == 0) out.opaqueRecords = static_cast<uint32_t>(r.tris.size());
         out.depth = std::max(out.depth, r.max_depth);
         out.triangles += r.triangles;
         out.nodes.insert(out.nodes.end(), r.nodes.begin(), r.nodes.end());
diff --git a/arkoserenderer_amd/csrc/bvh_builder.h b/arkoserenderer_amd/csrc/bvh_builder.h
--- a/arkoserenderer_amd/csrc/bvh_builder.h
+++ b/arkoserenderer_amd/csrc/bvh_builder.h
@@ -64,6 +64,7 @@
     std::vector<GpuTriangle> tris;
     int32_t roots[3] = { -1, -1, -1 };
     uint32_t opaqueNodes = 0, depth = 0, maxLeaf = 0;
+    uint32_t opaqueRecords = 0;
     uint64_t triangles = 0;
     float sah = 0.0f;
     float inflateAbs = 0.0f;
diff --git a/arkoserenderer_amd/csrc/ddgi_kernels.h b/arkoserenderer_amd/csrc/ddgi_kernels.h
--- a/arkoserenderer_amd/csrc/ddgi_kernels.h
+++ b/arkoserenderer_amd/csrc/ddgi_kernels.h
@@ -6,6 +6,7 @@
 #include "../../include/ark_ddgi.h"
 #include "ddgi_types.h"
 #include "lbvh_build.h"
+#include "seed_cache.h"
 #include "sun_cover_map.h"
 
 namespace ark {
@@ -116,6 +117,7 @@
     int32_t root_masked;
     int32_t root_blend;
     uint32_t opaque_nodes;
+    uint32_t opaque_tri_first, opaque_tri_end;
     int32_t texture_count;
     const uint32_t* indices;
     const float* vertices;
@@ -195,6 +197,9 @@
     unsigned long long* counters;
     uint32_t* cover_counts;
     uint16_t* ray_steps;
+    uint32_t* seed_cache;
+    uint32_t seed_offsets_write;
+    uint32_t* seed_counts;
     const float4* ray_list;
     const uint32_t* list_count;
     const uint32_t* abort_word;
diff --git a/arkoserenderer_amd/csrc/ddgi_kernels.hip b/arkoserenderer_amd/csrc/ddgi_kernels.hip
--- a/arkoserenderer_amd/csrc/ddgi_kernels.hip
+++ b/arkoserenderer_amd/csrc/ddgi_kernels.hip
@@ -725,16 +725,18 @@
 struct PoolRec {
     V3 o, d;
     uint32_t a;
+    uint32_t c;
 };
 
 struct ProbeRays {
     static constexpr bool kMaskedPass = true;
+    static constexpr bool kSeeds = true;
     static constexpr float kTmin = 0.0001f;
     __device__ static void grab(const FrameArgs& f, uint32_t home, uint32_t lane, uint32_t& tried, uint32_t& b, uint32_t& e, uint32_t chunk)
     {
         grabRaysWave(f, f.ray_counter, home, lane, tried, b, e, chunk);
     }
-    __device__ static PoolRec stage(const FrameArgs& f, uint32_t r)
+    __device__ static PoolRec stage(const SceneArgs& sc, const FrameArgs& f, uint32_t r)
     {
         const uint32_t qp = r / f.R;
         const uint32_t slot = slotAt(f, qp);
@@ -744,6 +746,11 @@
         rec.o = { ps.pos[0], ps.pos[1], ps.pos[2] };
         rec.d = rotate(v3(fv.x, fv.y, fv.z), v3(ps.axis[0], ps.axis[1], ps.axis[2]), ps.angle_sin, ps.angle_cos);
         rec.a = slot * f.R + __float_as_uint(fv.w);
+        rec.c = seed::kNone;
+        if (f.seed_cache) {
+            const uint32_t w = f.seed_cache[static_cast<size_t>(ps.probe_index) * seed::kProbeWords + seed::texelOf(rec.d.x, rec.d.y, rec.d.z)];
+            if (seed::candidateOk(w, sc.opaque_tri_first, sc.opaque_tri_end)) rec.c = w;
+        }
         return rec;
     }
     __device__ static void take(const FrameArgs& f, uint32_t r, uint32_t recA, uint32_t& ray, float& tmax)
@@ -755,18 +762,20 @@
 
 struct ListRays {
     static constexpr bool kMaskedPass = false;
+    static constexpr bool kSeeds = false;
     static constexpr float kTmin = 0.01f;
     __device__ static void grab(const FrameArgs& f, uint32_t home, uint32_t lane, uint32_t& tried, uint32_t& b, uint32_t& e, uint32_t chunk)
     {
         grabItemsWave(f.ray_counter, *f.list_count, home, lane, tried, b, e, chunk);
     }
-    __device__ static PoolRec stage(const FrameArgs& f, uint32_t r)
+    __device__ static PoolRec stage(const SceneArgs&, const FrameArgs& f, uint32_t r)
     {
         const float4 a = f.ray_list[2u * r], b = f.ray_list[2u * r + 1u];
         PoolRec rec;
         rec.o = { a.x, a.y, a.z };
         rec.d = { b.x, b.y, b.z };
         rec.a = __float_as_uint(a.w);
+        rec.c = seed::kNone;
         return rec;
     }
     __device__ static void take(const FrameArgs& f, uint32_t r, uint32_t recA, uint32_t& ray, float& tmax)
@@ -776,7 +785,7 @@
     }
 };
 
-template<bool COUNT, int WPE, class Src = ProbeRays, int SLOTS = 64>
+template<bool COUNT, int WPE, class Src = ProbeRays, int SLOTS = 64, bool SEEDW = false>
 __global__ void __launch_bounds__(kTraceBlock) __attribute__((amdgpu_waves_per_eu(WPE))) k_trace(SceneArgs sc, FrameArgs f)
 {
     if (frameAborted(f.abort_word)) return;
@@ -793,6 +802,7 @@
     const uint32_t chunk = min(f.grab_chunk, static_cast<uint32_t>(SLOTS));
     const float tmin = Src::kTmin;
     uint32_t cNodes = 0, cTris = 0, cHits = 0, cIter = 0, rSteps = 0;
+    uint32_t cSeedHits = 0, seedTri = seed::kNone;
 
     uint32_t poolNext = 0, poolEnd = 0;
     uint32_t poolBase = 0;
@@ -810,7 +820,14 @@
     float opaqueT = 0.0f;
     auto done = [&]() { return travDoneDual(ts, nBits, st); };
     bool pending = false;
+    auto seedWrite = [&]() {
+        if (Src::kSeeds && SEEDW && h.tri != kNoHit) {
+            const uint32_t probe = f.slots[ray / f.R].probe_index;
+            f.seed_cache[static_cast<size_t>(probe) * seed::kProbeWords + seed::texelOf(d.x, d.y, d.z)] = h.tri;
+        }
+    };
     auto storeHit = [&]() {
+        if (pass == 0) seedWrite();
         GpuHit out;
         if (h.tri == kNoHit) {
             out.t = __builtin_bit_cast(float, 0x7f800000u);
@@ -840,12 +857,13 @@
             const uint32_t avail = poolEnd - poolNext;
             uint32_t fb = 0, fe = 0;
             if (avail < n) Src::grab(f, home, lane, tried, fb, fe, chunk);
-            uint32_t r = kNoHit, recA = 0;
+            uint32_t r = kNoHit, recA = 0, recC = seed::kNone;
             auto readRec = [&](uint32_t slot) {
                 const uint4 lo = pool[slot], hi = pool[SLOTS + slot];
                 o = { __uint_as_float(lo.x), __uint_as_float(lo.y), __uint_as_float(lo.z) };
                 d = { __uint_as_float(lo.w), __uint_as_float(hi.x), __uint_as_float(hi.y) };
                 recA = hi.z;
+                recC = hi.w;
             };
             if (!active && rank < avail) {
                 r = poolNext + rank;
@@ -854,9 +872,9 @@
             if (fb < fe) {
                 __builtin_amdgcn_fence(__ATOMIC_SEQ_CST, "wavefront");
                 if (lane < fe - fb) {
-                    const PoolRec s = Src::stage(f, fb + lane);
+                    const PoolRec s = Src::stage(sc, f, fb + lane);
                     pool[lane] = make_uint4(__float_as_uint(s.o.x), __float_as_uint(s.o.y), __float_as_uint(s.o.z), __float_as_uint(s.d.x));
-                    pool[SLOTS + lane] = make_uint4(__float_as_uint(s.d.y), __float_as_uint(s.d.z), s.a, 0u);
+                    pool[SLOTS + lane] = make_uint4(__float_as_uint(s.d.y), __float_as_uint(s.d.z), s.a, s.c);
                 }
                 __builtin_amdgcn_fence(__ATOMIC_SEQ_CST, "wavefront");
                 poolBase = __builtin_amdgcn_readfirstlane(fb);
@@ -875,7 +893,8 @@
                 pass = 0;
                 st.depth = 0;
                 nBits = 0;
-                ts = TravState { static_cast<uint32_t>(sc.root_opaque), sc.root_opaque >= 0 ? rootGroupBits() : 0u, 0u, 0u };
+                ts = TravState { static_cast<uint32_t>(sc.root_opaque), sc.root_opaque >= 0 ? rootGroupBits() : 0u, recC, recC != seed::kNone ? 1u : 0u };
+                if (COUNT) seedTri = recC;
             }
             if (avail < n) {
                 if (fb >= fe) {
@@ -895,6 +914,10 @@
             rSteps += active ? 1u : 0u;
         }
         if (active) travStepDual<kTraceBlock, false, true>(sc, nc, ts, nBase, nBits, st, o, d, idir, oct, tmin, h, pass, cNodes, cTris);
+        if (COUNT && active && seedTri != seed::kNone) {
+            cSeedHits += h.tri == seedTri ? 1u : 0u;
+            seedTri = seed::kNone;
+        }
         if (active && done() && (!Src::kMaskedPass || sc.root_masked < 0) && !exhausted) {
             active = false;
             pending = true;
@@ -903,6 +926,7 @@
             if (Src::kMaskedPass && pass == 0) {
                 opaqueT = (h.tri != kNoHit) ? (h.backface ? -h.t : h.t) : f.z_far;
                 if (sc.root_masked >= 0 && opaqueT >= tmin) {
+                    seedWrite();
                     pass = 1;
                     finished = false;
                     ts = TravState { static_cast<uint32_t>(sc.root_masked), rootGroupBits(), 0u, 0u };
@@ -930,6 +954,7 @@
         atomicAdd(&f.counters[1], static_cast<unsigned long long>(cTris));
         atomicAdd(&f.counters[2], static_cast<unsigned long long>(cHits));
         if (lane == 0) atomicAdd(&f.counters[7], static_cast<unsigned long long>(cIter));
+        if (f.seed_counts) atomicAdd(&f.seed_counts[0], cSeedHits);
     }
 }
 
@@ -2096,8 +2121,14 @@
 hipError_t launch_trace(const SceneArgs& sc, const FrameArgs& f, uint32_t blocks, bool count, hipStream_t s)
 {
     void* args[] = { const_cast<SceneArgs*>(&sc), const_cast<FrameArgs*>(&f) };
+    const bool small = !count && f.grab_chunk <= 32u;
     const void* fn = kernel_trace_ptr(count);
-    if (!count && f.grab_chunk <= 32u) fn = reinterpret_cast<const void*>(&dev::k_trace<false, kTraceWpe, dev::ProbeRays, 32>);
+    if (small) fn = reinterpret_cast<const void*>(&dev::k_trace<false, kTraceWpe, dev::ProbeRays, 32>);
+    if (f.seed_cache && !f.seed_offsets_write) {
+        fn = count ? reinterpret_cast<const void*>(&dev::k_trace<true, 1, dev::ProbeRays, 64, true>)
+             : small ? reinterpret_cast<const void*>(&dev::k_trace<false, kTraceWpe, dev::ProbeRays, 32, true>)
+                     : reinterpret_cast<const void*>(&dev::k_trace<false, kTraceWpe, dev::ProbeRays, 64, true>);
+    }
     return hipLaunchKernel(fn, dim3(blocks), dim3(kTraceBlock), args, 0, s);
 }
 
diff --git a/arkoserenderer_amd/csrc/ddgi_update.hip b/arkoserenderer_amd/csrc/ddgi_update.hip
--- a/arkoserenderer_amd/csrc/ddgi_update.hip
+++ b/arkoserenderer_amd/csrc/ddgi_update.hip
@@ -358,6 +358,8 @@
             const uint32_t cls = (a > 0.0f && a < maxOffset) ? 1u : (a < 0.0f ? 2u : 0u);
             const GpuProbeSlot& ps = f.slots[slot0 + p];
             const V3 d = rotate(v3(fb[k].x, fb[k].y, fb[k].z), v3(ps.axis[0], ps.axis[1], ps.axis[2]), ps.angle_sin, ps.angle_cos);
+            if (f.seed_offsets_write && h[k].tri != kNoHit)
+                f.seed_cache[static_cast<size_t>(ps.probe_index) * seed::kProbeWords + seed::texelOf(d.x, d.y, d.z)] = h[k].tri;
             float* v = valL + p * stride + 6u * s;
             v[0] = cls == 1u ? d.x : 0.0f;
             v[1] = cls == 1u ? d.y : 0.0f;
diff --git a/arkoserenderer_amd/csrc/lbvh_device_build.cpp b/arkoserenderer_amd/csrc/lbvh_device_build.cpp
--- a/arkoserenderer_amd/csrc/lbvh_device_build.cpp
+++ b/arkoserenderer_amd/csrc/lbvh_device_build.cpp
@@ -262,6 +262,7 @@
         }
         nodeTotal = a.levelBase;
         if (c == 0) g.opaqueNodes = nodeTotal;
+        if (c == 0) g.opaqueRecords = counters[kLbvhRecords];
     }
     const uint32_t outRecords = counters[kLbvhRecords];
     if (!(DeviceBvh::bytesFor(nodeTotal, outRecords) < (1ull << 32))) {
diff --git a/arkoserenderer_amd/csrc/lbvh_device_build.h b/arkoserenderer_amd/csrc/lbvh_device_build.h
--- a/arkoserenderer_amd/csrc/lbvh_device_build.h
+++ b/arkoserenderer_amd/csrc/lbvh_device_build.h
@@ -28,6 +28,7 @@
     LbvhGpuTrace* trace = nullptr;
     int32_t roots[3] { -1, -1, -1 };
     uint32_t opaqueNodes = 0, prims = 0;
+    uint32_t opaqueRecords = 0;
     float inflateAbs = 0.0f;
     std::vector<uint32_t> order;
 };
diff --git a/arkoserenderer_amd/csrc/scene_store.cpp b/arkoserenderer_amd/csrc/scene_store.cpp
--- a/arkoserenderer_amd/csrc/scene_store.cpp
+++ b/arkoserenderer_amd/csrc/scene_store.cpp
@@ -36,7 +36,7 @@
     std::vector<int> classOf;
     DeviceBuffer perm;
     int32_t roots[3] { -1, -1, -1 };
-    uint32_t opaqueNodes = 0, maxLeaf = 0;
+    uint32_t opaqueNodes = 0, opaqueRecords = 0, maxLeaf = 0;
     float sah = 0.0f;
     std::string error;
     float dir[3] {};
@@ -354,6 +354,7 @@
     }
     std::copy(w.roots, w.roots + 3, job->roots);
     job->opaqueNodes = w.opaqueNodes;
+    job->opaqueRecords = w.opaqueRecords;
     job->maxLeaf = w.maxLeaf;
     job->sah = w.sah;
     job->bvh.depth = w.depth;
@@ -437,6 +438,7 @@
     if (world) {
         std::copy(g.roots, g.roots + 3, job->roots);
         job->opaqueNodes = g.opaqueNodes;
+        job->opaqueRecords = g.opaqueRecords;
         job->maxLeaf = std::min<uint32_t>(g.prims, static_cast<uint32_t>(kBvh8MaxLeafSize));
         job->sah = 0.0f;
     } else {
@@ -473,7 +475,7 @@
             job->bvh = DeviceBvh {};
             job->perm.release();
             job->roots[0] = job->roots[1] = job->roots[2] = -1;
-            job->opaqueNodes = 0;
+            job->opaqueNodes = job->opaqueRecords = 0;
             job->gpuFallback = true;
         }
     }
@@ -524,12 +526,15 @@
     st.args.instances = st.instances.as<GpuInstance>();
 }
 
-void setWorldRoots(SceneStore& st, const int32_t roots[3], uint32_t opaqueNodes)
+void setWorldRoots(SceneStore& st, const int32_t roots[3], uint32_t opaqueNodes, uint32_t opaqueRecords)
 {
     st.args.root_opaque = roots[0];
     st.args.root_masked = roots[1];
     st.args.root_blend = roots[2];
     st.args.opaque_nodes = opaqueNodes;
+    st.args.opaque_tri_first = 0u;
+    st.args.opaque_tri_end = roots[0] >= 0 ? opaqueRecords : 0u;
+    ++st.worldTopologySeq;
 }
 
 void setSunArgs(SceneStore& st)
@@ -733,7 +738,7 @@
         ARK_HIP(retireBuffer(st, job->snap, s));
         ARK_HIP(growBoxes(st, st.world, s));
         setWorldArgs(st);
-        setWorldRoots(st, job->roots, job->opaqueNodes);
+        setWorldRoots(st, job->roots, job->opaqueNodes, job->opaqueRecords);
         st.args.tri_normals = st.triNormals.as<float4>();
         st.bvhMaxDepth = std::max(st.world.depth, st.sunArgs.sun_root >= 0 ? st.sun.depth : 0u);
         st.bvhStats.node_count = st.world.nodeCount;
@@ -1111,7 +1116,7 @@
     }
     SceneArgs& sc = st->args;
     setWorldArgs(*st);
-    setWorldRoots(*st, w.roots, w.opaqueNodes);
+    setWorldRoots(*st, w.roots, w.opaqueNodes, w.opaqueRecords);
     sc.tri_normals = st->triNormals.as<float4>();
     sc.texture_count = static_cast<int32_t>(s->texture_count);
     sc.indices = st->indices.as<uint32_t>();
diff --git a/arkoserenderer_amd/csrc/scene_store.h b/arkoserenderer_amd/csrc/scene_store.h
--- a/arkoserenderer_amd/csrc/scene_store.h
+++ b/arkoserenderer_amd/csrc/scene_store.h
@@ -117,6 +117,7 @@
     bool installValid = false;
     hipEvent_t evGeometry = nullptr;
     uint32_t geometrySeq = 0;
+    uint32_t worldTopologySeq = 0;
     SceneStore();
     SceneStore(const SceneStore&) = delete;
     SceneStore& operator=(const SceneStore&) = delete;
diff --git a/arkoserenderer_amd/csrc/seed_cache.h b/arkoserenderer_amd/csrc/seed_cache.h
--- /dev/null
+++ b/arkoserenderer_amd/csrc/seed_cache.h
@@ -0,0 +1,49 @@
+#pragma once
+
+#include <stdint.h>
+
+#if defined(__HIPCC__) || defined(__CUDACC__)
+#define ARK_SEED_FN __host__ __device__ inline
+#else
+#define ARK_SEED_FN inline
+#endif
+
+namespace ark {
+namespace seed {
+
+#ifndef ARK_SEED_TEXELS
+#define ARK_SEED_TEXELS 16
+#endif
+constexpr uint32_t kTexels = ARK_SEED_TEXELS;
+constexpr uint32_t kProbeWords = kTexels * kTexels;
+constexpr uint32_t kNone = 0xffffffffu;
+
+ARK_SEED_FN uint32_t texelOfT(float x, float y, float z, uint32_t texels)
+{
+    const float ax = x < 0.0f ? -x : x, ay = y < 0.0f ? -y : y, az = z < 0.0f ? -z : z;
+    const float n = ax + ay + az;
+    const float inv = n > 0.0f ? 1.0f / n : 0.0f;
+    float u = x * inv, v = y * inv;
+    if (z < 0.0f) {
+        const float au = u < 0.0f ? -u : u, av = v < 0.0f ? -v : v;
+        const float fu = (1.0f - av) * (u < 0.0f ? -1.0f : 1.0f);
+        const float fv = (1.0f - au) * (v < 0.0f ? -1.0f : 1.0f);
+        u = fu;
+        v = fv;
+    }
+    const float T = static_cast<float>(texels);
+    const float fx = (u * 0.5f + 0.5f) * T, fy = (v * 0.5f + 0.5f) * T;
+    const uint32_t ix = fx > 0.0f ? (fx < T ? static_cast<uint32_t>(fx) : texels - 1u) : 0u;
+    const uint32_t iy = fy > 0.0f ? (fy < T ? static_cast<uint32_t>(fy) : texels - 1u) : 0u;
+    return iy * texels + ix;
+}
+
+ARK_SEED_FN uint32_t texelOf(float x, float y, float z) { return texelOfT(x, y, z, kTexels); }
+
+ARK_SEED_FN bool candidateOk(uint32_t word, uint32_t first, uint32_t end)
+{
+    return word >= first && word < end;
+}
+
+}
+}
diff --git a/arkoserenderer_amd/ddgi.py b/arkoserenderer_amd/ddgi.py
--- a/arkoserenderer_amd/ddgi.py
+++ b/arkoserenderer_amd/ddgi.py
@@ -56,6 +56,7 @@
     gpu_rebuild_plan: bool = False
     sun_cover_map: bool = True
     fused_sun_shade: bool = True
+    ray_seeds: bool = True
     build_threads: int = 0
 
 
@@ -97,6 +98,7 @@
     d.flags |= abi.ARK_DDGI_FLAG_GPU_REBUILD_PLAN if config.gpu_rebuild_plan else 0
     d.flags |= 0 if config.sun_cover_map else abi.ARK_DDGI_FLAG_NO_SUN_COVER_MAP
     d.flags |= 0 if config.fused_sun_shade else abi.ARK_DDGI_FLAG_NO_FUSED_SUN_SHADE
+    d.flags |= 0 if config.ray_seeds else abi.ARK_DDGI_FLAG_NO_RAY_SEEDS
     d.build_threads = int(config.build_threads)
     return d
 
@@ -331,6 +333,14 @@
         out = (C.c_uint64 * 2)()
         self.check(self.lib.ark_ddgi_debug_shade_schedule(self.h, out), "ark_ddgi_debug_shade_schedule")
         return {"sun_only": bool(out[0]), "deferred": int(out[1])}
+
+    def seed_info(self) -> dict:
+        out = (C.c_uint64 * 5)()
+        self.check(self.lib.ark_ddgi_debug_seed_info(self.h, out), "ark_ddgi_debug_seed_info")
+        return {"enabled": bool(out[0]), "texels": int(out[1]), "first": int(out[2]), "end": int(out[3]), "candidate_hits": int(out[4])}
+
+    def seed_fill(self, mode: int, value: int = 0):
+        self.check(self.lib.ark_ddgi_debug_seed_fill(self.h, int(mode), int(value)), "ark_ddgi_debug_seed_fill")
 
     def set_sun_only_small_windows(self, on: bool):
         self.check(self.lib.ark_ddgi_debug_set_sun_only_small_windows(self.h, int(on)), "ark_ddgi_debug_set_sun_only_small_windows")
diff --git a/arkoserenderer_amd/host/apps/ddgi_headless.cpp b/arkoserenderer_amd/host/apps/ddgi_headless.cpp
--- a/arkoserenderer_amd/host/apps/ddgi_headless.cpp
+++ b/arkoserenderer_amd/host/apps/ddgi_headless.cpp
@@ -280,6 +280,7 @@
     double exchangeTimeout = 0.0;
     std::string saveStatePath, loadStatePath, frameScriptPath;
     int firstFrame = 0, gpuRebuild = 0;
+    bool raySeeds = true;
     bool deadlineTest = false;
     const std::time_t startedAt = std::time(nullptr);
     float zFar = 10000.0f, exposure = 1.0f, env = 1.0f, ambient = 0.0f;
@@ -317,6 +318,7 @@
         else if (a == "--first-frame") firstFrame = std::atoi(next());
         else if (a == "--frame-script") frameScriptPath = next();
         else if (a == "--gpu-rebuild") gpuRebuild = std::atoi(next());
+        else if (a == "--no-ray-seeds") raySeeds = false;
         else ARKOSE_LOG(Fatal, "unknown argument %s", a.c_str());
     }
     SceneFile file;
@@ -363,6 +365,7 @@
         node.setGpuRebuildSun((gpuRebuild & 2) != 0);
         node.setGpuRebuildSah((gpuRebuild & 4) != 0);
         node.setGpuRebuildPlan((gpuRebuild & 8) != 0);
+        node.setRaySeeds(raySeeds);
         if (slabCount > 1) node.setShard(shardRank, slabCount);
         return pipeline;
     };
diff --git a/arkoserenderer_amd/host/rendering/nodes/DDGINode.cpp b/arkoserenderer_amd/host/rendering/nodes/DDGINode.cpp
--- a/arkoserenderer_amd/host/rendering/nodes/DDGINode.cpp
+++ b/arkoserenderer_amd/host/rendering/nodes/DDGINode.cpp
@@ -75,7 +75,8 @@
     desc.shard_rank = m_shardRank;
     desc.shard_count = m_shardCount;
     desc.flags = (m_gpuRebuild ? ARK_DDGI_FLAG_GPU_REBUILD : 0u) | (m_gpuRebuildSun ? ARK_DDGI_FLAG_GPU_REBUILD_SUN : 0u) |
-                 (m_gpuRebuildSah ? ARK_DDGI_FLAG_GPU_REBUILD_SAH : 0u) | (m_gpuRebuildPlan ? ARK_DDGI_FLAG_GPU_REBUILD_PLAN : 0u);
+                 (m_gpuRebuildSah ? ARK_DDGI_FLAG_GPU_REBUILD_SAH : 0u) | (m_gpuRebuildPlan ? ARK_DDGI_FLAG_GPU_REBUILD_PLAN : 0u) |
+                 (m_raySeeds ? 0u : ARK_DDGI_FLAG_NO_RAY_SEEDS);
     auto created = reg.createOrReuseDdgiContext("ddgi", desc);
     ArkDdgiCtx* ctx = created.first;
     if (!ctx) {
diff --git a/arkoserenderer_amd/host/rendering/nodes/DDGINode.h b/arkoserenderer_amd/host/rendering/nodes/DDGINode.h
--- a/arkoserenderer_amd/host/rendering/nodes/DDGINode.h
+++ b/arkoserenderer_amd/host/rendering/nodes/DDGINode.h
@@ -26,6 +26,7 @@
     void setGpuRebuildSun(bool on) { m_gpuRebuildSun = on; }
     void setGpuRebuildSah(bool on) { m_gpuRebuildSah = on; }
     void setGpuRebuildPlan(bool on) { m_gpuRebuildPlan = on; }
+    void setRaySeeds(bool on) { m_raySeeds = on; }
     void setSlabExchange(SlabExchange* exchange) { m_exchange = exchange; }
     void* pendingExchange() const { return m_exchangePending; }
     ArkDdgiCtx* context() const { return m_ctx; }
@@ -60,6 +61,7 @@
     bool m_gpuRebuildSun { false };
     bool m_gpuRebuildSah { false };
     bool m_gpuRebuildPlan { false };
+    bool m_raySeeds { true };
     ArkDdgiCtx* m_ctx { nullptr };
     uint32_t m_instanceVersion { 0 };
     SlabExchange* m_exchange { nullptr };
diff --git a/include/ark_ddgi.h b/include/ark_ddgi.h
--- a/include/ark_ddgi.h
+++ b/include/ark_ddgi.h
@@ -91,6 +91,7 @@
 #define ARK_DDGI_FLAG_NO_SUN_COVER_MAP 0x20u
 #define ARK_DDGI_FLAG_NO_FUSED_SUN_SHADE 0x40u
 #define ARK_DDGI_FLAG_GPU_REBUILD_PLAN 0x80u
+#define ARK_DDGI_FLAG_NO_RAY_SEEDS 0x100u
 
 typedef struct ArkRTVertex {
     float tex_coord[2];
diff --git a/include/ark_ddgi_debug.h b/include/ark_ddgi_debug.h
--- a/include/ark_ddgi_debug.h
+++ b/include/ark_ddgi_debug.h
@@ -68,6 +68,11 @@
 int ark_ddgi_debug_shade_schedule(struct ArkDdgiCtx* ctx, uint64_t* out);
 int ark_ddgi_debug_set_sun_only_small_windows(struct ArkDdgiCtx* ctx, int enabled);
 
+uint32_t ark_ddgi_debug_seed_texel(float x, float y, float z);
+int ark_ddgi_debug_seed_candidate_ok(uint32_t word, uint32_t first, uint32_t end);
+int ark_ddgi_debug_seed_info(struct ArkDdgiCtx* ctx, uint64_t* out);
+int ark_ddgi_debug_seed_fill(struct ArkDdgiCtx* ctx, int mode, uint64_t value);
+
 #ifdef __cplusplus
 }
 #endif
```

New measurement: 3251 Mrays/s (median of 6 runs). +5.6%, better.
